# muelea/tuch

Measured on AMD Instinct MI355X. Metric: SMPLify-DC fit iters/sec at batch 64, higher is better.
Workload: dtype f32; 1 GPU; configs[1] extended to the full stage-2 step: batch=64/GPU SMPL forward + contact_fitting_loss (L_P/L_C push/pull, winding inside test, segment filter, r2r) + backward + Adam, V=6890 F=13776, float32; bodies_per_gpu=64, global_batch=64, launch=hipGraph replay of the whole step

## Files before the change

### include/tuch_amd.h

```cpp
#ifndef TUCH_AMD_H
#define TUCH_AMD_H

#include <stddef.h>
#include <stdint.h>

#ifdef __cplusplus
extern "C" {
#endif

const char* tuch_last_error(void);
int tuch_abi_version(void);


int tuch_batch_pairwise_dist(const float* x, const float* y, int B, int Nx, int Ny, int squared,
                             float* P, void* stream);

int tuch_batch_pairwise_dist_bwd(const float* x, const float* y, const float* grad_P, int B, int Nx, int Ny,
                                 int squared, float* grad_x, float* grad_y, void* stream);

int tuch_solid_angles_bwd(const float* points, const float* triangles, const float* grad_out, const float* grad_w,
                          int B, int Q, int F, float* grad_points, float* grad_triangles, void* stream);

int tuch_solid_angles(const float* points, const float* triangles, int B, int Q, int F, float* out,
                      void* stream);
// ... 74 lines not shown
size_t tuch_smplify_stage2_fused_scratch_floats(int B);
int tuch_smplify_stage2_fused(const float* points, const int32_t* partner, const uint8_t* exterior,
                              const uint8_t* body_valid, int B, int N, int mode, float euclthres,
                              const float* small_terms, const float* r2r, const int32_t* ij, int P, float contact_scale,
                              float r2r_scale, float* share, int* ticket, float* terms, float* out, float* grad_points,
                              const tuch_contact_model* model, const void* pair_keys, void* grad_fixed_zeroed, void* stream);
int tuch_fixed_to_float(const void* fixed, size_t n, float* out, void* stream);
void tuch_set_deterministic(int on);
int tuch_get_deterministic(void);

int tuch_region_pair_keys(const tuch_contact_model* model, const float* verts, int B, const uint8_t* select,
                          int use_geomask, void* keys_zeroed, void* stream);
int tuch_smplify_stage2_finish(const float* points, const int32_t* partner, const uint8_t* exterior,
                               const uint8_t* body_valid, int B, int N, int mode, float euclthres,
                               const float* small_terms, const float* r2r, int P, float contact_scale, float r2r_scale,
                               float* share, int* ticket, float* terms, float* out, void* stream);
int tuch_smplify_stage2_bwd(const float* grad_out, const uint8_t* body_valid, const float* points, const int32_t* partner,
                            const uint8_t* exterior, int B, int N, int mode, float euclthres, float contact_scale,
                            const int32_t* ij, int P, float r2r_scale, const float* gj, const float* gc, const float* gp,
                            int NJ, float* grad_points, float* gj_out, float* gc_out, float* gp_out, void* stream);

typedef struct tuch_contact_model tuch_contact_model;

int tuch_contact_model_create(tuch_contact_model** out, int V, int F, const int32_t* faces ,
                              const uint8_t* geomask ,
                              int num_segments, const int32_t* seg_q_off, const int32_t* seg_q_vidx,
                              const int32_t* seg_f_off, const int32_t* seg_faces,
                              int num_caps, const int32_t* cap_off, const int32_t* cap_vidx,
                              int num_regions, const int32_t* region_off, const int32_t* region_vidx,
                              int num_pairs, const int32_t* pairs);
void tuch_contact_model_destroy(tuch_contact_model* model);
int tuch_contact_model_set_option(tuch_contact_model* model, const char* name, int value);
int tuch_contact_model_get_option(const tuch_contact_model* model, const char* name, int* value);
int tuch_contact_model_canary_hits(const tuch_contact_model* model, int* hits_host, int reset);
int tuch_contact_model_canary_selftest(const tuch_contact_model* model, void* workspace, size_t workspace_bytes, void* stream);
const uint64_t* tuch_contact_model_mask_bits(const tuch_contact_model* model);
const int32_t* tuch_contact_model_faces(const tuch_contact_model* model);
int32_t* tuch_contact_model_tickets(const tuch_contact_model* model);
const uint64_t* tuch_contact_model_tree_mask_bits(const tuch_contact_model* model);
int tuch_contact_model_info(const tuch_contact_model* model, int* V, int* F, int* num_segments,
                            int* seg_q_total, int* num_pairs);
int tuch_contact_model_strips(const tuch_contact_model* model, int* stream_len, int* num_strips,
                              int32_t* vidx_host, float* sign_host);

int tuch_winding_tree_work(const tuch_contact_model* model, const float* verts, int B, void* workspace,
                           size_t workspace_bytes, unsigned long long* out_host, void* stream);

int tuch_ray_work(const tuch_contact_model* model, const float* verts, int B, void* workspace,
                  size_t workspace_bytes, unsigned long long* out_host, void* stream);
int tuch_contact_model_tree_order(const tuch_contact_model* model, int32_t* qperm_host, int32_t* face_leaf_host);

size_t tuch_v2v_model_workspace_bytes(const tuch_contact_model* model, int B);
size_t tuch_v2v_hint_bytes(const tuch_contact_model* model, int B);
int tuch_v2v_min_model(const tuch_contact_model* model, const float* verts, int B, float* min_d2,
                       int32_t* argmin, void* hint_inout, void* workspace, size_t workspace_bytes, void* stream);
int tuch_v2v_min_model_shared(const tuch_contact_model* model, const float* verts, int B, float* min_d2,
                              int32_t* argmin, void* hint_inout, void* workspace, size_t workspace_bytes, int leave_room,
                              void* stream);
int tuch_v2v_min_model_shared_zero(const tuch_contact_model* model, const float* verts, int B, float* min_d2, int32_t* argmin,
                                   void* hint_inout, void* workspace, size_t workspace_bytes, int leave_room, void* zero,
                                   size_t zero_bytes, void* stream);

int tuch_v2v_min_model_can_cap(const tuch_contact_model* model);
int tuch_v2v_min_model_capped(const tuch_contact_model* model, const float* verts, int B, float* min_d2, int32_t* argmin,
                              void* hint_inout, void* workspace, size_t workspace_bytes, int leave_room, void* zero,
                              size_t zero_bytes, const uint8_t* prev_exterior, float cap, void* stream);
int tuch_v2v_min_model_fix(const tuch_contact_model* model, int B, const uint8_t* exterior, uint8_t* prev_exterior, float cap,
                           float* min_d2, int32_t* argmin, void* hint_inout, void* workspace, size_t workspace_bytes,
                           void* stream);

typedef struct tuch_cluster_tree tuch_cluster_tree;
int tuch_cluster_tree_build(int V, int F, const int32_t* faces, int leaf_faces, tuch_cluster_tree** out);
void tuch_cluster_tree_free(tuch_cluster_tree* tree);
int tuch_cluster_tree_info(const tuch_cluster_tree* tree, int* num_nodes, int* exact_len, int* stream_len,
                           int* num_qblocks, int* num_frontiers, int* frontier_total);
int tuch_cluster_tree_export(const tuch_cluster_tree* tree, int32_t* nodes, int32_t* vidx, float* sign,
                             int32_t* qperm, int32_t* frontier_off, int32_t* frontier_nodes,
                             int32_t* launch_order, int32_t* rows, int32_t* face_leaf);

size_t tuch_exterior_workspace_bytes(const tuch_contact_model* model, int B);
int tuch_exterior_flags(const tuch_contact_model* model, const float* verts, int B, int apply_segments,
                        float thresh, float* w, uint8_t* exterior, float* seg_w, uint8_t* seg_exterior,
                        void* workspace, size_t workspace_bytes, void* stream);

size_t tuch_winding_points_workspace_bytes(const tuch_contact_model* model, int B, int Q);
int tuch_winding_points(const tuch_contact_model* model, const float* verts, const float* points,
                        const int32_t* counts, int B, int Q, float thresh, float* w, uint8_t* exterior,
                        void* workspace, size_t workspace_bytes, void* stream);

int tuch_region_pair_min(const tuch_contact_model* model, const float* verts, int B, const uint8_t* select,
                         int use_geomask, float* out_min, int32_t* out_ij, void* stream);
int tuch_region_pair_min_bwd(const tuch_contact_model* model, const float* verts, int B, const int32_t* ij,
                             const float* grad_out, float* grad_verts, void* stream);

int tuch_self_contact(const float* verts , const uint64_t* geomask_bits, int B, int V, float euclthres,
                      const int32_t* vreg_off , const int32_t* vreg , int R,
                      uint8_t* in_contact , int32_t* partner , float* min_d2 ,
                      float* sig_d2 , float* cnc_d2 , void* stream);

typedef struct tuch_smpl_model tuch_smpl_model;

int tuch_smpl_model_create(tuch_smpl_model** out, int V, const float* v_template, const float* shapedirs,
                           const float* posedirs, const float* J_regressor, const float* lbs_weights,
                           const int32_t* parents, const int32_t* extra_vertex_ids,
                           const float* J_regressor_extra, const int32_t* joint_map);
void tuch_smpl_model_destroy(tuch_smpl_model* model);
int tuch_smpl_model_info(const tuch_smpl_model* model, int* V);

size_t tuch_smpl_forward_workspace_bytes(const tuch_smpl_model* model, int B);
int tuch_smpl_forward(const tuch_smpl_model* model, const float* betas, const float* pose, int pose2rot, int B,
                      float* verts, float* joints, void* workspace, size_t workspace_bytes, void* stream);
int tuch_smpl_forward_split(const tuch_smpl_model* model, const float* betas, const float* global_orient,
                            int global_orient_stride, const float* body_pose, int body_pose_stride, int pose2rot, int B,
                            float* verts, float* joints, void* workspace, size_t workspace_bytes, void* stream);
size_t tuch_smpl_backward_workspace_bytes(const tuch_smpl_model* model, int B);
int tuch_smpl_backward(const tuch_smpl_model* model, const float* pose, int pose2rot, int B,
                       const void* fwd_workspace, const float* g_verts, const float* g_joints, float* g_betas,
                       float* g_pose, void* workspace, size_t workspace_bytes, void* stream);
int tuch_smpl_backward_split(const tuch_smpl_model* model, const float* global_orient, int global_orient_stride,
                             const float* body_pose, int body_pose_stride, int pose2rot, int B,
                             const void* fwd_workspace, const float* g_verts, const float* g_joints, float* g_betas,
                             float* g_global_orient, int g_global_orient_stride, float* g_body_pose,
                             int g_body_pose_stride, void* workspace, size_t workspace_bytes, void* stream);
int tuch_smpl_backward_split_add(const tuch_smpl_model* model, const float* global_orient, int global_orient_stride,
                                 const float* body_pose, int body_pose_stride, int pose2rot, int B,
                                 const void* fwd_workspace, const float* g_verts, const float* g_joints, float* g_betas,
                                 float* g_global_orient, int g_global_orient_stride, float* g_body_pose,
                                 int g_body_pose_stride, const float* g_body_pose_add, int g_body_pose_add_stride,
                                 void* workspace, size_t workspace_bytes, void* stream, const void* g_verts_fixed);
int tuch_smpl_backward_split_adam(const tuch_smpl_model* model, const float* global_orient, int global_orient_stride,
                                  const float* body_pose, int body_pose_stride, int B, const void* fwd_workspace,
                                  const float* g_verts, const float* g_joints, float* g_betas, float* g_global_orient,
                                  int g_global_orient_stride, float* g_body_pose, int g_body_pose_stride,
                                  const float* g_body_pose_add, int g_body_pose_add_stride,
                                  float* param_global_orient, int param_global_orient_stride, float* param_body_pose,
                                  int param_body_pose_stride, float* exp_avg_global_orient, float* exp_avg_sq_global_orient,
                                  float* exp_avg_body_pose, float* exp_avg_sq_body_pose, float* step, int* ticket,
                                  float lr, float beta1, float beta2, float eps,
                                  void* workspace, size_t workspace_bytes, void* stream, const void* g_verts_fixed);

int tuch_estimate_translation(const float* joints3d, const float* keypoints2d, const uint8_t* has_anno, int B, int J,
                              float focal_length, float img_size, float* trans, void* stream);
int tuch_rotmat_to_angle_axis(const float* rotmat, int N, int row_stride, float* angle_axis, void* stream);

int tuch_procrustes(const void* S1, const void* S2, int B, int N, int D, int coords_first, int is_double, void* S1_hat,
                    void* err, void* stream);
int tuch_pose_metrics(const float* pred_vertices, const float* gt_vertices, const float* gt_joints,
                      const float* J_regressor, const int32_t* joint_map, int B, int V, int R, int J, int pelvis_index,
                      float* mpjpe, float* pa_mpjpe, float* v2v, float* joints, void* stream);

typedef struct tuch_hd_model tuch_hd_model;
int tuch_hd_model_create(tuch_hd_model** out, const tuch_contact_model* contact_model, int N, const int32_t* hd_idx,
                         const float* hd_w, const int32_t* hd_face);
int tuch_hd_model_create_k(tuch_hd_model** out, const tuch_contact_model* contact_model, int N, int K,
                           const int32_t* hd_idx, const float* hd_w, const int32_t* hd_face);
void tuch_hd_model_destroy(tuch_hd_model* model);
int tuch_hd_model_info(const tuch_hd_model* model, int* N, int32_t* order_host);
size_t tuch_hd_contact_saved_bytes(const tuch_hd_model* model, int B);
size_t tuch_hd_contact_workspace_bytes(const tuch_hd_model* model, int B);
int tuch_hd_contact_fwd(const tuch_hd_model* model, const float* verts, const uint8_t* exterior, const float* min_d2,
                        const int32_t* partner, const uint8_t* valid, int B, float euclthres, float thresh, float* terms,
                        void* saved, size_t saved_bytes, void* workspace, size_t workspace_bytes, void* stream);
int tuch_hd_contact_bwd(const tuch_hd_model* model, const void* saved, const float* grad_terms, int B,
                        float* grad_verts, void* workspace, size_t workspace_bytes, void* stream);
int tuch_hd_contact_selection(const tuch_hd_model* model, const void* saved, int B, int32_t* counts_host,
                              int32_t* selected_host);
// ... 12 lines not shown
```

### tuch_amd/_C.py

```python
from __future__ import annotations

import ctypes
import os
from ctypes import POINTER, c_char_p, c_float, c_int, c_size_t, c_void_p

import torch

_HERE = os.path.dirname(os.path.abspath(__file__))
LIB_PATH = os.environ.get('TUCH_AMD_LIB') or os.path.join(_HERE, 'libtuch_amd.so')
_lib = None

_SIGNATURES = {
    'tuch_last_error': (c_char_p, []),
    'tuch_abi_version': (c_int, []),
    'tuch_batch_pairwise_dist': (c_int, [c_void_p, c_void_p, c_int, c_int, c_int, c_int, c_void_p, c_void_p]),
    'tuch_batch_pairwise_dist_bwd': (c_int, [c_void_p, c_void_p, c_void_p, c_int, c_int, c_int, c_int, c_void_p, c_void_p,
                                             c_void_p]),
    'tuch_solid_angles_bwd': (c_int, [c_void_p, c_void_p, c_void_p, c_void_p, c_int, c_int, c_int, c_void_p, c_void_p, c_void_p]),
    'tuch_solid_angles': (c_int, [c_void_p, c_void_p, c_int, c_int, c_int, c_void_p, c_void_p]),
    'tuch_gather_triangles': (c_int, [c_void_p, c_void_p, c_int, c_int, c_int, c_void_p, c_void_p]),
    'tuch_winding_workspace_bytes': (c_size_t, [c_int, c_int, c_int]),
    'tuch_winding_numbers': (c_int, [c_void_p, c_void_p, c_int, c_int, c_int, c_void_p, c_void_p, c_float,
                                     c_void_p, c_size_t, c_void_p]),
    'tuch_geomask_words': (c_int, [c_int]),
# ... 1 lines not shown
    'tuch_pack_geomask': (c_int, [c_void_p, c_int, c_void_p, c_void_p]),
    'tuch_v2v_workspace_bytes': (c_size_t, [c_int, c_int]),
    'tuch_v2v_min_masked': (c_int, [c_void_p, c_void_p, c_int, c_int, c_void_p, c_void_p, c_void_p, c_size_t,
                                    c_void_p]),
    'tuch_v2v_min_indexed_workspace_bytes': (c_size_t, [c_int, c_int]),
    'tuch_v2v_min_indexed': (c_int, [c_void_p, c_void_p, c_void_p, c_void_p, c_int, c_int, c_int, c_void_p, c_void_p,
                                     c_void_p, c_size_t, c_void_p]),
    'tuch_v2v_min_indexed_mfma_workspace_bytes': (c_size_t, [c_int, c_int]),
    'tuch_v2v_min_indexed_mfma': (c_int, [c_void_p, c_void_p, c_void_p, c_void_p, c_int, c_int, c_int, c_void_p, c_void_p,
                                          c_void_p, c_size_t, c_void_p]),
    'tuch_contact_terms_fwd': (c_int, [c_void_p, c_void_p, c_void_p, c_void_p, c_int, c_int, c_int, c_float,
                                       c_void_p, c_void_p]),
    'tuch_contact_terms_bwd': (c_int, [c_void_p, c_void_p, c_void_p, c_void_p, c_int, c_int, c_int, c_float,
                                       c_void_p, c_void_p]),
    'tuch_valid_mean_fwd': (c_int, [c_void_p, c_void_p, c_int, c_int, c_void_p, c_void_p]),
    'tuch_valid_mean_bwd': (c_int, [c_void_p, c_void_p, c_void_p, c_int, c_int, c_void_p, c_void_p]),
    'tuch_smpl_backward_split_adam': (c_int, [c_void_p, c_void_p, c_int, c_void_p, c_int, c_int, c_void_p, c_void_p, c_void_p,
                                              c_void_p, c_void_p, c_int, c_void_p, c_int, c_void_p, c_int,
                                              c_void_p, c_int, c_void_p, c_int, c_void_p, c_void_p, c_void_p, c_void_p, c_void_p,
                                              c_void_p, c_float, c_float, c_float, c_float, c_void_p, c_size_t, c_void_p, c_void_p]),
    'tuch_contact_terms_bwd_fixed': (c_int, [c_void_p, c_void_p, c_void_p, c_void_p, c_int, c_int, c_int, c_float,
                                             c_void_p, c_void_p, c_void_p]),
    'tuch_smplify_small_terms': (c_int, [c_void_p] * 9 + [c_int, c_int, c_int, c_float, c_float, c_float] + [c_void_p] * 5),
    'tuch_smplify_stage1_terms': (c_int, [c_void_p] * 7 + [c_int, c_int, c_int, c_float, c_float, c_float, c_float] + [c_void_p] * 7),
    'tuch_adam_step': (c_int, [c_int, c_void_p, c_void_p, c_void_p, c_void_p, c_void_p, c_void_p, c_void_p, c_float, c_float,
                                c_void_p]),
    'tuch_smplify_objective': (c_int, [c_void_p, c_void_p, c_void_p, c_int, c_int, c_float, c_float, c_void_p, c_void_p]),
    'tuch_smplify_objective_bwd': (c_int, [c_void_p, c_int, c_int, c_float, c_float, c_void_p, c_void_p, c_void_p,
                                           c_void_p]),
    'tuch_smplify_tail_bwd': (c_int, [c_void_p] * 5 + [c_int, c_int, c_int, c_float, c_float] + [c_void_p] * 6),
    'tuch_contact_model_create': (c_int, [POINTER(c_void_p), c_int, c_int, c_void_p, c_void_p,
                                          c_int, c_void_p, c_void_p, c_void_p, c_void_p,
                                          c_int, c_void_p, c_void_p,
                                          c_int, c_void_p, c_void_p, c_int, c_void_p]),
    'tuch_contact_model_destroy': (None, [c_void_p]),
    'tuch_contact_model_set_option': (c_int, [c_void_p, c_char_p, c_int]),
    'tuch_contact_model_get_option': (c_int, [c_void_p, c_char_p, POINTER(c_int)]),
    'tuch_contact_model_canary_hits': (c_int, [c_void_p, POINTER(c_int), c_int]),
    'tuch_contact_model_canary_selftest': (c_int, [c_void_p, c_void_p, c_size_t, c_void_p]),
    'tuch_contact_model_mask_bits': (c_void_p, [c_void_p]),
    'tuch_contact_model_faces': (c_void_p, [c_void_p]),
    'tuch_contact_model_tickets': (c_void_p, [c_void_p]),
    'tuch_contact_model_tree_mask_bits': (c_void_p, [c_void_p]),
    'tuch_contact_model_info': (c_int, [c_void_p, POINTER(c_int), POINTER(c_int), POINTER(c_int),
                                        POINTER(c_int), POINTER(c_int)]),
    'tuch_contact_model_strips': (c_int, [c_void_p, POINTER(c_int), POINTER(c_int), c_void_p, c_void_p]),
    'tuch_cluster_tree_build': (c_int, [c_int, c_int, c_void_p, c_int, POINTER(c_void_p)]),
    'tuch_cluster_tree_free': (None, [c_void_p]),
    'tuch_cluster_tree_info': (c_int, [c_void_p] + [POINTER(c_int)] * 6),
    'tuch_cluster_tree_export': (c_int, [c_void_p] * 10),
    'tuch_hd_points_fwd': (c_int, [c_void_p] * 5 + [c_int, c_int, c_void_p, c_void_p]),
    'tuch_hd_points_bwd': (c_int, [c_void_p] * 5 + [c_int, c_int, c_void_p, c_void_p]),
    'tuch_estimate_translation': (c_int, [c_void_p, c_void_p, c_void_p, c_int, c_int, c_float, c_float, c_void_p, c_void_p]),
    'tuch_rotmat_to_angle_axis': (c_int, [c_void_p, c_int, c_int, c_void_p, c_void_p]),
    'tuch_winding_tree_work': (c_int, [c_void_p, c_void_p, c_int, c_void_p, c_size_t, c_void_p, c_void_p]),
    'tuch_hd_model_create': (c_int, [POINTER(c_void_p), c_void_p, c_int, c_void_p, c_void_p, c_void_p]),
    'tuch_hd_model_create_k': (c_int, [POINTER(c_void_p), c_void_p, c_int, c_int, c_void_p, c_void_p, c_void_p]),
    'tuch_hd_model_destroy': (None, [c_void_p]),
    'tuch_hd_model_info': (c_int, [c_void_p, POINTER(c_int), c_void_p]),
    'tuch_hd_contact_saved_bytes': (c_size_t, [c_void_p, c_int]),
    'tuch_hd_contact_workspace_bytes': (c_size_t, [c_void_p, c_int]),
    'tuch_hd_contact_fwd': (c_int, [c_void_p] * 6 + [c_int, c_float, c_float, c_void_p, c_void_p, c_size_t, c_void_p, c_size_t,
                                    c_void_p]),
    'tuch_hd_contact_bwd': (c_int, [c_void_p, c_void_p, c_void_p, c_int, c_void_p, c_void_p, c_size_t, c_void_p]),
    'tuch_hd_contact_selection': (c_int, [c_void_p, c_void_p, c_int, c_void_p, c_void_p]),
    'tuch_hd_contact_details': (c_int, [c_void_p, c_void_p, c_int, c_void_p, c_void_p]),
    'tuch_ray_work': (c_int, [c_void_p, c_void_p, c_int, c_void_p, c_size_t, c_void_p, c_void_p]),
    'tuch_contact_model_tree_order': (c_int, [c_void_p, c_void_p, c_void_p]),
    'tuch_v2v_model_workspace_bytes': (c_size_t, [c_void_p, c_int]),
    'tuch_v2v_hint_bytes': (c_size_t, [c_void_p, c_int]),
    'tuch_v2v_min_model': (c_int, [c_void_p, c_void_p, c_int, c_void_p, c_void_p, c_void_p, c_void_p, c_size_t, c_void_p]),
    'tuch_v2v_min_model_shared': (c_int, [c_void_p, c_void_p, c_int, c_void_p, c_void_p, c_void_p, c_void_p, c_size_t, c_int,
                                          c_void_p]),
    'tuch_v2v_min_model_shared_zero': (c_int, [c_void_p, c_void_p, c_int, c_void_p, c_void_p, c_void_p, c_void_p, c_size_t, c_int,
                                               c_void_p, c_size_t, c_void_p]),
    'tuch_exterior_workspace_bytes': (c_size_t, [c_void_p, c_int]),
    'tuch_v2v_min_model_can_cap': (c_int, [c_void_p]),
    'tuch_v2v_min_model_capped': (c_int, [c_void_p, c_void_p, c_int, c_void_p, c_void_p, c_void_p, c_void_p, c_size_t, c_int,
                                          c_void_p, c_size_t, c_void_p, c_float, c_void_p]),
    'tuch_v2v_min_model_fix': (c_int, [c_void_p, c_int, c_void_p, c_void_p, c_float, c_void_p, c_void_p, c_void_p, c_void_p,
                                       c_size_t, c_void_p]),
    'tuch_exterior_flags': (c_int, [c_void_p, c_void_p, c_int, c_int, c_float, c_void_p, c_void_p, c_void_p,
                                    c_void_p, c_void_p, c_size_t, c_void_p]),
    'tuch_winding_points_workspace_bytes': (c_size_t, [c_void_p, c_int, c_int]),
    'tuch_winding_points': (c_int, [c_void_p, c_void_p, c_void_p, c_void_p, c_int, c_int, c_float, c_void_p, c_void_p,
                                    c_void_p, c_size_t, c_void_p]),
    'tuch_contact_terms_ragged_fwd': (c_int, [c_void_p, c_void_p, c_void_p, c_void_p, c_int, c_int, c_float, c_void_p,
                                              c_void_p]),
    'tuch_contact_terms_ragged_bwd': (c_int, [c_void_p, c_void_p, c_void_p, c_void_p, c_void_p, c_int, c_int, c_float,
                                              c_void_p, c_void_p]),
    'tuch_region_pair_min': (c_int, [c_void_p, c_void_p, c_int, c_void_p, c_int, c_void_p, c_void_p, c_void_p]),
    'tuch_smpl_model_create': (c_int, [POINTER(c_void_p), c_int] + [c_void_p] * 9),
    'tuch_smpl_model_destroy': (None, [c_void_p]),
    'tuch_smpl_model_info': (c_int, [c_void_p, POINTER(c_int)]),
    'tuch_smpl_forward_workspace_bytes': (c_size_t, [c_void_p, c_int]),
    'tuch_smpl_backward_workspace_bytes': (c_size_t, [c_void_p, c_int]),
    'tuch_smpl_forward': (c_int, [c_void_p, c_void_p, c_void_p, c_int, c_int, c_void_p, c_void_p, c_void_p,
                                  c_size_t, c_void_p]),
    'tuch_smpl_backward': (c_int, [c_void_p, c_void_p, c_int, c_int, c_void_p, c_void_p, c_void_p, c_void_p,
                                   c_void_p, c_void_p, c_size_t, c_void_p]),
    'tuch_smplify_stage2_fused_scratch_floats': (c_size_t, [c_int]),
    'tuch_smplify_stage2_fused': (c_int, [c_void_p, c_void_p, c_void_p, c_void_p, c_int, c_int, c_int, c_float, c_void_p, c_void_p,
                                           c_void_p, c_int, c_float, c_float, c_void_p, c_void_p, c_void_p, c_void_p, c_void_p,
                                           c_void_p, c_void_p, c_void_p, c_void_p]),
    'tuch_set_deterministic': (None, [c_int]),
    'tuch_get_deterministic': (c_int, []),
    'tuch_region_pair_keys': (c_int, [c_void_p, c_void_p, c_int, c_void_p, c_int, c_void_p, c_void_p]),
    'tuch_smplify_stage2_finish': (c_int, [c_void_p, c_void_p, c_void_p, c_void_p, c_int, c_int, c_int, c_float, c_void_p,
                                           c_void_p, c_int, c_float, c_float, c_void_p, c_void_p, c_void_p, c_void_p,
                                           c_void_p]),
    'tuch_smplify_stage2_bwd': (c_int, [c_void_p, c_void_p, c_void_p, c_void_p, c_void_p, c_int, c_int, c_int, c_float,
                                        c_float, c_void_p, c_int, c_float, c_void_p, c_void_p, c_void_p, c_int, c_void_p,
                                        c_void_p, c_void_p, c_void_p, c_void_p]),
    'tuch_smpl_forward_split': (c_int, [c_void_p, c_void_p, c_void_p, c_int, c_void_p, c_int, c_int, c_int, c_void_p,
                                        c_void_p, c_void_p, c_size_t, c_void_p]),
    'tuch_smpl_backward_split': (c_int, [c_void_p, c_void_p, c_int, c_void_p, c_int, c_int, c_int, c_void_p, c_void_p,
                                         c_void_p, c_void_p, c_void_p, c_int, c_void_p, c_int, c_void_p, c_size_t,
                                         c_void_p]),
    'tuch_smpl_backward_split_add': (c_int, [c_void_p, c_void_p, c_int, c_void_p, c_int, c_int, c_int, c_void_p, c_void_p,
                                             c_void_p, c_void_p, c_void_p, c_int, c_void_p, c_int, c_void_p, c_int, c_void_p,
                                             c_size_t, c_void_p, c_void_p]),
    'tuch_fixed_to_float': (c_int, [c_void_p, c_size_t, c_void_p, c_void_p]),
    'tuch_region_pair_min_bwd': (c_int, [c_void_p, c_void_p, c_int, c_void_p, c_void_p, c_void_p, c_void_p]),
    'tuch_self_contact': (c_int, [c_void_p, c_void_p, c_int, c_int, c_float, c_void_p, c_void_p, c_int] + [c_void_p] * 6),
    'tuch_procrustes': (c_int, [c_void_p, c_void_p, c_int, c_int, c_int, c_int, c_int, c_void_p, c_void_p, c_void_p]),
    'tuch_pose_metrics': (c_int, [c_void_p] * 5 + [c_int] * 5 + [c_void_p] * 5),
}


def exported_symbols():
    return sorted(_SIGNATURES)


def lib() -> ctypes.CDLL:
    global _lib
    if _lib is None:
        if not os.path.exists(LIB_PATH):
            raise RuntimeError(
                'libtuch_amd.so is not built (%s). Run `python -m tuch_amd._build` (needs hipcc); '
                'there is no CPU fallback.' % LIB_PATH)
        L = ctypes.CDLL(LIB_PATH)
        for name, (res, args) in _SIGNATURES.items():
            fn = getattr(L, name)
            fn.restype = res
            fn.argtypes = args
        _lib = L
    return _lib


class TuchError(RuntimeError):
    pass


def check(rc: int) -> None:
    if rc != 0:
        raise TuchError('libtuch_amd error %d: %s' % (rc, lib().tuch_last_error().decode()))


def ptr(t) -> c_void_p:
    if t is None:
        return c_void_p(0)
    if not t.is_cuda:
        raise TuchError('tuch_amd kernels need tensors on a HIP device, got %s' % t.device)
    if not t.is_contiguous():
        raise TuchError('tuch_amd kernels need contiguous tensors')
    return c_void_p(t.data_ptr())
# ... 19 lines not shown
```

### tuch_amd/csrc/model.h

```cpp
#pragma once
#include "common.h"
#include <vector>

struct tuch_cluster_tree {
    int V = 0, F = 0, num_nodes = 0, exact_len = 0, stream_len = 0, num_qblocks = 0, num_heights = 0;
    std::vector<int32_t> nodes;
    std::vector<int32_t> vidx;
    std::vector<float> sign;
    std::vector<int32_t> qperm;
    std::vector<int32_t> height_off, height_nodes;
    std::vector<int32_t> frontier_off, frontier_nodes;
    std::vector<int32_t> launch_order;
    std::vector<int32_t> ancestors;
    std::vector<int32_t> rows;
    std::vector<int32_t> face_leaf;
};

bool tuch_cluster_tree_build_impl(int V, int F, const int32_t* faces, int leaf_faces, tuch_cluster_tree& t);
void tuch_build_strips(const int32_t* faces, int F, std::vector<int32_t>& vidx, std::vector<float>& sign,
                       int* num_strips);

struct tuch_contact_model;

struct tuch_options {
    int winding_ray = 1;
    int winding_tree = 1;
    int winding_strips = 1;
    int tree_waves = 32768;
    int ray_pair_cap = 16;
    int ray_waves = 32768;
    int ray_fans = 0;
    int ray_cross = 0;
    int ray_cross_split = 0;
    int v2v_tree = 1;
    int v2v_waves = 0;
    int v2v_cap = 0;
    int v2v_flat = 2;
    int v2v_pairs = 24;
    int v2v_lds = -1;
    int seg_splits = 16;
    int seg_assist = 1;
    int seg_fused = 1;
    int canary = 0;
    int hd_search = 1;
    int hd_search_waves = 4;
    int hd_overlap = 1;
};
void tuch_options_from_env(tuch_options* o);

bool tuch_ray_available(const tuch_contact_model* m);
struct RayEntry { int32_t leaf, node; uint32_t mask_lo, mask_hi; };
struct RayTile { int32_t ex_off, ex_len, first, n; };
struct RayBody { int32_t tiles, overflow; };
struct TreeNode;
void tuch_ray_layout_touch(const tuch_contact_model* m, int B, int Q);
size_t tuch_ray_workspace_bytes(const tuch_contact_model* m, int B, int Q);
int tuch_ray_exterior_verts(const tuch_contact_model* m, const float* verts, int B, float thresh, uint8_t* exterior,
                            float* w, void* workspace, hipStream_t s, unsigned long long* stats_host,
                            uint8_t* exterior_copy = nullptr);
const int32_t* tuch_ray_segment_counts(const tuch_contact_model* m, int B, const void* workspace);
void tuch_ray_segment_prepare(const tuch_contact_model* m, const float* verts, const float* caps, int assisted, int B,
                              float* seg_entries, hipStream_t s);
bool tuch_ray_segment_fused_available(const tuch_contact_model* m);
int tuch_ray_segment_flags_one(const tuch_contact_model* m, const float* verts, const uint8_t* body_flags,
                               const int32_t* leaf_counts, int B, float thresh, uint8_t* exterior, hipStream_t s);
int tuch_ray_segment_flags(const tuch_contact_model* m, const float* verts, const float* caps, const int32_t* seg_count,
                           const int32_t* seg_list, const int32_t* leaf_counts, int B, int nsplit, float thresh, float* seg_tris,
                           int32_t* seg_partial, float* seg_w, uint8_t* seg_ext, uint8_t* exterior, hipStream_t s);
int tuch_ray_exterior_points(const tuch_contact_model* m, const float* verts, const float* points, const int32_t* counts,
                             int B, int Q, float thresh, uint8_t* exterior, float* w, void* workspace, hipStream_t s);

int tuch_v2v_min_indexed_seeded(const float* points, const int32_t* vertex_ids, const int32_t* offsets,
                                const int32_t* counts, const float* seed_best, const int32_t* seed_arg,
                                const int32_t* all_masked_arg, const uint64_t* geomask_bits, int B, int V,
                                int max_points_per_body, float* min_d2, int32_t* argmin, void* workspace, hipStream_t s);
extern "C" size_t tuch_v2v_min_indexed_workspace_bytes(int B, int max_points_per_body);
size_t tuch_hd_search_workspace_bytes(int B, int max_points_per_body);
int tuch_hd_search(const float* points, const int32_t* vertex_ids, const int32_t* offsets, const int32_t* counts,
                   const int32_t* all_masked_arg, const uint64_t* geomask_bits, int B, int V, int max_points_per_body,
                   float* min_d2, int32_t* argmin, void* workspace, hipStream_t s, int waves);
extern "C" size_t tuch_winding_points_workspace_bytes(const tuch_contact_model* m, int B, int Q);
extern "C" int tuch_winding_points(const tuch_contact_model* m, const float* verts, const float* points,
                                   const int32_t* counts, int B, int Q, float thresh, float* w,
                                   uint8_t* exterior, void* workspace, size_t workspace_bytes, void* stream);

struct tuch_contact_model {
    int device;
    tuch_options opt;
    int V, F;
    int32_t* faces;
    int32_t* tickets;
    int32_t* canary_hits;
    uint64_t* mask_bits;
    int strip_len, num_strips;
    int32_t* strip_vidx;
    float* strip_sign;
    int tree_nodes, tree_stream_len, tree_exact_len, tree_qblocks, tree_heights, tree_leaves;
    int32_t* tree_node;
    int32_t* tree_vidx;
    float* tree_sign;
    int32_t* tree_sign_word;
    int32_t* tree_qperm;
    int32_t* tree_height_off;
    int32_t* tree_height_nodes;
    int32_t* tree_frontier_nodes;
    int32_t* tree_launch_order;
    int32_t* tree_ancestors;
    int32_t* tree_rows;
    int32_t* tree_v2v_info;
    uint64_t* tree_mask_bits;
    uint64_t* tree_masked;
    int32_t* tree_sub_leaf;
    uint64_t* tree_masked_leaf;
    int32_t* tree_leaf_group;
    uint64_t* tree_mask_bits_g;
    int tree_groups;
    int tree_leaf_rows_max;
    int mask_symmetric;
    int tree_num_frontiers;
    int tree_leaf_runs_tile;
    int* tree_frontier_off_host;
    int* tree_sub_leaf_host;
    int32_t* tree_face_leaf_host;
    int32_t* tree_qperm_host;
    int32_t* ring_off;
    int32_t* ring_vidx;
    int ring_max;
    int num_segments, num_caps, seg_q_total, seg_f_total;
    int32_t* seg_q_off;
    int32_t* seg_q_vidx;
    int32_t* seg_f_off;
    int32_t* seg_faces;
    int32_t* cap_off;
    int32_t* cap_vidx;
    int32_t* seg_link_off;
    int32_t* seg_link;
    int32_t* seg_ray_off;
    int32_t* seg_ray_ent;
    int seg_ray_total;
    int32_t* seg_elem_mask;
    int32_t* seg_vmask;
    int32_t* seg_vpos;
// ... 19 lines not shown
```

### tuch_amd/csrc/model.hip

```cpp
#include "model.h"
#include <stdio.h>
#include <stdlib.h>
#include <string.h>
#include <algorithm>
#include <vector>
#include <unordered_map>

extern "C" int tuch_geomask_words(int V);

namespace {

template <typename T>
int upload(T** dst, const T* src, size_t count)
{
    return tuch_table_upload((void**)dst, src, count * sizeof(T));
}

int* host_copy(const int32_t* src, size_t n)
{
    int* p = (int*)malloc(sizeof(int) * (n ? n : 1));
    if (n) memcpy(p, src, sizeof(int) * n);
    return p;
}

// ... 345 lines not shown
                        m->seg_cap_total = coff.back();
                        elem_mask_host = emask;
                        rc = upload(&m->seg_elem_mask, emask.data(), emask.size());
                        if (rc == TUCH_OK) rc = upload(&m->seg_vmask, vmask.data(), vmask.size());
                        if (rc == TUCH_OK) rc = upload(&m->seg_vpos, vpos.data(), vpos.size());
                        if (rc == TUCH_OK) rc = upload(&m->seg_cap_off, coff.data(), coff.size());
                        if (rc == TUCH_OK) rc = upload(&m->seg_cap_ent, cent.data(), cent.size());
                        std::vector<int32_t> crange(1, 0);
                        bool consecutive = true;
                        for (int sg = 0; sg < num_segments && consecutive; ++sg) {
                            int lo = num_caps, hi = -1;
                            auto see = [&](int id) { if (id >= V) { lo = std::min(lo, id - V); hi = std::max(hi, id - V); } };
                            for (int e = coff[sg]; e < coff[sg + 1]; ++e)
                                for (int k = 0; k < 3; ++k) see(cent[3 * (size_t)e + k]);
                            for (int q = seg_q_off[sg]; q < seg_q_off[sg + 1]; ++q)
                                for (int e = loff[q]; e < loff[q + 1]; ++e) { see(links[2 * (size_t)e]); see(links[2 * (size_t)e + 1]); }
                            if (hi < 0) { crange.push_back(crange.back()); continue; }
                            consecutive = lo == crange.back() && hi - lo + 1 <= 8;
                            crange.push_back(hi + 1);
                        }
                        if (rc == TUCH_OK && consecutive) rc = upload(&m->seg_cap_range, crange.data(), crange.size());
                    }
                }
            }
        }
    }
    if (rc == TUCH_OK && num_regions > 0) {
        m->num_regions = num_regions;
        m->num_pairs = num_pairs;
        m->region_off_host = host_copy(region_off, num_regions + 1);
        for (int r = 0; r < num_regions; ++r) {
            const int n = region_off[r + 1] - region_off[r];
            if (n > m->region_max) m->region_max = n;
        }
        rc = upload(&m->region_off, region_off, (size_t)num_regions + 1);
        if (rc == TUCH_OK) rc = upload(&m->region_vidx, region_vidx, (size_t)region_off[num_regions]);
        if (rc == TUCH_OK && num_pairs > 0) rc = upload(&m->pairs, pairs, (size_t)num_pairs * 2);
        if (rc == TUCH_OK && num_pairs > 0 && geomask) {
            std::vector<int64_t> off(num_pairs + 1, 0);
            for (int p = 0; p < num_pairs; ++p) {
                const int n1 = region_off[pairs[2 * p] + 1] - region_off[pairs[2 * p]];
                const int n2 = region_off[pairs[2 * p + 1] + 1] - region_off[pairs[2 * p + 1]];
                off[p + 1] = off[p] + (int64_t)n1 * ((n2 + 31) / 32);
            }
            std::vector<uint32_t> words((size_t)off[num_pairs], 0u);
            for (int p = 0; p < num_pairs; ++p) {
                const int32_t* r1 = region_vidx + region_off[pairs[2 * p]];
                const int32_t* r2 = region_vidx + region_off[pairs[2 * p + 1]];
                const int n1 = region_off[pairs[2 * p] + 1] - region_off[pairs[2 * p]];
                const int n2 = region_off[pairs[2 * p + 1] + 1] - region_off[pairs[2 * p + 1]];
                const int wpr = (n2 + 31) / 32;
                for (int a = 0; a < n1; ++a)
                    for (int k = 0; k < n2; ++k)
                        if (geomask[(size_t)r1[a] * V + r2[k]])
                            words[(size_t)off[p] + (size_t)a * wpr + (k >> 5)] |= 1u << (k & 31);
            }
            rc = upload(&m->pair_mask, words.data(), words.size());
            if (rc == TUCH_OK) rc = upload(&m->pair_mask_off, off.data(), off.size());
        }
    }
    if (rc == TUCH_OK && !tree_sign_host.empty()) {
        std::vector<int32_t> word(tree_sign_host.size(), 0);
        for (size_t p = 0; p < word.size(); ++p) {
            const int32_t sg = tree_sign_host[p] > 0.0f ? 1 : tree_sign_host[p] < 0.0f ? -1 : 0;
            const int32_t em = p < elem_mask_host.size() ? elem_mask_host[p] : 0;
            word[p] = (int32_t)(((uint32_t)em << 24) | ((uint32_t)sg & 0xffffffu));
        }
        rc = upload(&m->tree_sign_word, word.data(), word.size());
    }
    if (rc != TUCH_OK) {
        tuch_contact_model_destroy(m);
        *out = nullptr;
        return rc;
    }
    *out = m;
    return TUCH_OK;
}

namespace {
struct OptionName { const char* name; int tuch_options::*field; };
const OptionName kOptions[] = {
    {"winding_ray", &tuch_options::winding_ray}, {"winding_tree", &tuch_options::winding_tree},
    {"winding_strips", &tuch_options::winding_strips}, {"tree_waves", &tuch_options::tree_waves},
    {"ray_pair_cap", &tuch_options::ray_pair_cap}, {"ray_waves", &tuch_options::ray_waves}, {"ray_fans", &tuch_options::ray_fans}, {"ray_cross", &tuch_options::ray_cross}, {"v2v_cap", &tuch_options::v2v_cap}, {"ray_cross_split", &tuch_options::ray_cross_split},
    {"v2v_tree", &tuch_options::v2v_tree}, {"v2v_flat", &tuch_options::v2v_flat}, {"v2v_pairs", &tuch_options::v2v_pairs}, {"v2v_waves", &tuch_options::v2v_waves}, {"v2v_lds", &tuch_options::v2v_lds},
    {"seg_splits", &tuch_options::seg_splits}, {"seg_assist", &tuch_options::seg_assist}, {"seg_fused", &tuch_options::seg_fused},
    {"canary", &tuch_options::canary}, {"hd_search", &tuch_options::hd_search}, {"hd_search_waves", &tuch_options::hd_search_waves}, {"hd_overlap", &tuch_options::hd_overlap},
};
}

void tuch_options_from_env(tuch_options* o)
{
    for (const OptionName& k : kOptions) {
        char env[64] = "TUCH_";
        size_t n = strlen(env);
        for (const char* c = k.name; *c && n + 1 < sizeof(env); ++c) env[n++] = (char)toupper((unsigned char)*c);
        env[n] = 0;
        const char* e = getenv(env);
        if (e && *e) o->*(k.field) = atoi(e);
    }
}

extern "C" int tuch_contact_model_set_option(tuch_contact_model* m, const char* name, int value)
{
    TUCH_REQUIRE(m && name, "tuch_contact_model_set_option: null argument");
    for (const OptionName& k : kOptions)
        if (!strcmp(k.name, name)) {
            TUCH_REQUIRE(strcmp(name, "seg_assist") != 0, "tuch_contact_model_set_option: seg_assist is fixed when the model "
                         "is created (TUCH_SEG_ASSIST)");
            m->opt.*(k.field) = value;
            return TUCH_OK;
        }
    tuch_set_error("tuch_contact_model_set_option: unknown option '%s'", name);
    return TUCH_ERR_ARG;
}

extern "C" int tuch_contact_model_canary_hits(const tuch_contact_model* m, int* hits_host, int reset)
{
    TUCH_REQUIRE(m && hits_host, "tuch_contact_model_canary_hits: null argument");
    if (hipDeviceSynchronize() != hipSuccess ||
        hipMemcpy(hits_host, m->canary_hits, sizeof(int32_t), hipMemcpyDeviceToHost) != hipSuccess ||
        (reset && hipMemset(m->canary_hits, 0, sizeof(int32_t)) != hipSuccess)) {
        tuch_set_error("tuch_contact_model_canary_hits: %s", hipGetErrorString(hipGetLastError()));
        return TUCH_ERR_HIP;
    }
    return TUCH_OK;
}

extern "C" int tuch_contact_model_get_option(const tuch_contact_model* m, const char* name, int* value)
{
    TUCH_REQUIRE(m && name && value, "tuch_contact_model_get_option: null argument");
    if (!strcmp(name, "seg_fused_active")) {
        *value = tuch_ray_segment_fused_available(m) ? 1 : 0;
        return TUCH_OK;
    }
    for (const OptionName& k : kOptions)
        if (!strcmp(k.name, name)) {
            *value = m->opt.*(k.field);
            return TUCH_OK;
        }
    tuch_set_error("tuch_contact_model_get_option: unknown option '%s'", name);
    return TUCH_ERR_ARG;
}

extern "C" const uint64_t* tuch_contact_model_mask_bits(const tuch_contact_model* m)
{
    return m ? m->mask_bits : nullptr;
}

extern "C" const uint64_t* tuch_contact_model_tree_mask_bits(const tuch_contact_model* m)
{
    return m ? m->tree_mask_bits : nullptr;
}

extern "C" int32_t* tuch_contact_model_tickets(const tuch_contact_model* m)
{
    return m ? m->tickets : nullptr;
}

extern "C" const int32_t* tuch_contact_model_faces(const tuch_contact_model* m)
{
    return m ? m->faces : nullptr;
}

extern "C" int tuch_contact_model_tree_order(const tuch_contact_model* m, int32_t* qperm_host, int32_t* face_leaf_host)
{
    TUCH_REQUIRE(m, "tuch_contact_model_tree_order: null model");
// ... 32 lines not shown
```

### tuch_amd/csrc/ray_winding.hip

```cpp
#include "common.h"
#include "model.h"
#include "workspace.h"
#include "tree_device.h"
#include <stdlib.h>

#pragma clang fp contract(off)

namespace {

constexpr float kPi = 3.14159265358979323846f;
constexpr int kBlock = 256;
constexpr int kRayQueries = 64;
constexpr float kShearX = 0.3217f, kShearY = 0.4331f;
constexpr float kFanX = 0.8191f, kFanY = 0.3467f, kFanZ = 0.4571f;
constexpr int kSlabs = 9;
constexpr int kSlabStride = 10;
constexpr int kNearSlabs = 13;

struct RayElem { float x, y, z, sign; };

__device__ __forceinline__ float shear_x(float x, float z) { return __builtin_fmaf(-kShearX, z, x); }
__device__ __forceinline__ float shear_y(float y, float z) { return __builtin_fmaf(-kShearY, z, y); }

__global__ __launch_bounds__(kBlock) void ray_stream_kernel(
// ... 4 lines not shown
    const int p = blockIdx.x * kBlock + threadIdx.x;
    for (size_t g = ((size_t)b * gridDim.x + blockIdx.x) * kBlock + threadIdx.x; g < zeroed_n;
         g += (size_t)gridDim.x * gridDim.y * kBlock)
        zeroed[g] = make_uint4(0u, 0u, 0u, 0u);
    if (p >= Lpad) return;
    RayElem e = {0.f, 0.f, 0.f, 0.f};
    if (p < L) {
        const float* c = verts + ((size_t)b * V + vidx[p]) * 3;
        e.x = shear_x(c[0], c[2]); e.y = shear_y(c[1], c[2]); e.z = c[2]; e.sign = sign[p];
    }
    out[(size_t)b * Lpad + p] = e;
}

__device__ __forceinline__ void slab_project(float x, float y, float z, float (&p)[kSlabs])
{
    p[0] = x; p[1] = y; p[2] = z;
    p[3] = x + y; p[4] = x - y; p[5] = x + z; p[6] = x - z; p[7] = y + z; p[8] = y - z;
}

template <int kCtrl>
__device__ __forceinline__ float dpp_move(float x)
{
    return __int_as_float(__builtin_amdgcn_update_dpp(0, __float_as_int(x), kCtrl, 0xF, 0xF, true));
}
__device__ __forceinline__ float row_min(float v)
{
    v = fminf(v, dpp_move<0xB1>(v));
    v = fminf(v, dpp_move<0x4E>(v));
    v = fminf(v, dpp_move<0x141>(v));
    v = fminf(v, dpp_move<0x140>(v));
    return v;
}

__device__ __forceinline__ uint32_t half_below(float x)
{
    const _Float16 h = (_Float16)x;
    uint32_t u = __builtin_bit_cast(uint16_t, h);
    if ((float)h > x) u = (u & 0x8000u) ? u + 1 : (u == 0 ? 0x8001u : u - 1);
    return u;
}
__device__ __forceinline__ uint32_t half_above(float x)
{
    const _Float16 h = (_Float16)x;
    uint32_t u = __builtin_bit_cast(uint16_t, h);
    if ((float)h < x) u = (u & 0x8000u) ? (u == 0x8000u ? 0x0001u : u - 1) : u + 1;
    return u;
}
__device__ __host__ __forceinline__ size_t near_records_at(int B, int L) { return (size_t)B * kNearSlabs * L; }
__device__ __host__ __forceinline__ size_t near_centres_at(int B, int L) { return near_records_at(B, L) + (size_t)B * L * 8; }

struct QRec { float x, y, z; int32_t tag; };
constexpr int kNoSlot = 0xffffff;
struct RayPre { int blocks, qblocks; QRec* qrec; float4* ranges; const int32_t* vmask; };

__device__ __forceinline__ void ray_block_prepass(const float* __restrict__ vb, int first_vertex,
                                                  const int32_t* __restrict__ qperm, const int32_t* __restrict__ vmask,
                                                  int Q, int qb, int lane, QRec* __restrict__ qrec, float4* __restrict__ ranges)
{
    const int slot = qb * kRayQueries + lane;
    const float* q3 = vb + 3 * (size_t)qperm[slot];
    const float* c0 = vb + 3 * (size_t)first_vertex;
    const float qz = q3[2], qx = shear_x(q3[0], qz), qy = shear_y(q3[1], qz);
    const float cz = c0[2], cx = shear_x(c0[0], cz), cy = shear_y(c0[1], cz);
    QRec r;
    r.x = qx; r.y = qy; r.z = qz;
    r.tag = slot < Q ? (slot | (vmask ? vmask[slot] << 24 : 0)) : kNoSlot;
    qrec[slot] = r;
    const float rx = qx - cx, ry = qy - cy, rz = qz - cz;
    const float r4 = rx + ry, r5 = rx - ry, r6 = rx + rz, r7 = rx - rz, r8 = ry + rz, r9 = ry - rz;
    const float bx0 = wave_min_uniform(rx), bx1 = wave_max_uniform(rx), by0 = wave_min_uniform(ry), by1 = wave_max_uniform(ry);
    const float b40 = wave_min_uniform(r4), b41 = wave_max_uniform(r4), b50 = wave_min_uniform(r5), b51 = wave_max_uniform(r5);
    const float bz0 = wave_min_uniform(rz), b60 = wave_min_uniform(r6), b71 = wave_max_uniform(r7);
    const float b80 = wave_min_uniform(r8), b91 = wave_max_uniform(r9);
    if (lane == 0) {
        ranges[0] = make_float4(bx0, bx1, by0, by1);
        ranges[1] = make_float4(b40, b41, b50, b51);
        ranges[2] = make_float4(bz0, b60, b71, b80);
        ranges[3] = make_float4(b91, 0.f, 0.f, 0.f);
    }
}

__device__ __forceinline__ float fan_terms(const float* __restrict__ vb, int v, bool real, int& n,
                                           const int32_t* __restrict__ ring_off, const int32_t* __restrict__ ring_vidx);
template <bool kPose>
__global__ __launch_bounds__(kBoundsBlock) void ray_leaf_bounds_kernel(
    const RayElem* __restrict__ stream, int T, const TreeNode* __restrict__ nodes, int N,
    const int32_t* __restrict__ height_off, const int32_t* __restrict__ height_nodes, float* __restrict__ bounds,
    const float* __restrict__ verts, const int32_t* __restrict__ vidx, const float* __restrict__ sign, int V, int Lexact,
    RayElem* __restrict__ stream_out, uint4* __restrict__ zeroed, size_t zeroed_n,
    int leaf_blocks = 0, const int32_t* __restrict__ qperm = nullptr, const int32_t* __restrict__ ring_off = nullptr,
    const int32_t* __restrict__ ring_vidx = nullptr, float2* __restrict__ fans = nullptr, int fan_stride = 0,
    RayPre pre = RayPre{0, 0, nullptr, nullptr, nullptr})
{
    if (kPose && pre.blocks > 0 && (int)blockIdx.x >= (int)gridDim.x - pre.blocks) {
        for (size_t g = ((size_t)blockIdx.y * gridDim.x + blockIdx.x) * kBoundsBlock + threadIdx.x; g < zeroed_n;
             g += (size_t)gridDim.x * gridDim.y * kBoundsBlock)
            zeroed[g] = make_uint4(0u, 0u, 0u, 0u);
        const int qb = ((int)blockIdx.x - ((int)gridDim.x - pre.blocks)) * (kBoundsBlock / 64) + (int)(threadIdx.x >> 6);
        if (qb < pre.qblocks)
            ray_block_prepass(verts + (size_t)blockIdx.y * V * 3, vidx[0], qperm, pre.vmask, V, qb, threadIdx.x & 63,
                              pre.qrec + (size_t)blockIdx.y * pre.qblocks * kRayQueries,
                              pre.ranges + ((size_t)blockIdx.y * pre.qblocks + qb) * 4);
        return;
    }
    if (kPose && leaf_blocks > 0 && (int)blockIdx.x >= leaf_blocks) {
        for (size_t g = ((size_t)blockIdx.y * gridDim.x + blockIdx.x) * kBoundsBlock + threadIdx.x; g < zeroed_n;
             g += (size_t)gridDim.x * gridDim.y * kBoundsBlock)
            zeroed[g] = make_uint4(0u, 0u, 0u, 0u);
        const int i = ((int)blockIdx.x - leaf_blocks) * kBoundsBlock + (int)threadIdx.x;
        const bool real = i < V;
        const int v = qperm[real ? i : V - 1];
        int cr = 0;
        const float half = fan_terms(verts + (size_t)blockIdx.y * V * 3, v, real, cr, ring_off, ring_vidx);
        if (i < fan_stride) fans[(size_t)blockIdx.y * fan_stride + i] = make_float2(__int_as_float(cr), half);
        return;
    }
    const int b = blockIdx.y;
    const RayElem* st = stream + (size_t)b * T;
    const int group = threadIdx.x >> 4, sub = threadIdx.x & 15;
    const int i = height_off[0] + blockIdx.x * (kBoundsBlock / 16) + group;
    const bool real = i < height_off[1];
    const int node = height_nodes[real ? i : height_off[0]];
    const int off = nodes[node].ex_off, len = real ? nodes[node].ex_len : 0;
    if (kPose) {
        for (size_t g = ((size_t)b * gridDim.x + blockIdx.x) * kBoundsBlock + threadIdx.x; g < zeroed_n;
             g += (size_t)gridDim.x * gridDim.y * kBoundsBlock)
            zeroed[g] = make_uint4(0u, 0u, 0u, 0u);
        if (blockIdx.x == 0)
            for (int p = Lexact + (int)threadIdx.x; p < T; p += kBoundsBlock) stream_out[(size_t)b * T + p] = RayElem{0.f, 0.f, 0.f, 0.f};
    }
    float lo[kSlabs], nhi[kSlabs];
#pragma unroll
    for (int k = 0; k < kSlabs; ++k) { lo[k] = 3.0e38f; nhi[k] = 3.0e38f; }
    for (int p = sub; p < len; p += 16) {
        RayElem e;
        if (kPose) {
            const float* c = verts + ((size_t)b * V + vidx[off + p]) * 3;
            e.x = shear_x(c[0], c[2]); e.y = shear_y(c[1], c[2]); e.z = c[2]; e.sign = sign[off + p];
            stream_out[(size_t)b * T + off + p] = e;
        } else {
            e = st[off + p];
        }
        float pr[kSlabs];
        slab_project(e.x, e.y, e.z, pr);
#pragma unroll
        for (int k = 0; k < kSlabs; ++k) { lo[k] = fminf(lo[k], pr[k]); nhi[k] = fminf(nhi[k], -pr[k]); }
    }
#pragma unroll
    for (int k = 0; k < kSlabs; ++k) { lo[k] = row_min(lo[k]); nhi[k] = row_min(nhi[k]); }
    if (real && sub == 0) {
        const int L = height_off[1] - height_off[0], leaf = i - height_off[0];
        float lo_p[kSlabs], hi_p[kSlabs];
#pragma unroll
        for (int k = 0; k < kSlabs; ++k) {
            const float hi = -nhi[k];
            const float pad = 4e-7f * fmaxf(fabsf(lo[k]), fabsf(hi)) + 1e-9f;
            lo_p[k] = lo[k] - pad;
            hi_p[k] = hi + pad;
        }
        float c[3];
        if (kPose) {
            const float* c0 = verts + ((size_t)b * V + vidx[0]) * 3;
            c[0] = shear_x(c0[0], c0[2]); c[1] = shear_y(c0[1], c0[2]); c[2] = c0[2];
        } else {
            const RayElem e0 = st[0];
            c[0] = e0.x; c[1] = e0.y; c[2] = e0.z;
        }
        float pc[kSlabs];
        slab_project(c[0], c[1], c[2], pc);
        uint32_t lo_h[kSlabs], hi_h[kSlabs];
#pragma unroll
        for (int k = 0; k < kSlabs; ++k) {
            const float pad = 4e-6f * (fabsf(lo_p[k]) + fabsf(hi_p[k]) + fabsf(pc[k])) + 1e-7f;
            lo_h[k] = half_below(lo_p[k] - pc[k] - pad);
            hi_h[k] = half_above(hi_p[k] - pc[k] + pad);
        }
        uint4* r = reinterpret_cast<uint4*>(bounds + near_records_at(gridDim.y, L)) + ((size_t)b * L + leaf) * 2;
        r[0] = make_uint4(lo_h[0] | lo_h[1] << 16, lo_h[3] | lo_h[4] << 16, lo_h[6] | lo_h[8] << 16, hi_h[0] | hi_h[1] << 16);
        r[1] = make_uint4(hi_h[2] | hi_h[3] << 16, hi_h[4] | hi_h[5] << 16, hi_h[7] | (uint32_t)leaf << 16, (uint32_t)node);
        if (leaf == 0) *reinterpret_cast<float4*>(bounds + near_centres_at(gridDim.y, L) + (size_t)b * 4) = make_float4(c[0], c[1], c[2], 0.f);
    }
// ... 73 lines not shown
    s[A].z = el.z - qz;
    e[Bq] = edge_fn(s[Cq], s[A]);
    e[Cq] = edge_fn(s[A], s[Bq]);
    const int word = __float_as_int(el.sign);
    if ((word & 0xffffff) != 0) {
        const float numz = __builtin_fmaf(e[A], s[A].z, __builtin_fmaf(e[Cq], s[Cq].z, e[Bq] * s[Bq].z));
        const float mn = __builtin_fminf(__builtin_fminf(e[0], e[1]), e[2]);
        const float mx = __builtin_fmaxf(__builtin_fmaxf(e[0], e[1]), e[2]);
        int c = (int)(__builtin_fminf(mn, numz) > 0.0f) - (int)(__builtin_fmaxf(mx, numz) < 0.0f);
        const bool edge_zero = mn * mx == 0.0f;
        if (__builtin_amdgcn_ballot_w64(edge_zero)) {
            const bool tie = edge_zero & (numz != 0.0f);
            if (__builtin_amdgcn_ballot_w64(tie)) {
                if (tie) c = crossing_with_ties<kSkipIncident>(p3(s[Bq]), p3(s[Cq]), p3(s[A]), e[Bq], e[Cq], e[A]);
            }
        }
        asm("v_mad_i32_i24 %0, %1, %2, %0" : "+v"(count) : "v"(c), "s"(word));
        if (kSeg && ((uint32_t)word >> 24) != 0) {
            const uint32_t t = ((uint32_t)word >> 24) & (uint32_t)qmask;
            if (__builtin_amdgcn_ballot_w64((t != 0) & (c != 0))) {
                uint32_t cs;
                asm("v_mul_i32_i24 %0, %1, %2" : "=v"(cs) : "v"(c), "s"(word));
                pa += cs * (((t & 15u) * 0x00204081u) & 0x01010101u);
                pb += cs * ((((t >> 4) & 15u) * 0x00204081u) & 0x01010101u);
            }
        }
    }
}

template <bool kSkipIncident, bool kSeg>
__device__ __forceinline__ void ray_run(const RayElem* __restrict__ st, int off, int len,
                                        S3 (&s)[3], float (&e)[3], v2f qxy, float qz, int& count,
                                        int qmask, uint32_t& pa, uint32_t& pb)
{
    const RayElem* p = st + off;
    RayElem n0 = p[0], n1 = p[1], n2 = p[2];
    for (int left = len; left > 0; left -= 3, p += 3) {
        asm("" : "+s"(left));
        const RayElem e0 = n0, e1 = n1, e2 = n2;
        n0 = p[3]; n1 = p[4]; n2 = p[5];
        ray_step<0, kSkipIncident, kSeg>(e0, s, e, qxy, qz, count, qmask, pa, pb);
        ray_step<1, kSkipIncident, kSeg>(e1, s, e, qxy, qz, count, qmask, pa, pb);
        ray_step<2, kSkipIncident, kSeg>(e2, s, e, qxy, qz, count, qmask, pa, pb);
    }
}

constexpr int kFallbackChunks = 8;

__device__ __forceinline__ float wave_min(float v) { return wave_min_uniform(v); }
__device__ __forceinline__ float wave_max(float v) { return wave_max_uniform(v); }


__device__ __forceinline__ float lo_minus(uint32_t s, float q)
{
    float d;
    asm("v_fma_mix_f32 %0, %1, 1.0, -%2 op_sel_hi:[1,0,0]" : "=v"(d) : "v"(s), "v"(q));
    return d;
}
__device__ __forceinline__ float hi_minus(uint32_t s, float q)
{
    float d;
    asm("v_fma_mix_f32 %0, %1, 1.0, -%2 op_sel:[1,0,0] op_sel_hi:[1,0,0]" : "=v"(d) : "v"(s), "v"(q));
    return d;
}
__device__ __forceinline__ float minus_lo(float q, uint32_t s)
{
    float d;
    asm("v_fma_mix_f32 %0, -%1, 1.0, %2 op_sel_hi:[1,0,0]" : "=v"(d) : "v"(s), "v"(q));
    return d;
}
__device__ __forceinline__ float minus_hi(float q, uint32_t s)
{
    float d;
    asm("v_fma_mix_f32 %0, -%1, 1.0, %2 op_sel:[1,0,0] op_sel_hi:[1,0,0]" : "=v"(d) : "v"(s), "v"(q));
    return d;
}
__device__ __forceinline__ float max3(float a, float b, float c)
{
    float d;
    asm("v_max3_f32 %0, %1, %2, %3" : "=v"(d) : "v"(a), "v"(b), "v"(c));
    return d;
}

template <bool kVerts, int kWaves>
__global__ __launch_bounds__(64 * kWaves) void ray_near_kernel(
    const float* __restrict__ pts, const TreeNode* __restrict__ nodes, const float* __restrict__ bounds, int N,
    int num_leaves, const int32_t* __restrict__ qperm,
    const int32_t* __restrict__ counts, int Q, int qblocks, RayEntry* __restrict__ lists, int32_t* __restrict__ list_len,
    int32_t* __restrict__ leaf_cnt,
    unsigned long long* __restrict__ stats,
    const int32_t* __restrict__ ring_off = nullptr, const int32_t* __restrict__ ring_vidx = nullptr,
    float2* __restrict__ fans = nullptr)
{
    if (kVerts && (int)blockIdx.x >= qblocks) {
        const int i = ((int)blockIdx.x - qblocks) * (64 * kWaves) + (int)threadIdx.x;
        const bool real = i < Q;
        const int v = qperm[real ? i : Q - 1];
        int cr = 0;
        const float half = fan_terms(pts + (size_t)blockIdx.y * Q * 3, v, real, cr, ring_off, ring_vidx);
        if (i < qblocks * kRayQueries) fans[(size_t)blockIdx.y * qblocks * kRayQueries + i] = make_float2(__int_as_float(cr), half);
        return;
    }
    __builtin_amdgcn_s_setprio(3);
    const int qb = blockIdx.x, b = blockIdx.y, lane = threadIdx.x & 63;
    const int wave = kWaves > 1 ? __builtin_amdgcn_readfirstlane(threadIdx.x >> 6) : 0;
    __shared__ uint4 queue[64 * kWaves][2];
    __shared__ float range[16];
    __shared__ int queued[2], slots;
    int i0;
    bool real;
    if (kVerts) {
        i0 = qperm[qb * kRayQueries + lane];
        real = qb * kRayQueries + lane < Q;
    } else {
        const int n = counts ? counts[b] : Q;
        if (qb * kRayQueries >= n) {
            if (threadIdx.x == 0) list_len[(size_t)b * qblocks + qb] = 0;
            return;
        }
        i0 = min(qb * kRayQueries + lane, n - 1);
        real = qb * kRayQueries + lane < n;
    }
    if (threadIdx.x == 0) { queued[0] = 0; queued[1] = 0; slots = 0; }
    const float4 ctr = *reinterpret_cast<const float4*>(bounds + near_centres_at(gridDim.y, num_leaves) + (size_t)b * 4);
    const uint4* recs = reinterpret_cast<const uint4*>(bounds + near_records_at(gridDim.y, num_leaves)) + (size_t)b * num_leaves * 2;
    struct Chunk { uint4 r0, r1; };
    auto load_chunk = [&](int base) {
        Chunk c;
        const int lc = min(base + lane, num_leaves - 1);
        c.r0 = recs[lc * 2];
        c.r1 = recs[lc * 2 + 1];
        return c;
    };
    Chunk nxt = load_chunk(wave * 64);
    const float* q3 = pts + ((size_t)b * Q + i0) * 3;
    const float qz = q3[2];
    const float qx = shear_x(q3[0], qz), qy = shear_y(q3[1], qz);
    const float rx = qx - ctr.x, ry = qy - ctr.y, rz = qz - ctr.z;
    const float r4 = rx + ry, r5 = rx - ry, r6 = rx + rz, r7 = rx - rz, r8 = ry + rz, r9 = ry - rz;
    float bx0, bx1, by0, by1, b40, b41, b50, b51, bz0, b60, b71, b80, b91;
    if (kWaves == 4) {
        if (wave == 0) {
            const float a = wave_min(rx), c = wave_max(rx), d = wave_min(ry), e = wave_max(ry);
            if (lane == 0) { range[0] = a; range[1] = c; range[2] = d; range[3] = e; }
        } else if (wave == 1) {
            const float a = wave_min(r4), c = wave_max(r4), d = wave_min(r5), e = wave_max(r5);
            if (lane == 0) { range[4] = a; range[5] = c; range[6] = d; range[7] = e; }
        } else if (wave == 2) {
            const float a = wave_min(rz), c = wave_min(r6), d = wave_max(r7);
            if (lane == 0) { range[8] = a; range[9] = c; range[10] = d; }
        } else {
            const float a = wave_min(r8), c = wave_max(r9);
            if (lane == 0) { range[11] = a; range[12] = c; }
        }
        __syncthreads();
        bx0 = range[0]; bx1 = range[1]; by0 = range[2]; by1 = range[3]; b40 = range[4]; b41 = range[5]; b50 = range[6];
        b51 = range[7]; bz0 = range[8]; b60 = range[9]; b71 = range[10]; b80 = range[11]; b91 = range[12];
    } else {
        bx0 = wave_min(rx); bx1 = wave_max(rx); by0 = wave_min(ry); by1 = wave_max(ry);
        b40 = wave_min(r4); b41 = wave_max(r4); b50 = wave_min(r5); b51 = wave_max(r5);
        bz0 = wave_min(rz); b60 = wave_min(r6); b71 = wave_max(r7); b80 = wave_min(r8); b91 = wave_max(r9);
    }
    RayEntry* list = lists + ((size_t)b * qblocks + qb) * num_leaves;
    unsigned long long useful = 0, listed = 0;
    auto outside13 = [&](const uint4& s0, const uint4& s1, float x1, float x0, float y1, float y0, float p1, float p0,
                         float m1, float m0, float z0, float xz0, float xz1, float yz0, float yz1) {
        float out = max3(lo_minus(s0.x, x1), minus_lo(x0, s0.w), hi_minus(s0.x, y1));
        out = max3(out, minus_hi(y0, s0.w), lo_minus(s0.y, p1));
        out = max3(out, minus_hi(p0, s1.x), hi_minus(s0.y, m1));
        out = max3(out, minus_lo(m0, s1.y), minus_lo(z0, s1.x));
        out = max3(out, minus_hi(xz0, s1.y), lo_minus(s0.z, xz1));
        return max3(out, minus_lo(yz0, s1.z), hi_minus(s0.z, yz1));
    };
    auto outside = [&](const uint4& s0, const uint4& s1) {
        return outside13(s0, s1, rx, rx, ry, ry, r4, r4, r5, r5, rz, r6, r7, r8, r9);
    };
    int nslots = 0;
    auto emit = [&](const uint4& s1, unsigned long long hit) {
        if (!hit) return;
        const int leaf = (int)(s1.z >> 16), nd = (int)s1.w;
        if (kWaves == 1) ++nslots;
        if (lane == 0) {
            const int slot = kWaves == 1 ? nslots - 1 : atomicAdd(&slots, 1);
            list[slot] = RayEntry{leaf, nd, (uint32_t)hit, (uint32_t)(hit >> 32)};
            atomicAdd(&leaf_cnt[(size_t)b * num_leaves + leaf], __builtin_popcountll(hit));
        }
        if (stats) {
            const int len = nodes[nd].ex_len;
            useful += (unsigned long long)__builtin_popcountll(hit) * len;
            listed += 64ull * len;
        }
    };
    auto sync = [&] { if (kWaves > 1) __syncthreads(); else __builtin_amdgcn_wave_barrier(); };
    for (int round = 0; round * 64 * kWaves < num_leaves; ++round) {
        const int base = (round * kWaves + wave) * 64;
        const Chunk c = nxt;
        if (base + 64 * kWaves < num_leaves) nxt = load_chunk(base + 64 * kWaves);
        const bool pass = (base + lane < num_leaves) &
                          !(outside13(c.r0, c.r1, bx1, bx0, by1, by0, b41, b40, b51, b50, bz0, b60, b71, b80, b91) > 0.0f);
        const unsigned long long mask = __builtin_amdgcn_ballot_w64(pass);
        if (mask) {
            int at = 0;
            if (kWaves > 1) {
                if (lane == 0) at = atomicAdd(&queued[round & 1], __builtin_popcountll(mask));
                at = __builtin_amdgcn_readfirstlane(at);
            }
            at += __builtin_amdgcn_mbcnt_hi((uint32_t)(mask >> 32), __builtin_amdgcn_mbcnt_lo((uint32_t)mask, 0));
            if (pass) { queue[at][0] = c.r0; queue[at][1] = c.r1; }
        }
        sync();
        const int n = kWaves > 1 ? queued[round & 1] : __builtin_popcountll(mask);
        if (kWaves > 1 && threadIdx.x == 0) queued[(round + 1) & 1] = 0;
        if (kWaves == 1) {
            for (int i = 0; i < n; i += 4) {
                const int k1 = min(i + 1, n - 1), k2 = min(i + 2, n - 1), k3 = min(i + 3, n - 1);
                const uint4 a0 = queue[i][0], a1 = queue[i][1], c0 = queue[k1][0], c1 = queue[k1][1];
                const uint4 d0 = queue[k2][0], d1 = queue[k2][1], f0 = queue[k3][0], f1 = queue[k3][1];
                const float out_a = outside(a0, a1), out_c = outside(c0, c1), out_d = outside(d0, d1), out_f = outside(f0, f1);
                const unsigned long long hit_a = __builtin_amdgcn_ballot_w64(real && !(out_a > 0.0f));
                const unsigned long long hit_c = __builtin_amdgcn_ballot_w64(real && !(out_c > 0.0f) && i + 1 < n);
                const unsigned long long hit_d = __builtin_amdgcn_ballot_w64(real && !(out_d > 0.0f) && i + 2 < n);
                const unsigned long long hit_f = __builtin_amdgcn_ballot_w64(real && !(out_f > 0.0f) && i + 3 < n);
                emit(a1, hit_a);
                emit(c1, hit_c);
                emit(d1, hit_d);
                emit(f1, hit_f);
            }
        } else
        for (int i = wave * 2; i < n; i += kWaves * 2) {
            const int k = i + 1 < n ? i + 1 : i;
            const uint4 a0 = queue[i][0], a1 = queue[i][1], c0 = queue[k][0], c1 = queue[k][1];
            const float out_a = outside(a0, a1), out_c = outside(c0, c1);
            const unsigned long long hit_a = __builtin_amdgcn_ballot_w64(real && !(out_a > 0.0f));
            const unsigned long long hit_c = __builtin_amdgcn_ballot_w64(real && !(out_c > 0.0f) && k != i);
            emit(a1, hit_a);
            emit(c1, hit_c);
        }
        sync();
    }
    if (stats && lane == 0) { atomicAdd(stats + 1, useful); atomicAdd(stats + 2, listed); }
    if (threadIdx.x == 0) list_len[(size_t)b * qblocks + qb] = kWaves == 1 ? nslots : slots;
}

constexpr int kTilesBlock = 256;
__global__ __launch_bounds__(kTilesBlock) void ray_tiles_kernel(
    const int32_t* __restrict__ leaf_cnt, const TreeNode* __restrict__ nodes, const int32_t* __restrict__ leaf_nodes,
    int num_leaves, int cap, int max_tiles, int fallback_tiles, int32_t* __restrict__ leaf_off,
    RayTile* __restrict__ tiles, RayBody* __restrict__ body)
{
    const int b = blockIdx.x, t = threadIdx.x;
    const int per = (num_leaves + kTilesBlock - 1) / kTilesBlock;
    const int l0 = min(t * per, num_leaves), l1 = min(l0 + per, num_leaves);
    const int32_t* cnt = leaf_cnt + (size_t)b * num_leaves;
    int pairs = 0, ntile = 0;
    for (int l = l0; l < l1; ++l) { pairs += cnt[l]; ntile += (cnt[l] + 63) >> 6; }
    __shared__ int sp[kTilesBlock], st[kTilesBlock];
    sp[t] = pairs;
    st[t] = ntile;
    __syncthreads();
    for (int d = 1; d < kTilesBlock; d <<= 1) {
        const int ap = t >= d ? sp[t - d] : 0, at = t >= d ? st[t - d] : 0;
        __syncthreads();
        sp[t] += ap;
        st[t] += at;
        __syncthreads();
    }
    const int total_pairs = sp[kTilesBlock - 1], total_tiles = st[kTilesBlock - 1];
    const bool overflow = total_pairs > cap || total_tiles > max_tiles;
    if (t == 0) body[b] = RayBody{overflow ? fallback_tiles : total_tiles, overflow ? 1 : 0};
    if (overflow) return;
    int off = sp[t] - pairs, tile = st[t] - ntile;
    RayTile* out = tiles + (size_t)b * max_tiles;
    for (int l = l0; l < l1; ++l) {
        leaf_off[(size_t)b * num_leaves + l] = off;
        const TreeNode nd = nodes[leaf_nodes[l]];
        for (int k = 0; k < cnt[l]; k += 64) out[tile++] = RayTile{nd.ex_off, nd.ex_len, off + k, min(64, cnt[l] - k)};
        off += cnt[l];
    }
}

__global__ __launch_bounds__(64) void ray_fill_kernel(
    const RayEntry* __restrict__ lists, const int32_t* __restrict__ list_len, const RayBody* __restrict__ body,
    const int32_t* __restrict__ leaf_off, int num_leaves, int qblocks, int cap, int32_t* __restrict__ leaf_fill,
    int32_t* __restrict__ pairs)
{
    const int qb = blockIdx.x, b = blockIdx.y, lane = threadIdx.x;
    if (body[b].overflow) return;
    const int cnt = list_len[(size_t)b * qblocks + qb];
    const RayEntry* list = lists + ((size_t)b * qblocks + qb) * num_leaves;
    int32_t* out = pairs + (size_t)b * cap;
    for (int base = 0; base < cnt; base += 64) {
        const int j = base + lane;
        RayEntry e = RayEntry{0, 0, 0u, 0u};
        int dst = 0;
        if (j < cnt) {
            e = list[j];
            const int n = __builtin_popcount(e.mask_lo) + __builtin_popcount(e.mask_hi);
            dst = leaf_off[(size_t)b * num_leaves + e.leaf] + atomicAdd(&leaf_fill[(size_t)b * num_leaves + e.leaf], n);
        }
        const int m = min(64, cnt - base);
        for (int k = 0; k < m; ++k) {
            const uint32_t lo = __builtin_amdgcn_readlane(e.mask_lo, k), hi = __builtin_amdgcn_readlane(e.mask_hi, k);
            const int d = __builtin_amdgcn_readlane(dst, k);
            const unsigned long long mask = ((unsigned long long)hi << 32) | lo;
            if ((mask >> lane) & 1ull)
                out[d + __builtin_popcountll(mask & ((1ull << lane) - 1ull))] = qb * kRayQueries + lane;
        }
    }
}

constexpr int kTilesFillBlock = 64, kFillSplit = 64, kFillMaxBlocks = 2048;
__device__ __forceinline__ int wave_inclusive_scan(int v, int lane)
{
#pragma unroll
    for (int d = 1; d < 64; d <<= 1) {
        const int up = __shfl_up(v, d, 64);
        if (lane >= d) v += up;
    }
    return v;
}
__global__ __launch_bounds__(kTilesFillBlock) void ray_tiles_fill_kernel(
    const int32_t* __restrict__ leaf_cnt, const TreeNode* __restrict__ nodes, const int32_t* __restrict__ leaf_nodes,
    int num_leaves, int cap, int max_tiles, int fallback_tiles, RayTile* __restrict__ tiles, RayBody* __restrict__ body,
    const RayEntry* __restrict__ lists, const int32_t* __restrict__ list_len, int qblocks, int32_t* __restrict__ leaf_fill,
    int32_t* __restrict__ pairs, int list_stride)
{
    __builtin_amdgcn_s_setprio(3);
    extern __shared__ int32_t dyn[];
    int32_t* off_s = dyn;
    int32_t* tile_s = dyn + num_leaves;
    int32_t* blk = dyn + 2 * num_leaves;
    const int b = blockIdx.x, lane = threadIdx.x;
    const int per = (num_leaves + 63) / 64;
    const int l0 = min(lane * per, num_leaves), l1 = min(l0 + per, num_leaves);
    const int perq = (qblocks + 63) / 64;
    const int q0 = min(lane * perq, qblocks), q1 = min(q0 + perq, qblocks);
    const int32_t* cnt = leaf_cnt + (size_t)b * num_leaves;
    const int32_t* len = list_len + (size_t)b * qblocks;
    int npairs = 0, ntile = 0, nent = 0;
    for (int l = l0; l < l1; ++l) { const int c = cnt[l]; npairs += c; ntile += (c + 63) >> 6; }
    for (int q = q0; q < q1; ++q) nent += len[q];
    const int sp = wave_inclusive_scan(npairs, lane), st = wave_inclusive_scan(ntile, lane), sq = wave_inclusive_scan(nent, lane);
    const int total_pairs = __builtin_amdgcn_readlane(sp, 63), total_tiles = __builtin_amdgcn_readlane(st, 63);
    const int total = __builtin_amdgcn_readlane(sq, 63);
    const bool overflow = total_pairs > cap || total_tiles > max_tiles;
    if (lane == 0 && blockIdx.y == 0) body[b] = RayBody{overflow ? fallback_tiles : total_tiles, overflow ? 1 : 0};
    if (overflow) return;
    {
        int off = sp - npairs, tile = st - ntile;
        for (int l = l0; l < l1; ++l) {
            const int c = cnt[l];
            off_s[l] = off;
            tile_s[l] = tile;
            off += c;
            tile += (c + 63) >> 6;
        }
        int ent = sq - nent;
        for (int q = q0; q < q1; ++q) { blk[q] = ent; ent += len[q]; }
        if (lane == 0) blk[qblocks] = total;
    }
    __syncthreads();
    for (int l = (int)blockIdx.y + (int)gridDim.y * lane; l < num_leaves; l += (int)gridDim.y * 64) {
        const TreeNode nd = nodes[leaf_nodes[l]];
        const int ex_off = nd.ex_off, ex_len = nd.ex_len;
        const int c = cnt[l], off = off_s[l];
        RayTile* out = tiles + (size_t)b * max_tiles + tile_s[l];
        for (int k = 0; k < c; k += 64) *out++ = RayTile{ex_off, ex_len, off + k, min(64, c - k)};
    }
    int32_t* fill = leaf_fill + (size_t)b * num_leaves;
    int32_t* out = pairs + (size_t)b * cap;
    for (int base = (int)blockIdx.y * 64; base < total; base += (int)gridDim.y * 64) {
        const int g = base + lane;
        RayEntry e = RayEntry{0, 0, 0u, 0u};
        int dst = 0, qb = 0;
        if (g < total) {
            int lo = 0, hi = qblocks;
            while (hi - lo > 1) {
                const int mid = (lo + hi) >> 1;
                if (blk[mid] <= g) lo = mid; else hi = mid;
            }
            qb = lo;
            e = lists[((size_t)b * qblocks + qb) * list_stride + (g - blk[qb])];
            dst = off_s[e.leaf] + atomicAdd(&fill[e.leaf], __builtin_popcount(e.mask_lo) + __builtin_popcount(e.mask_hi));
        }
        const int m = min(64, total - base);
        for (int k = 0; k < m; ++k) {
            const uint32_t lo = __builtin_amdgcn_readlane(e.mask_lo, k), hi = __builtin_amdgcn_readlane(e.mask_hi, k);
            const int d = __builtin_amdgcn_readlane(dst, k), q = __builtin_amdgcn_readlane(qb, k);
            const unsigned long long mask = ((unsigned long long)hi << 32) | lo;
            if ((mask >> lane) & 1ull)
                out[d + __builtin_popcountll(mask & ((1ull << lane) - 1ull))] = q * kRayQueries + lane;
        }
    }
}

template <bool kVerts, bool kCount, bool kSeg>
__global__ __launch_bounds__(64) void ray_leaf_kernel(
    const float* __restrict__ pts, const RayElem* __restrict__ stream, const RayTile* __restrict__ tiles,
    const RayBody* __restrict__ body, const int32_t* __restrict__ pairs, const RayEntry* __restrict__ lists,
    const int32_t* __restrict__ list_len, const TreeNode* __restrict__ nodes, int num_leaves,
    const int32_t* __restrict__ qperm, const int32_t* __restrict__ counts, int Q, int T, int qblocks, int num_bodies,
    int cap, int max_tiles, int32_t* __restrict__ count, unsigned long long* __restrict__ stats,
    const int32_t* __restrict__ vmask, int32_t* __restrict__ seg_count)
{
    const int lane = threadIdx.x;
    struct Work { int b, off, len, slot, qmask; bool active; float qx, qy, qz; };
    int b_cur = blockIdx.x, base = 0, g = blockIdx.y;
    auto fetch = [&]() {
        Work w;
        w.b = -1; w.off = w.len = w.slot = 0; w.qmask = 0; w.active = false; w.qx = w.qy = w.qz = 0.0f;
        while (b_cur < num_bodies) {
            const int b = b_cur;
            const int nt = __builtin_amdgcn_readfirstlane(body[b].tiles);
            if (g >= base + nt) { base += nt; b_cur += gridDim.x; continue; }
            const int t = g - base;
            g += gridDim.y;
            const float* pb = pts + (size_t)b * Q * 3;
            w.b = b;
            int i0;
            if (!__builtin_amdgcn_readfirstlane(body[b].overflow)) {
                const RayTile tile = tiles[(size_t)b * max_tiles + t];
                const int n = __builtin_amdgcn_readfirstlane(tile.n), first = __builtin_amdgcn_readfirstlane(tile.first);
                w.active = lane < n;
                w.slot = pairs[(size_t)b * cap + first + (w.active ? lane : 0)];
                i0 = kVerts ? qperm[w.slot] : w.slot;
                w.off = __builtin_amdgcn_readfirstlane(tile.ex_off);
                w.len = __builtin_amdgcn_readfirstlane(tile.ex_len);
            } else {
                const int nq = kVerts ? Q : (counts ? counts[b] : Q);
                w.slot = (t / kFallbackChunks) * kRayQueries + lane;
                w.active = w.slot < nq;
                i0 = kVerts ? qperm[w.slot] : min(w.slot, nq - 1);
                w.off = t;
                w.len = -1;
            }
            w.qz = pb[3 * i0 + 2];
            w.qx = shear_x(pb[3 * i0], w.qz);
            w.qy = shear_y(pb[3 * i0 + 1], w.qz);
            if (kSeg) w.qmask = vmask[w.slot];
            break;
        }
        return w;
    };
    int walked = 0;
    Work next = fetch();
    while (next.b >= 0) {
        const Work w = next;
        next = fetch();
        S3 s[3];
        float e[3];
#pragma unroll
        for (int k = 0; k < 3; ++k) { s[k].xy = (v2f){0.0f, 0.0f}; s[k].z = 0.0f; e[k] = 0.0f; }
        const v2f qxy = {w.qx, w.qy};
        int crossings = 0;
        uint32_t pa = kSegBias, pb = kSegBias;
        const RayElem* st = stream + (size_t)w.b * T;
        if (w.len >= 0) {
            ray_run<kVerts, kSeg>(st, w.off, w.len, s, e, qxy, w.qz, crossings, w.qmask, pa, pb);
            if (kCount) walked += w.len;
        } else {
            const int qb = w.off / kFallbackChunks, c = w.off % kFallbackChunks;
            const int cnt = __builtin_amdgcn_readfirstlane(list_len[(size_t)w.b * qblocks + qb]);
            const RayEntry* list = lists + ((size_t)w.b * qblocks + qb) * num_leaves;
            for (int j = c; j < cnt; j += kFallbackChunks) {
                const TreeNode nd = nodes[__builtin_amdgcn_readfirstlane(list[j].node)];
                ray_run<kVerts, kSeg>(st, nd.ex_off, nd.ex_len, s, e, qxy, w.qz, crossings, w.qmask, pa, pb);
                if (kCount) walked += nd.ex_len;
            }
        }
        if (w.active && crossings != 0) atomicAdd(&count[((size_t)w.b * qblocks) * kRayQueries + w.slot], crossings);
        if (kSeg && w.active && (pa != kSegBias || pb != kSegBias)) {
            int32_t* sc = seg_count + 2 * (((size_t)w.b * qblocks) * kRayQueries + w.slot);
            if (pa != kSegBias) atomicAdd(sc, (int32_t)(pa - kSegBias));
            if (pb != kSegBias) atomicAdd(sc + 1, (int32_t)(pb - kSegBias));
        }
    }
    if (kCount && lane == 0) atomicAdd(stats, (unsigned long long)walked);
}

constexpr int kCrossRing = 256, kCrossTrip = 3;
template <bool kSeg>
__global__ __launch_bounds__(64) void ray_cross_kernel(
    const RayElem* __restrict__ stream, const TreeNode* __restrict__ nodes, const float* __restrict__ bounds, int num_leaves,
    int nsplit,
    const QRec* __restrict__ qrec, const float4* __restrict__ ranges, int T, int qblocks, int num_bodies,
    int32_t* __restrict__ count, int32_t* __restrict__ seg_count)
{
    __shared__ QRec ring[kCrossRing];
    const int lane = threadIdx.x;
    const int unit = blockIdx.y / nsplit, z = blockIdx.y % nsplit;
    const int b = blockIdx.x + gridDim.x * (unit / num_leaves);
    if (b >= num_bodies) return;
    const int leaf = unit % num_leaves;
    const uint4* recs = reinterpret_cast<const uint4*>(bounds + near_records_at(num_bodies, num_leaves)) + ((size_t)b * num_leaves + leaf) * 2;
    const uint4 s0 = recs[0], s1 = recs[1];
    const float4 ctr = *reinterpret_cast<const float4*>(bounds + near_centres_at(num_bodies, num_leaves) + (size_t)b * 4);
    const TreeNode nd = nodes[(int)s1.w];
    const int ex_off = __builtin_amdgcn_readfirstlane(nd.ex_off), ex_len = __builtin_amdgcn_readfirstlane(nd.ex_len);
    const RayElem* st = stream + (size_t)b * T;
    const QRec* qb_base = qrec + (size_t)b * qblocks * kRayQueries;
    const float4* rg = ranges + (size_t)b * qblocks * 4;
    const int mine = qblocks > z ? (qblocks - z + nsplit - 1) / nsplit : 0;
    auto outside13 = [&](float x1, float x0, float y1, float y0, float p1, float p0, float m1, float m0, float z0, float xz0,
                         float xz1, float yz0, float yz1) {
        float out = max3(lo_minus(s0.x, x1), minus_lo(x0, s0.w), hi_minus(s0.x, y1));
        out = max3(out, minus_hi(y0, s0.w), lo_minus(s0.y, p1));
        out = max3(out, minus_hi(p0, s1.x), hi_minus(s0.y, m1));
        out = max3(out, minus_lo(m0, s1.y), minus_lo(z0, s1.x));
        out = max3(out, minus_hi(xz0, s1.y), lo_minus(s0.z, xz1));
        return max3(out, minus_lo(yz0, s1.z), hi_minus(s0.z, yz1));
    };
// ... 432 lines not shown
    bool active = q < Qs_total;
    const int s = active ? seg_of_q[q] : 0;
    const int k = q - seg_q_off[s];
    active = active && k < count[b * S + s];
    int n = 0;
    float half_sum = 0.0f;
    int qq = 0, v = 0;
    if (active) {
        for (int sp = 0; sp < ns; ++sp) {
            n += partial[((size_t)b * nsplit + sp) * Qs_total + q];
            half_sum += partial_half[((size_t)b * nsplit + sp) * Qs_total + q];
        }
        qq = seg_q_off[s] + list[(size_t)b * Qs_total + q];
        v = seg_q_vidx[qq];
        if (leaf_counts) n += seg_leaf_count(leaf_counts + 2 * ((size_t)b * slots + vpos[v]), s);
    }
    const float* vb = verts + (size_t)b * V * 3;
    const float* cb = caps + (size_t)b * K * 3;
    const float vx = vb[3 * v], vy = vb[3 * v + 1], vz = vb[3 * v + 2];
    const float qx = shear_x(vx, vz), qy = shear_y(vy, vz);
    const P3 u_dir = {kFanX, kFanY, kFanZ};
    const P3 us = {shear_x(kFanX, kFanZ), shear_y(kFanY, kFanZ), kFanZ};
    auto cone = [&](const float* p0, const float* p1, float ax, float ay, float az, float sx, float sy, float& h, int& c) {
        const P3 pb = {p0[0] - ax, p0[1] - ay, p0[2] - az}, pc = {p1[0] - ax, p1[1] - ay, p1[2] - az};
        const P3 sb = {shear_x(p0[0], p0[2]) - sx, shear_y(p0[1], p0[2]) - sy, p0[2] - az};
        const P3 sc = {shear_x(p1[0], p1[2]) - sx, shear_y(p1[1], p1[2]) - sy, p1[2] - az};
        int c1;
        float h1;
        cone_term(us, sb, sc, u_dir, pb, pc, c1, h1);
        h += h1;
        c += c1;
    };
    const int e0 = active ? link_off[qq] : 0, e1 = active ? link_off[qq + 1] : 0;
    constexpr int kLongLinks = 16;
    if (e1 - e0 <= kLongLinks) {
        for (int e = e0; e < e1; e += 2) {
            int id[4];
            float pp[4][3];
#pragma unroll
            for (int u = 0; u < 4; ++u) id[u] = link[2 * min(e + (u >> 1), e1 - 1) + (u & 1)];
#pragma unroll
            for (int u = 0; u < 4; ++u) {
                const float* p = id[u] < V ? vb + 3 * (size_t)id[u] : cb + 3 * (size_t)(id[u] - V);
                pp[u][0] = p[0]; pp[u][1] = p[1]; pp[u][2] = p[2];
            }
#pragma unroll
            for (int h = 0; h < 2; ++h)
                if (e + h < e1) cone(pp[2 * h], pp[2 * h + 1], vx, vy, vz, qx, qy, half_sum, n);
        }
    }
    unsigned long long todo = __builtin_amdgcn_ballot_w64(e1 - e0 > kLongLinks);
    const int lane = threadIdx.x & 63;
    while (todo) {
        const int src = __builtin_ctzll(todo);
        todo &= todo - 1;
        const int le0 = __builtin_amdgcn_readlane(e0, src), le1 = __builtin_amdgcn_readlane(e1, src);
        const float lvx = __shfl(vx, src), lvy = __shfl(vy, src), lvz = __shfl(vz, src);
        const float lqx = __shfl(qx, src), lqy = __shfl(qy, src);
        float h = 0.0f;
        int cr = 0;
        for (int e = le0 + lane; e < le1; e += 64) {
            const int i0 = link[2 * e], i1 = link[2 * e + 1];
            const float* p0 = i0 < V ? vb + 3 * (size_t)i0 : cb + 3 * (size_t)(i0 - V);
            const float* p1 = i1 < V ? vb + 3 * (size_t)i1 : cb + 3 * (size_t)(i1 - V);
            const float a0[3] = {p0[0], p0[1], p0[2]}, a1[3] = {p1[0], p1[1], p1[2]};
            cone(a0, a1, lvx, lvy, lvz, lqx, lqy, h, cr);
        }
#pragma unroll
        for (int m = 32; m >= 1; m >>= 1) { h += __shfl_xor(h, m); cr += __shfl_xor(cr, m); }
        if (lane == src) { half_sum += h; n += cr; }
    }
    if (!active) return;
    const float w = (float)n - half_sum * (0.5f / kPi);
    const size_t o = (size_t)b * Qs_total + qq;
    if (seg_w) seg_w[o] = w;
    if (seg_ext) seg_ext[o] = w <= thresh;
    if (exterior && !(w <= thresh)) exterior[(size_t)b * V + v] = 1;
}

inline size_t align256(size_t x) { return (x + 255) & ~(size_t)255; }

struct RayLayout {
    size_t stream, bounds, lists, list_len, zeroed, zeroed_bytes, leaf_cnt, leaf_fill, count, leaf_off, tiles, body, pairs,
        stats, fans, qrec, ranges, total;
    int T, qblocks, cap, max_tiles, workers, columns;
    size_t seg_count;
};

constexpr int kSegFusedMaxQ = 4096;
constexpr int kSegFusedMaxCaps = 8;

template <int kWaves>
__device__ __forceinline__ void seg_fused_caps(const float* __restrict__ vb, const int32_t* __restrict__ cap_off,
                                               const int32_t* __restrict__ cap_vidx, int c_lo, int c_hi, float* s_caps)
{
    const int lane = threadIdx.x & 63, wave = threadIdx.x >> 6;
    for (int c = c_lo + wave; c < c_hi; c += kWaves) {
        float sx = 0.f, sy = 0.f, sz = 0.f;
        const int beg = cap_off[c], end = cap_off[c + 1];
        for (int k = beg + lane; k < end; k += 64) {
            const float* p = vb + 3 * cap_vidx[k];
            sx += p[0]; sy += p[1]; sz += p[2];
        }
#pragma unroll
        for (int o = 32; o > 0; o >>= 1) { sx += __shfl_down(sx, o, 64); sy += __shfl_down(sy, o, 64); sz += __shfl_down(sz, o, 64); }
        if (lane == 0) {
            const float inv = 1.0f / (float)(end - beg);
            s_caps[3 * (c - c_lo)] = sx * inv; s_caps[3 * (c - c_lo) + 1] = sy * inv; s_caps[3 * (c - c_lo) + 2] = sz * inv;
        }
    }
}

constexpr int kSegOneBlock = 512, kSegOneWaves = kSegOneBlock / 64, kSegOneChunk = 256, kSegOneZ = 8;
constexpr int kSegOneOwn = kSegFusedMaxQ / kSegOneZ;
#ifdef TUCH_SEG_CLOCKS
__device__ unsigned long long g_seg_clocks[8192][8];
#define SEG_CLOCK(i) do { if (threadIdx.x == 0) { const int blk = (blockIdx.z * gridDim.y + blockIdx.y) * gridDim.x + blockIdx.x; if (blk < 8192) g_seg_clocks[blk][i] = __builtin_amdgcn_s_memrealtime(); } } while (0)
extern "C" int tuch_debug_seg_clocks(unsigned long long* out)
{
    return hipMemcpyFromSymbol(out, HIP_SYMBOL(g_seg_clocks), sizeof(unsigned long long) * 8192 * 8) == hipSuccess ? TUCH_OK : TUCH_ERR_HIP;
}
#else
#define SEG_CLOCK(i) do { } while (0)
#endif

__global__ __launch_bounds__(kSegOneBlock) void segment_one_kernel(
    const float* __restrict__ verts, const uint8_t* __restrict__ body_flags, uint8_t* __restrict__ exterior,
    const int32_t* __restrict__ seg_q_off, const int32_t* __restrict__ seg_q_vidx,
    const int32_t* __restrict__ cap_range, const int32_t* __restrict__ cap_off, const int32_t* __restrict__ cap_vidx,
    const int32_t* __restrict__ ent_off, const int32_t* __restrict__ ent,
    const int32_t* __restrict__ link_off, const int32_t* __restrict__ link, const int32_t* __restrict__ leaf_counts,
    const int32_t* __restrict__ vpos, int slots, int V, float thresh)
{
    __shared__ int32_t s_list[kSegFusedMaxQ];
    __shared__ int32_t s_cnt[kSegOneOwn];
    __shared__ float s_half[kSegOneOwn];
    __shared__ float sT[kSegOneChunk * 9];
    __shared__ float s_caps[kSegFusedMaxCaps * 3];
    __shared__ int32_t s_wave[kSegOneWaves];
    __shared__ int32_t s_n;
    const int sg = blockIdx.x, b = blockIdx.y, z = blockIdx.z, t = threadIdx.x, lane = t & 63, wave = t >> 6;
    const float* vb = verts + (size_t)b * V * 3;
    uint8_t* eb = exterior + (size_t)b * V;
    const int q_beg = seg_q_off[sg], nq = seg_q_off[sg + 1] - q_beg;
    SEG_CLOCK(0);
    {
        const uint8_t* fb = body_flags + (size_t)b * V;
        constexpr int kRounds = kSegFusedMaxQ / kSegOneBlock;
        uint32_t interior = 0;
#pragma unroll
        for (int r = 0; r < kRounds; ++r) {
            const int q = r * kSegOneBlock + t;
            if (q < nq && fb[seg_q_vidx[q_beg + q]] == 0) interior |= 1u << r;
        }
        if (t == 0) s_n = 0;
        __syncthreads();
        for (int r = 0; r * kSegOneBlock < nq; ++r) {
            const bool in = (interior >> r) & 1u;
            const unsigned long long bal = __builtin_amdgcn_ballot_w64(in);
            if (lane == 0) s_wave[wave] = __builtin_popcountll(bal);
            __syncthreads();
            int base = s_n;
            for (int w2 = 0; w2 < wave; ++w2) base += s_wave[w2];
            if (in) s_list[base + __builtin_popcountll(bal & ((1ull << lane) - 1ull))] = r * kSegOneBlock + t;
            __syncthreads();
            if (t == 0) { int add = 0; for (int w2 = 0; w2 < kSegOneWaves; ++w2) add += s_wave[w2]; s_n += add; }
            __syncthreads();
// ... 132 lines not shown
            const float lvx = __shfl(vx, src), lvy = __shfl(vy, src), lvz = __shfl(vz, src);
            const float lqx = __shfl(qx, src), lqy = __shfl(qy, src);
            float h = 0.0f;
            int cr = 0;
            for (int e = le0 + lane; e < le1; e += 64) {
                float a0[3], a1[3];
                pos(link[2 * e], a0);
                pos(link[2 * e + 1], a1);
                cone(a0, a1, lvx, lvy, lvz, lqx, lqy, h, cr);
            }
#pragma unroll
            for (int m2 = 32; m2 >= 1; m2 >>= 1) { h += __shfl_xor(h, m2); cr += __shfl_xor(cr, m2); }
            if (lane == src) { half_sum += h; cnt += cr; }
        }
        if (active) {
            const float w = (float)cnt - half_sum * (0.5f / kPi);
            if (!(w <= thresh)) eb[v] = 1;
        }
    }
    SEG_CLOCK(4);
}

}

bool tuch_ray_segment_fused_available(const tuch_contact_model* m)
{
    return m && m->seg_cap_off && m->seg_cap_range && m->seg_elem_mask && m->seg_q_max <= kSegFusedMaxQ && m->opt.seg_fused != 0;
}

int tuch_ray_segment_flags_one(const tuch_contact_model* m, const float* verts, const uint8_t* body_flags,
                               const int32_t* leaf_counts, int B, float thresh, uint8_t* exterior, hipStream_t s)
{
    hipLaunchKernelGGL(segment_one_kernel, dim3(m->num_segments, B, kSegOneZ), dim3(kSegOneBlock), 0, s, verts, body_flags, exterior,
                       (const int32_t*)m->seg_q_off, (const int32_t*)m->seg_q_vidx, (const int32_t*)m->seg_cap_range,
                       (const int32_t*)m->cap_off, (const int32_t*)m->cap_vidx, (const int32_t*)m->seg_cap_off,
                       (const int32_t*)m->seg_cap_ent, (const int32_t*)m->seg_link_off, (const int32_t*)m->seg_link, leaf_counts,
                       (const int32_t*)m->seg_vpos, 2 * m->tree_qblocks * kRayQueries, m->V, thresh);
    return tuch_check_launch("tuch_ray_segment_flags_one");
}

bool tuch_ray_available(const tuch_contact_model* m)
{
    if (!m || m->tree_nodes <= 0 || !m->ring_off || m->tree_exact_len <= 0) return false;
    if (m->tree_leaves > 65535) return false;
    return m->opt.winding_ray != 0;
}

static int ray_pair_cap(const tuch_contact_model* m) { return m->opt.ray_pair_cap < 1 ? 1 : m->opt.ray_pair_cap; }

static RayLayout full_layout(const tuch_contact_model* m, int B, int Q, bool verts)
{
    RayLayout l;
    l.qblocks = verts ? 2 * m->tree_qblocks : ceil_div(Q, kRayQueries);
    l.T = ceil_div(m->tree_exact_len, 3) * 3 + 6;
    const int L = m->tree_leaves;
    const long cap = (long)ray_pair_cap(m) * Q;
    l.cap = (int)(cap < 0x3fffffffL ? cap : 0x3fffffffL);
    l.max_tiles = l.cap / 64 + L;
    if (l.max_tiles < l.qblocks * kFallbackChunks) l.max_tiles = l.qblocks * kFallbackChunks;
    l.columns = B < 8 ? B : 8;
    const int waves = m->opt.ray_waves > 0 ? m->opt.ray_waves : 32768;
    l.workers = waves / l.columns > 0 ? waves / l.columns : 1;
    size_t o = 0;
    l.stream = tuch_ws_take(o, (size_t)B * l.T * sizeof(RayElem));
    l.bounds = tuch_ws_take(o, (size_t)B * m->tree_nodes * 2 * kSlabStride * sizeof(float));
    l.lists = tuch_ws_take(o, (size_t)B * l.qblocks * L * sizeof(RayEntry));
    l.list_len = tuch_ws_take(o, (size_t)B * l.qblocks * sizeof(int32_t));
    l.zeroed = o;
    l.leaf_cnt = tuch_ws_take(o, (size_t)B * L * sizeof(int32_t), false);
    l.leaf_fill = tuch_ws_take(o, (size_t)B * L * sizeof(int32_t), false);
    l.count = tuch_ws_take(o, (size_t)B * l.qblocks * kRayQueries * sizeof(int32_t), false);
    l.seg_count = o;
    if (verts && m->seg_elem_mask) o += align256(2 * (size_t)B * l.qblocks * kRayQueries * sizeof(int32_t));
    l.zeroed_bytes = o - l.zeroed;
    (void)tuch_ws_take(o, 0);
    l.leaf_off = tuch_ws_take(o, (size_t)B * L * sizeof(int32_t));
    l.tiles = tuch_ws_take(o, (size_t)B * l.max_tiles * sizeof(RayTile));
    l.body = tuch_ws_take(o, (size_t)B * sizeof(RayBody));
    l.pairs = tuch_ws_take(o, (size_t)B * l.cap * sizeof(int32_t));
    l.stats = tuch_ws_take(o, 256);
    l.fans = verts ? tuch_ws_take(o, (size_t)B * l.qblocks * kRayQueries * sizeof(float2)) : 0;
    l.qrec = verts ? tuch_ws_take(o, (size_t)B * l.qblocks * kRayQueries * sizeof(QRec)) : 0;
    l.ranges = verts ? tuch_ws_take(o, (size_t)B * l.qblocks * 4 * sizeof(float4)) : 0;
    l.total = o;
    return l;
}

void tuch_ray_layout_touch(const tuch_contact_model* m, int B, int Q)
{
    (void)full_layout(m, B, Q > 0 ? Q : m->V, Q <= 0);
}

size_t tuch_ray_workspace_bytes(const tuch_contact_model* m, int B, int Q)
{
    if (!m || m->tree_nodes <= 0 || B <= 0) return 0;
    const size_t a = full_layout(m, B, m->V, true).total;
    const size_t b = Q > 0 ? full_layout(m, B, Q, false).total : 0;
    return a > b ? a : b;
}

static bool fans_in_bounds_launch(const tuch_contact_model* m) { return m->ring_off && m->opt.ray_fans == 1 && m->tree_leaf_runs_tile; }
static bool cross_in_one_launch(const tuch_contact_model* m);
static bool fans_in_near_launch(const tuch_contact_model* m) { return m->ring_off && m->opt.ray_fans == 2 && !cross_in_one_launch(m); }

static bool cross_in_one_launch(const tuch_contact_model* m)
{
    return m->opt.ray_cross != 0 && 2L * m->tree_qblocks * kRayQueries < kNoSlot;
}

static void launch_ray_boxes(const tuch_contact_model* m, const RayLayout& l, const float* verts, int B, char* ws, hipStream_t s,
                             bool one_launch, bool query_side = false)
{
    RayElem* st = (RayElem*)(ws + l.stream);
    float* bounds = (float*)(ws + l.bounds);
    const RayPre pre{query_side ? ceil_div(l.qblocks, kBoundsBlock / 64) : 0, l.qblocks, (QRec*)(ws + l.qrec), (float4*)(ws + l.ranges),
                     (const int32_t*)m->seg_vmask};
    if (one_launch && m->tree_leaf_runs_tile) {
        const int leaf_blocks = ceil_div(m->tree_leaves, kBoundsBlock / 16);
        const bool fans = fans_in_bounds_launch(m);
        hipLaunchKernelGGL(ray_leaf_bounds_kernel<true>, dim3(leaf_blocks + (fans ? ceil_div(m->V, kBoundsBlock) : 0) + pre.blocks, B),
                           dim3(kBoundsBlock), 0,
                           s, (const RayElem*)st, l.T, (const TreeNode*)m->tree_node, m->tree_nodes,
                           (const int32_t*)m->tree_height_off, (const int32_t*)m->tree_height_nodes, bounds, verts,
                           (const int32_t*)m->tree_vidx, (const float*)m->tree_sign_word, m->V, m->tree_exact_len, st,
                           (uint4*)(ws + l.zeroed), l.zeroed_bytes / sizeof(uint4), fans ? leaf_blocks : 0,
                           (const int32_t*)m->tree_qperm, (const int32_t*)m->ring_off, (const int32_t*)m->ring_vidx,
                           (float2*)(ws + l.fans), l.qblocks * kRayQueries, pre);
        return;
    }
    if (query_side)
        hipLaunchKernelGGL(ray_prepass_kernel, dim3(pre.blocks, B), dim3(kBoundsBlock), 0, s, verts, (const int32_t*)m->tree_vidx,
                           (const int32_t*)m->tree_qperm, m->V, pre);
    hipLaunchKernelGGL(ray_stream_kernel, dim3(ceil_div(l.T, kBlock), B), dim3(kBlock), 0, s, verts,
                       (const int32_t*)m->tree_vidx, (const float*)m->tree_sign_word, m->V, m->tree_exact_len, l.T, st,
                       (uint4*)(ws + l.zeroed), l.zeroed_bytes / sizeof(uint4));
    hipLaunchKernelGGL(ray_leaf_bounds_kernel<false>, dim3(ceil_div(m->tree_leaves, kBoundsBlock / 16), B), dim3(kBoundsBlock), 0, s,
                       (const RayElem*)st, l.T, (const TreeNode*)m->tree_node, m->tree_nodes,
                       (const int32_t*)m->tree_height_off, (const int32_t*)m->tree_height_nodes, bounds,
                       (const float*)nullptr, (const int32_t*)nullptr, (const float*)nullptr, 0, 0, (RayElem*)nullptr,
                       (uint4*)nullptr, (size_t)0);
}

template <bool kVerts>
static int launch_ray_counts(const tuch_contact_model* m, const RayLayout& l, const float* verts, const float* queries,
                             const int32_t* counts, int B, int Q, char* ws, hipStream_t s, unsigned long long* stats)
{
    const bool one = kVerts && !stats && cross_in_one_launch(m);
    launch_ray_boxes(m, l, verts, B, ws, s, kVerts, one);
    const int L = m->tree_leaves;
    const TreeNode* nodes = (const TreeNode*)m->tree_node;
    if (one) {
        const int columns = B < 8 ? B : 8;
        int nsplit = m->opt.ray_cross_split > 0 ? m->opt.ray_cross_split : (B <= 8 ? 4 : B <= 32 ? 2 : 1);
        if (nsplit > l.qblocks) nsplit = l.qblocks;
        const dim3 grid(columns, ceil_div(B, columns) * L * nsplit);
        int32_t* seg_cnt = (int32_t*)(ws + l.seg_count);
        if (m->seg_elem_mask)
            hipLaunchKernelGGL(ray_cross_kernel<true>, grid, dim3(64), 0, s, (const RayElem*)(ws + l.stream), nodes, (const float*)(ws + l.bounds), L,
                               nsplit, (const QRec*)(ws + l.qrec), (const float4*)(ws + l.ranges), l.T, l.qblocks, B,
                               (int32_t*)(ws + l.count), seg_cnt);
        else
            hipLaunchKernelGGL(ray_cross_kernel<false>, grid, dim3(64), 0, s, (const RayElem*)(ws + l.stream), nodes, (const float*)(ws + l.bounds), L,
                               nsplit, (const QRec*)(ws + l.qrec), (const float4*)(ws + l.ranges), l.T, l.qblocks, B,
                               (int32_t*)(ws + l.count), seg_cnt);
        return TUCH_OK;
    }
    const int32_t* leaf_nodes = (const int32_t*)m->tree_height_nodes;
    const int32_t* qperm = kVerts ? (const int32_t*)m->tree_qperm : nullptr;
    RayEntry* lists = (RayEntry*)(ws + l.lists);
    int32_t* list_len = (int32_t*)(ws + l.list_len);
    int32_t* leaf_cnt = (int32_t*)(ws + l.leaf_cnt);
    int32_t* leaf_off = (int32_t*)(ws + l.leaf_off);
    RayTile* tiles = (RayTile*)(ws + l.tiles);
    RayBody* body = (RayBody*)(ws + l.body);
    int32_t* pairs = (int32_t*)(ws + l.pairs);
    const bool fans = kVerts && fans_in_near_launch(m);
    float2* fan_out = fans ? (float2*)(ws + l.fans) : nullptr;
    if ((long)l.qblocks * B <= 2048)
        hipLaunchKernelGGL((ray_near_kernel<kVerts, 4>), dim3(l.qblocks + (fans ? ceil_div(Q, 256) : 0), B), dim3(256), 0, s, queries, nodes,
                           (const float*)(ws + l.bounds), m->tree_nodes, L, qperm, counts, Q, l.qblocks, lists, list_len,
                           leaf_cnt, stats, (const int32_t*)m->ring_off, (const int32_t*)m->ring_vidx, fan_out);
    else
        hipLaunchKernelGGL((ray_near_kernel<kVerts, 1>), dim3(l.qblocks + (fans ? ceil_div(Q, 64) : 0), B), dim3(64), 0, s, queries, nodes,
                           (const float*)(ws + l.bounds), m->tree_nodes, L, qperm, counts, Q, l.qblocks, lists, list_len,
                           leaf_cnt, stats, (const int32_t*)m->ring_off, (const int32_t*)m->ring_vidx, fan_out);
    const size_t tf_lds = (2 * (size_t)L + l.qblocks + 1) * sizeof(int32_t);
    if (l.qblocks <= kFillMaxBlocks && tf_lds <= 48u * 1024)
        hipLaunchKernelGGL(ray_tiles_fill_kernel, dim3(B, std::min(256, std::max(kFillSplit, 2048 / B))), dim3(kTilesFillBlock), tf_lds, s, (const int32_t*)leaf_cnt,
                           nodes, leaf_nodes, L, l.cap, l.max_tiles, l.qblocks * kFallbackChunks, tiles, body,
                           (const RayEntry*)lists, (const int32_t*)list_len, l.qblocks, (int32_t*)(ws + l.leaf_fill), pairs, L);
    else {
    hipLaunchKernelGGL(ray_tiles_kernel, dim3(B), dim3(kTilesBlock), 0, s, (const int32_t*)leaf_cnt, nodes, leaf_nodes, L, l.cap,
                       l.max_tiles, l.qblocks * kFallbackChunks, leaf_off, tiles, body);
    hipLaunchKernelGGL(ray_fill_kernel, dim3(l.qblocks, B), dim3(64), 0, s, (const RayEntry*)lists, (const int32_t*)list_len,
                       (const RayBody*)body, (const int32_t*)leaf_off, L, l.qblocks, l.cap, (int32_t*)(ws + l.leaf_fill), pairs);
    }
    const dim3 grid(l.columns, l.workers);
    const bool seg = kVerts && m->seg_elem_mask;
    const int32_t* vmask = (const int32_t*)m->seg_vmask;
    int32_t* seg_count = (int32_t*)(ws + l.seg_count);
#define TUCH_LAUNCH_RAY_LEAF(COUNT, SEG)                                                                                      \
    hipLaunchKernelGGL((ray_leaf_kernel<kVerts, COUNT, SEG>), grid, dim3(64), 0, s, queries, (const RayElem*)(ws + l.stream),  \
                       (const RayTile*)tiles, (const RayBody*)body, (const int32_t*)pairs, (const RayEntry*)lists,            \
                       (const int32_t*)list_len, nodes, L, qperm, counts, Q, l.T, l.qblocks, B, l.cap, l.max_tiles,           \
                       (int32_t*)(ws + l.count), stats, vmask, seg_count)
    if (stats) {
        if (seg) TUCH_LAUNCH_RAY_LEAF(true, kVerts); else TUCH_LAUNCH_RAY_LEAF(true, false);
    } else {
        if (seg) TUCH_LAUNCH_RAY_LEAF(false, kVerts); else TUCH_LAUNCH_RAY_LEAF(false, false);
    }
#undef TUCH_LAUNCH_RAY_LEAF
    return TUCH_OK;
}

int tuch_ray_exterior_verts(const tuch_contact_model* m, const float* verts, int B, float thresh, uint8_t* exterior,
                            float* w, void* workspace, hipStream_t s, unsigned long long* stats_host, uint8_t* exterior_copy)
{
    const RayLayout l = full_layout(m, B, m->V, true);
    char* ws = (char*)workspace;
    unsigned long long* stats = stats_host ? (unsigned long long*)(ws + l.stats) : nullptr;
    if (stats && hipMemsetAsync(stats, 0, 4 * sizeof(unsigned long long), s) != hipSuccess) return TUCH_ERR_HIP;
    const int rc = launch_ray_counts<true>(m, l, verts, verts, nullptr, B, m->V, ws, s, stats);
    if (rc != TUCH_OK) return rc;
    if (w || exterior)
        hipLaunchKernelGGL(ray_finalize_verts_kernel, dim3(ceil_div(m->V, kBlock), B), dim3(kBlock), 0, s, verts,
                           (const int32_t*)(ws + l.count), (const int32_t*)m->tree_qperm, (const int32_t*)m->ring_off,
                           (const int32_t*)m->ring_vidx, m->V, l.qblocks * kRayQueries, thresh, w, exterior, exterior_copy,
                           (const float2*)(fans_in_bounds_launch(m) || fans_in_near_launch(m) ? ws + l.fans : nullptr));
    if (stats_host) {
        RayBody bodies[8];
        const int nb = B < 8 ? B : 8;
        if (hipMemcpyAsync(stats_host, stats, 3 * sizeof(unsigned long long), hipMemcpyDeviceToHost, s) != hipSuccess ||
            hipMemcpyAsync(bodies, ws + l.body, nb * sizeof(RayBody), hipMemcpyDeviceToHost, s) != hipSuccess ||
            hipStreamSynchronize(s) != hipSuccess)
            return TUCH_ERR_HIP;
        unsigned long long tiles = 0;
        for (int b = 0; b < nb; ++b) tiles += bodies[b].tiles;
        stats_host[3] = tiles * B / nb;
    }
    return tuch_check_launch("tuch_ray_exterior_verts");
}

const int32_t* tuch_ray_segment_counts(const tuch_contact_model* m, int B, const void* workspace)
{
    if (!m->seg_elem_mask) return nullptr;
    return (const int32_t*)((const char*)workspace + full_layout(m, B, m->V, true).seg_count);
}

int tuch_ray_exterior_points(const tuch_contact_model* m, const float* verts, const float* points, const int32_t* counts,
                             int B, int Q, float thresh, uint8_t* exterior, float* w, void* workspace, hipStream_t s)
{
    const RayLayout l = full_layout(m, B, Q, false);
    char* ws = (char*)workspace;
    const int rc = launch_ray_counts<false>(m, l, verts, points, counts, B, Q, ws, s, nullptr);
    if (rc != TUCH_OK) return rc;
    hipLaunchKernelGGL(ray_finalize_points_kernel, dim3(ceil_div(Q, kBlock), B), dim3(kBlock), 0, s,
                       (const int32_t*)(ws + l.count), counts, Q, l.qblocks * kRayQueries, thresh, w, exterior);
    return tuch_check_launch("tuch_ray_exterior_points");
}

void tuch_ray_segment_prepare(const tuch_contact_model* m, const float* verts, const float* caps, int assisted, int B,
                              float* seg_entries, hipStream_t s)
{
    const bool as = assisted && m->seg_cap_off;
    const int E = as ? m->seg_cap_total : m->seg_ray_total;
    hipLaunchKernelGGL(segment_shear_entries_kernel, dim3(ceil_div(E > 0 ? E : 1, kBlock), B), dim3(kBlock), 0, s,
                       verts, caps, (const int32_t*)(as ? m->seg_cap_ent : m->seg_ray_ent), m->V, m->num_caps, E, seg_entries);
}

int tuch_ray_segment_flags(const tuch_contact_model* m, const float* verts, const float* caps, const int32_t* seg_count,
                           const int32_t* seg_list, const int32_t* leaf_counts, int B, int nsplit, float thresh,
                           float* seg_entries, int32_t* seg_partial, float* seg_w, uint8_t* seg_ext, uint8_t* exterior,
                           hipStream_t s)
{
    const bool assisted = leaf_counts && m->seg_cap_off;
    const int E = assisted ? m->seg_cap_total : m->seg_ray_total;
    const int32_t* ent_off = (const int32_t*)(assisted ? m->seg_cap_off : m->seg_ray_off);
    float* partial_half = (float*)(seg_partial + (size_t)B * nsplit * m->seg_q_total);
    int2* items = (int2*)(partial_half + (size_t)B * nsplit * m->seg_q_total);
    int32_t* items_total = (int32_t*)(items + (size_t)B * m->num_seg_blocks);
    const long worst = (long)B * m->num_seg_blocks * nsplit;
    const int grid = (int)(worst < 8192 ? worst : 8192);
    hipLaunchKernelGGL(segment_items_kernel, dim3(1), dim3(kItemsBlock), 0, s, seg_count, B * m->num_segments, items, items_total,
                       nsplit, grid);
    hipLaunchKernelGGL(segment_ray_kernel, dim3((unsigned)grid), dim3(64), 0, s, verts,
                       (const float*)seg_entries, (const int2*)items, (const int32_t*)items_total, (const int32_t*)m->seg_q_off,
                       (const int32_t*)m->seg_q_vidx, ent_off, seg_count, seg_list, m->V, E,
                       m->seg_q_total, m->num_segments, nsplit, seg_partial, partial_half);
    hipLaunchKernelGGL(segment_ray_finalize_kernel, dim3(ceil_div(m->seg_q_total, kBlock), B), dim3(kBlock), 0, s, verts, caps,
                       (const int32_t*)seg_partial, (const float*)partial_half, (const int32_t*)m->seg_of_q,
                       (const int32_t*)m->seg_q_off, (const int32_t*)m->seg_q_vidx, (const int32_t*)m->seg_link_off,
                       (const int32_t*)m->seg_link, seg_count, seg_list, assisted ? leaf_counts : nullptr,
                       (const int32_t*)m->seg_vpos, 2 * m->tree_qblocks * kRayQueries, m->V,
                       m->num_caps, m->seg_q_total, m->num_segments, nsplit, (const int32_t*)items_total, thresh, seg_w, seg_ext,
                       exterior);
    return tuch_check_launch("tuch_ray_segment_flags");
}
```

### tuch_amd/csrc/winding.hip

```cpp
#include "common.h"
#include "model.h"
#include "workspace.h"
#include "tree_device.h"
#include <stdlib.h>

namespace {

constexpr float kPi = 3.14159265358979323846f;
constexpr float kHalfPi = 1.57079632679489661923f;
constexpr int kBlock = 256;
constexpr int kQueriesPerLane = 2;
constexpr int kQueriesPerBlock = kBlock * kQueriesPerLane;
constexpr int kStripBlock = 128;
constexpr int kStripQueries = kStripBlock * kQueriesPerLane;

__device__ __forceinline__ v2f atan_poly(v2f t)
{
    const v2f s = t * t;
    v2f p = splat2(0.0024567253421992064f);
    p = fma2(p, s, splat2(-0.014401361346244812f));
    p = fma2(p, s, splat2(0.03978123143315315f));
    p = fma2(p, s, splat2(-0.07234857976436615f));
    p = fma2(p, s, splat2(0.10498946160078049f));
    p = fma2(p, s, splat2(-0.14161229133605957f));
// ... 745 lines not shown
                       (const int32_t*)m->tree_height_off, (const int32_t*)m->tree_height_nodes, m->tree_heights,
                       bounds);
}

void launch_tree_walk(const tuch_contact_model* m, const ExteriorLayout& l, const float* verts, int B, char* ws,
                      unsigned long long* stats, hipStream_t s)
{
    StreamElem* st = (StreamElem*)(ws + l.tris);
    const int T = m->tree_stream_len + 3;
    float* bounds = (float*)(ws + l.bounds);
    launch_tree_boxes(m, verts, B, st, bounds, s);
    const int f0 = m->tree_frontier_off_host[l.tree_frontier];
    const dim3 grid(B < 8 ? B : 8, 2 * l.tree_subs * m->tree_qblocks, ceil_div(B, 8));
    const int32_t* frontier = (const int32_t*)m->tree_frontier_nodes + f0;
    const int32_t* ancestors = (const int32_t*)m->tree_ancestors + (size_t)f0 * kMaxAncestors;
    const int32_t* order = (const int32_t*)m->tree_launch_order + (size_t)f0 * m->tree_qblocks;
    if (stats)
        hipLaunchKernelGGL(winding_tree_kernel<true>, grid, dim3(64), 0, s, verts, (const StreamElem*)st,
                           (const TreeNode*)m->tree_node, (const float*)bounds, m->tree_nodes, frontier, ancestors, order,
                           (const int32_t*)m->tree_qperm, (const int32_t*)nullptr, m->V, T, l.tree_subs, B, (float*)(ws + l.partial), stats);
    else
        hipLaunchKernelGGL(winding_tree_kernel<false>, grid, dim3(64), 0, s, verts, (const StreamElem*)st,
                           (const TreeNode*)m->tree_node, (const float*)bounds, m->tree_nodes, frontier, ancestors, order,
                           (const int32_t*)m->tree_qperm, (const int32_t*)nullptr, m->V, T, l.tree_subs, B, (float*)(ws + l.partial), stats);
}

}

extern "C" size_t tuch_winding_workspace_bytes(int B, int Q, int F)
{
    if (B <= 0 || Q <= 0 || F <= 0) return 0;
    return (size_t)B * choose_splits(B, Q, F) * Q * sizeof(float);
}

extern "C" int tuch_winding_numbers(const float* points, const float* triangles, int B, int Q, int F,
                                    float* w, uint8_t* exterior, float exterior_thresh,
                                    void* workspace, size_t workspace_bytes, void* stream)
{
    TUCH_REQUIRE(points && triangles && (w || exterior), "tuch_winding_numbers: null pointer");
    TUCH_REQUIRE(B > 0 && B <= 65535 && Q > 0 && F > 0, "tuch_winding_numbers: bad sizes B=%d Q=%d F=%d", B, Q, F);
    const int nsplit = choose_splits(B, Q, F);
    const size_t need = (size_t)B * nsplit * Q * sizeof(float);
    if (!workspace || workspace_bytes < need) {
        tuch_set_error("tuch_winding_numbers: workspace %zu < %zu bytes", workspace_bytes, need);
        return TUCH_ERR_WORKSPACE;
    }
    hipStream_t s = (hipStream_t)stream;
    const int per_split = ceil_div(F, nsplit);
    dim3 grid(ceil_div(Q, kQueriesPerBlock), nsplit, B);
    hipLaunchKernelGGL(winding_partial_kernel, grid, dim3(kBlock), 0, s, points, triangles, Q, F,
                       per_split, (float*)workspace);
    hipLaunchKernelGGL(winding_finalize_kernel, dim3(ceil_div(Q, kBlock), B), dim3(kBlock), 0, s,
                       (const float*)workspace, Q, Q, nsplit, exterior_thresh, w, exterior);
    return tuch_check_launch("tuch_winding_numbers");
}

extern "C" int tuch_solid_angles(const float* points, const float* triangles, int B, int Q, int F,
                                 float* out, void* stream)
{
    TUCH_REQUIRE(points && triangles && out, "tuch_solid_angles: null pointer");
    TUCH_REQUIRE(B > 0 && Q > 0 && F > 0 && F <= 65535 && B <= 65535, "tuch_solid_angles: bad sizes");
    hipLaunchKernelGGL(solid_angles_kernel, dim3(ceil_div(Q, kBlock), F, B), dim3(kBlock), 0,
                       (hipStream_t)stream, points, triangles, Q, F, out);
    return tuch_check_launch("tuch_solid_angles");
}

extern "C" int tuch_gather_triangles(const float* verts, const int32_t* faces, int B, int V, int F,
                                     float* triangles, void* stream)
{
    TUCH_REQUIRE(verts && faces && triangles, "tuch_gather_triangles: null pointer");
    TUCH_REQUIRE(B > 0 && V > 0 && F > 0, "tuch_gather_triangles: bad sizes");
    hipLaunchKernelGGL(gather_triangles_kernel, dim3(ceil_div(F * 3, kBlock), B), dim3(kBlock), 0,
                       (hipStream_t)stream, verts, faces, V, F, triangles);
    return tuch_check_launch("tuch_gather_triangles");
}

extern "C" size_t tuch_exterior_workspace_bytes(const tuch_contact_model* m, int B)
{
    if (!m || B <= 0) return 0;
    tuch_ws_scope scope(m->opt.canary != 0);
    return exterior_layout(m, B).total;
}

extern "C" int tuch_exterior_flags(const tuch_contact_model* m, const float* verts, int B,
                                   int apply_segments, float thresh, float* w, uint8_t* exterior,
                                   float* seg_w, uint8_t* seg_exterior,
                                   void* workspace, size_t workspace_bytes, void* stream)
{
    TUCH_REQUIRE(m && verts && exterior, "tuch_exterior_flags: null pointer");
    TUCH_REQUIRE(B > 0 && B <= 65535, "tuch_exterior_flags: bad batch %d", B);
    tuch_ws_scope scope(m->opt.canary != 0);
    const ExteriorLayout l = scope.record(0, [&] { return exterior_layout(m, B); });
    if (!workspace || workspace_bytes < l.total) {
        tuch_set_error("tuch_exterior_flags: workspace %zu < %zu bytes", workspace_bytes, l.total);
        return TUCH_ERR_WORKSPACE;
    }
    if (tuch_ray_available(m)) scope.record(l.ray, [&] { tuch_ray_layout_touch(m, B, 0); return 0; });
    scope.arm(workspace, m->canary_hits, (hipStream_t)stream);
    char* ws = (char*)workspace;
    float* tris = (float*)(ws + l.tris);
    hipStream_t s = (hipStream_t)stream;
    int rc = TUCH_OK;
    const int ray = ray_mode(m);
    const bool segments = apply_segments && m->num_segments > 0;
    const bool body_by_rays = ray == 2 || (ray == 1 && !w);
    const bool segments_by_rays = segments && m->seg_link_off && (ray == 2 || (ray == 1 && !seg_w));
    const bool segments_fused = segments && segments_by_rays && body_by_rays && !seg_w && !seg_exterior &&
                                tuch_ray_segment_fused_available(m);
    if (segments && !segments_fused) {
        if (m->num_caps > 0) {
            hipLaunchKernelGGL(cap_centroid_kernel, dim3(m->num_caps, B), dim3(64), 0, s,
                               verts, (const int32_t*)m->cap_off, (const int32_t*)m->cap_vidx, m->V,
                               m->num_caps, (float*)(ws + l.caps), (int32_t*)(ws + l.seg_count), m->num_segments);
        } else if (hipMemsetAsync(ws + l.seg_count, 0, (size_t)B * m->num_segments * sizeof(int32_t), s) != hipSuccess) {
            tuch_set_error("tuch_exterior_flags: hipMemsetAsync failed");
            return TUCH_ERR_HIP;
        }
        if (segments_by_rays)
            tuch_ray_segment_prepare(m, verts, (const float*)(ws + l.caps), body_by_rays && m->seg_elem_mask, B,
                                     (float*)(ws + l.seg_tris), s);
    }
    if (body_by_rays) {
        rc = tuch_ray_exterior_verts(m, verts, B, thresh, exterior, w, ws + l.ray, s, nullptr,
                                     segments_fused ? (uint8_t*)(ws + l.body_flags) : (uint8_t*)nullptr);
        if (rc != TUCH_OK) return rc;
    } else if (use_strips(m) && use_tree(m)) {
        launch_tree_walk(m, l, verts, B, ws, nullptr, s);
        hipLaunchKernelGGL(winding_finalize_tree_kernel, dim3(ceil_div(m->V, kBlock), B), dim3(kBlock), 0, s,
                           (const float*)(ws + l.partial), (const int32_t*)m->tree_qperm, m->V,
                           2 * m->tree_qblocks * kTreeQueries, l.tree_subs, thresh, w, exterior);
    } else if (use_strips(m) && m->strip_len > 0) {
        StreamElem* st = (StreamElem*)tris;
        hipLaunchKernelGGL(gather_stream_kernel, dim3(ceil_div(l.lpad, kBlock), B), dim3(kBlock), 0, s, verts,
                           (const int32_t*)m->strip_vidx, (const float*)m->strip_sign, m->V, m->strip_len,
                           l.lpad, st);
        const int nsplit = choose_strip_splits(B, m->V, l.lpad);
        const int per_split = ceil_div(ceil_div(l.lpad - 6, nsplit), 3) * 3;
        hipLaunchKernelGGL(winding_strip_kernel, dim3(B, nsplit, ceil_div(m->V, kStripQueries)), dim3(kStripBlock),
                           0, s, verts, (const StreamElem*)st, m->V, l.lpad, per_split, (const int32_t*)nullptr,
                           (float*)(ws + l.partial));
        hipLaunchKernelGGL(winding_finalize_kernel, dim3(ceil_div(m->V, kBlock), B), dim3(kBlock), 0, s,
                           (const float*)(ws + l.partial), m->V, m->V, nsplit, thresh, w, exterior);
    } else {
        hipLaunchKernelGGL(gather_triangles_kernel, dim3(ceil_div(m->F * 3, kBlock), B), dim3(kBlock), 0, s,
                           verts, (const int32_t*)m->faces, m->V, m->F, tris);
        rc = tuch_winding_numbers(verts, tris, B, m->V, m->F, w, exterior, thresh, ws + l.partial,
                                  l.bounds - l.partial, stream);
        if (rc != TUCH_OK) return rc;
    }
    if (segments_fused) {
        rc = tuch_ray_segment_flags_one(m, verts, (const uint8_t*)(ws + l.body_flags), tuch_ray_segment_counts(m, B, ws + l.ray), B, thresh,
                                        exterior, s);
        if (rc != TUCH_OK) return rc;
    } else if (segments) {
        float* caps = (float*)(ws + l.caps);
        float* seg_tris = (float*)(ws + l.seg_tris);
        float* seg_partial = (float*)(ws + l.seg_partial);
        int32_t* seg_count = (int32_t*)(ws + l.seg_count);
        int32_t* seg_list = (int32_t*)(ws + l.seg_list);
        const bool all = seg_w || seg_exterior;
        hipLaunchKernelGGL(segment_compact_kernel, dim3(ceil_div(m->seg_q_total, kBlock), B), dim3(kBlock), 0, s,
                           all ? (const uint8_t*)nullptr : (const uint8_t*)exterior, (const int32_t*)m->seg_of_q,
                           (const int32_t*)m->seg_q_off, (const int32_t*)m->seg_q_vidx, m->V, m->seg_q_total,
                           m->num_segments, seg_count, seg_list);
        if (segments_by_rays) {
            rc = tuch_ray_segment_flags(m, verts, caps, seg_count, seg_list,
                                        body_by_rays ? tuch_ray_segment_counts(m, B, ws + l.ray) : nullptr, B, seg_splits(m),
                                        thresh, seg_tris, (int32_t*)seg_partial, seg_w, seg_exterior, exterior, s);
            if (rc != TUCH_OK) return rc;
            return tuch_check_launch("tuch_exterior_flags");
        }
        hipLaunchKernelGGL(gather_segment_triangles_kernel, dim3(ceil_div(m->seg_f_total * 3, kBlock), B),
                           dim3(kBlock), 0, s, verts, (const float*)caps, (const int32_t*)m->seg_faces,
                           m->V, m->num_caps, m->seg_f_total, seg_tris);
        hipLaunchKernelGGL(segment_winding_kernel, dim3(B, seg_splits(m), m->num_seg_blocks), dim3(kSegBlock),
                           0, s, verts, (const float*)seg_tris, (const int32_t*)m->seg_blocks,
                           (const int32_t*)m->seg_q_off, (const int32_t*)m->seg_q_vidx,
                           (const int32_t*)m->seg_f_off, (const int32_t*)seg_count, (const int32_t*)seg_list,
                           m->V, m->seg_f_total, m->seg_q_total, m->num_segments, seg_partial);
        hipLaunchKernelGGL(segment_finalize_kernel, dim3(ceil_div(m->seg_q_total, kBlock), B), dim3(kBlock), 0, s,
                           (const float*)seg_partial, (const int32_t*)m->seg_of_q, (const int32_t*)m->seg_q_off,
                           (const int32_t*)m->seg_q_vidx, (const int32_t*)seg_count, (const int32_t*)seg_list,
                           m->V, m->seg_q_total, m->num_segments, seg_splits(m), thresh, seg_w, seg_exterior, exterior);
    }
    return tuch_check_launch("tuch_exterior_flags");
}

extern "C" int tuch_winding_tree_work(const tuch_contact_model* m, const float* verts, int B,
                                      void* workspace, size_t workspace_bytes, unsigned long long* out_host, void* stream)
{
    TUCH_REQUIRE(m && verts && out_host, "tuch_winding_tree_work: null pointer");
    TUCH_REQUIRE(m->tree_nodes > 0, "tuch_winding_tree_work: the model has no cluster tree");
    TUCH_REQUIRE(B > 0 && B <= 65535, "tuch_winding_tree_work: bad batch %d", B);
    const ExteriorLayout l = exterior_layout(m, B);
    if (!workspace || workspace_bytes < l.total) {
        tuch_set_error("tuch_winding_tree_work: workspace %zu < %zu bytes", workspace_bytes, l.total);
        return TUCH_ERR_WORKSPACE;
    }
    char* ws = (char*)workspace;
    hipStream_t s = (hipStream_t)stream;
    unsigned long long* stats = (unsigned long long*)(ws + l.stats);
    if (hipMemsetAsync(stats, 0, 2 * sizeof(unsigned long long), s) != hipSuccess) return TUCH_ERR_HIP;
    launch_tree_walk(m, l, verts, B, ws, stats, s);
    if (hipMemcpyAsync(out_host, stats, 2 * sizeof(unsigned long long), hipMemcpyDeviceToHost, s) != hipSuccess ||
        hipStreamSynchronize(s) != hipSuccess) {
        tuch_set_error("tuch_winding_tree_work: copy back failed");
        return TUCH_ERR_HIP;
    }
    out_host[2] = (unsigned long long)B * l.tree_subs * m->tree_qblocks * 2;
    out_host[3] = (unsigned long long)m->strip_len;
    return tuch_check_launch("tuch_winding_tree_work");
}

extern "C" int tuch_ray_work(const tuch_contact_model* m, const float* verts, int B, void* workspace,
                             size_t workspace_bytes, unsigned long long* out_host, void* stream)
{
    TUCH_REQUIRE(m && verts && out_host, "tuch_ray_work: null pointer");
    TUCH_REQUIRE(tuch_ray_available(m), "tuch_ray_work: the model has no cluster tree / vertex rings");
    TUCH_REQUIRE(B > 0 && B <= 65535, "tuch_ray_work: bad batch %d", B);
    const ExteriorLayout l = exterior_layout(m, B);
    if (!workspace || workspace_bytes < l.total) {
        tuch_set_error("tuch_ray_work: workspace %zu < %zu bytes", workspace_bytes, l.total);
        return TUCH_ERR_WORKSPACE;
    }
    return tuch_ray_exterior_verts(m, verts, B, 0.99f, nullptr, nullptr, (char*)workspace + l.ray, (hipStream_t)stream, out_host);
}

struct PointsLayout { size_t stream, bounds, partial, total; int frontier, nsub, qblocks; };

static PointsLayout points_layout(const tuch_contact_model* m, int B, int Q)
{
    PointsLayout l;
    l.qblocks = ceil_div(Q, kTreeQueries);
    int f = 0;
    while (f + 1 < m->tree_num_frontiers &&
           (long)B * l.qblocks * (m->tree_frontier_off_host[f + 1] - m->tree_frontier_off_host[f]) < 65536L) ++f;
    l.frontier = f;
    l.nsub = m->tree_frontier_off_host[f + 1] - m->tree_frontier_off_host[f];
    size_t o = 0;
    l.stream = tuch_ws_take(o, (size_t)B * (m->tree_stream_len + 3) * sizeof(StreamElem));
    l.bounds = tuch_ws_take(o, (size_t)B * m->tree_nodes * 2 * kSlabStride * sizeof(float));
    l.partial = tuch_ws_take(o, (size_t)B * l.nsub * l.qblocks * kTreeQueries * sizeof(float));
    l.total = o;
    return l;
}

extern "C" size_t tuch_winding_points_workspace_bytes(const tuch_contact_model* m, int B, int Q)
{
    if (!m || B <= 0 || Q <= 0) return 0;
    tuch_ws_scope scope(m->opt.canary != 0);
    const int lpad = strip_lpad(m->strip_len);
    const size_t flat = align256((size_t)B * lpad * sizeof(StreamElem)) +
                        align256((size_t)B * choose_strip_splits(B, Q, lpad) * Q * sizeof(float));
    if (m->tree_nodes <= 0) return flat;
    size_t tree = points_layout(m, B, Q).total;
    const size_t ray = tuch_ray_workspace_bytes(m, B, Q);
    if (ray > tree) tree = ray;
    return tree > flat ? tree : flat;
}

extern "C" int tuch_winding_points(const tuch_contact_model* m, const float* verts, const float* points,
                                   const int32_t* counts, int B, int Q, float thresh, float* w,
                                   uint8_t* exterior, void* workspace, size_t workspace_bytes, void* stream)
{
    TUCH_REQUIRE(m && verts && points && (w || exterior), "tuch_winding_points: null pointer");
    TUCH_REQUIRE(B > 0 && B <= 65535 && Q > 0, "tuch_winding_points: bad sizes B=%d Q=%d", B, Q);
    const size_t need = tuch_winding_points_workspace_bytes(m, B, Q);
    if (!workspace || workspace_bytes < need) {
        tuch_set_error("tuch_winding_points: workspace %zu < %zu bytes", workspace_bytes, need);
        return TUCH_ERR_WORKSPACE;
// ... 50 lines not shown
```

### tuch_amd/ops.py

```python
from __future__ import annotations

import contextlib
import ctypes
import os
import weakref
from typing import Dict, List, Optional, Sequence, Tuple

import numpy as np
import torch
from torch.autograd.function import once_differentiable

from . import _C, backward_pass
from .backward_pass import backward_scalar

MODE_SMPLIFY = 0
MODE_TRAIN = 1


def _f32(t: torch.Tensor) -> torch.Tensor:
    if t.dtype is torch.float32 and t.is_contiguous():
        return t.detach()
    return t.detach().to(torch.float32).contiguous()


# ... 599 lines not shown


_DERIVED = {}


def cached_derived(key_tensors, build):
    key = tuple((t.data_ptr(), t._version, tuple(t.shape)) if t is not None else None for t in key_tensors)
    hit = _DERIVED.get(key)
    if hit is None:
        while len(_DERIVED) >= 256:
            _DERIVED.pop(next(iter(_DERIVED)))
        hit = (build(), key_tensors)
        _DERIVED[key] = hit
    return hit[0]


def region_tables(cdict):
    csig = cdict['csig']
    names = list(csig.keys())
    index = {n: i for i, n in enumerate(names)}

    def find(key):
        for k in (key, str(key)):
            try:
                if k in index:
                    return index[k]
            except TypeError:
                pass
        if hasattr(key, 'item'):
            return find(key.item())
        raise KeyError('region %r of cdict[\'classes\'] is not a key of cdict[\'csig\']' % (key,))
    regions = [np.asarray(csig[n], dtype=np.int64) for n in names]
    pairs = np.asarray([[find(p[0]), find(p[1])] for p in cdict['classes']], np.int64).reshape(-1, 2)
    return regions, pairs


def _i32(a) -> np.ndarray:
    return np.ascontiguousarray(np.asarray(a), dtype=np.int32)


def segment_faces(body_faces: np.ndarray, vidx: np.ndarray, bands: Sequence[np.ndarray], first_cap: int,
                  num_verts: Optional[int] = None) -> np.ndarray:
    body_faces = np.asarray(body_faces, np.int64)
    inside = np.isin(body_faces, np.asarray(vidx)).sum(1) == 3
    fans = []
    for k, band in enumerate(bands):
        band = np.asarray(band, np.int64)
        fans.append(np.stack([band[1:], band[:-1], np.full(len(band) - 1, first_cap + k, np.int64)], 1))
    return np.concatenate([body_faces[inside]] + fans, 0) if fans else body_faces[inside]


def cluster_tree(faces, num_verts: int, leaf_faces: int = 64) -> dict:
    L = _C.lib()
    f = np.ascontiguousarray(np.asarray(faces).reshape(-1, 3), dtype=np.int32)
    h = ctypes.c_void_p()
    _C.check(L.tuch_cluster_tree_build(int(num_verts), f.shape[0], f.ctypes.data_as(ctypes.c_void_p), int(leaf_faces),
                                       ctypes.byref(h)))
    try:
        vals = [ctypes.c_int(0) for _ in range(6)]
        _C.check(L.tuch_cluster_tree_info(h, *[ctypes.byref(v) for v in vals]))
        n, exact_len, stream_len, qblocks, nfr, frtot = [v.value for v in vals]
        out = dict(nodes=np.zeros((n, 8), np.int32), vidx=np.zeros(stream_len, np.int32),
                   sign=np.zeros(stream_len, np.float32), qperm=np.zeros(qblocks * 128, np.int32),
                   frontier_off=np.zeros(nfr + 1, np.int32), frontier_nodes=np.zeros(frtot, np.int32),
                   launch_order=np.zeros(frtot * qblocks, np.int32), rows=np.zeros((n, 2), np.int32),
                   face_leaf=np.zeros(f.shape[0], np.int32))
        _C.check(L.tuch_cluster_tree_export(h, *[out[k].ctypes.data_as(ctypes.c_void_p) for k in
                                                 ('nodes', 'vidx', 'sign', 'qperm', 'frontier_off', 'frontier_nodes',
                                                  'launch_order', 'rows', 'face_leaf')]))
        out['exact_len'] = exact_len
        return out
    finally:
        L.tuch_cluster_tree_free(h)


class ContactModel:

    def __init__(self, faces, geomask=None, segments=None, regions=None, pairs=None,
                 device: Optional[torch.device] = None):
        self.device = torch.device(device if device is not None else 'cuda')
        faces = np.asarray(faces.detach().cpu() if isinstance(faces, torch.Tensor) else faces)
        self.faces_np = faces.astype(np.int64)
        self._hints = {}
        self._prev_flags = {}
        self.num_verts = int(faces.max()) + 1
        self.num_faces = int(faces.shape[0])
        gm = None
        if geomask is not None:
            gm = geomask.detach().cpu().numpy() if isinstance(geomask, torch.Tensor) else np.asarray(geomask)
            self.num_verts = max(self.num_verts, gm.shape[0])
            gm = np.ascontiguousarray(gm.astype(np.uint8))
            assert gm.shape == (self.num_verts, self.num_verts)
        self.has_mask = gm is not None
        v = self.num_verts
        segments = list(segments or [])
        seg_q_off, seg_q, seg_f_off, seg_f, cap_off, cap_v = [0], [], [0], [], [0], []
        for vidx, bands in segments:
            first_cap = v + len(cap_off) - 1
            seg_f.append(segment_faces(self.faces_np, vidx, bands, first_cap))
            seg_f_off.append(seg_f_off[-1] + len(seg_f[-1]))
            seg_q.append(np.asarray(vidx, np.int64))
            seg_q_off.append(seg_q_off[-1] + len(vidx))
            for band in bands:
                cap_v.append(np.asarray(band, np.int64))
                cap_off.append(cap_off[-1] + len(band))
        self.num_segments = len(segments)
        self.seg_q_total = seg_q_off[-1]
        self.seg_q_off = seg_q_off
        self.seg_vidx = [np.asarray(s[0], np.int64) for s in segments]
        regions = list(regions or [])
        reg_off = np.cumsum([0] + [len(r) for r in regions])
        self.num_pairs = 0 if pairs is None else len(pairs)
        cat = lambda lst, width=None: (np.concatenate(lst) if lst else np.zeros(0, np.int64))
        keep = dict(
            faces=_i32(faces), seg_q_off=_i32(seg_q_off), seg_q=_i32(cat(seg_q)), seg_f_off=_i32(seg_f_off),
            seg_f=_i32(cat(seg_f).reshape(-1, 3)), cap_off=_i32(cap_off), cap_v=_i32(cat(cap_v)),
            reg_off=_i32(reg_off), reg_v=_i32(cat([np.asarray(r) for r in regions])),
            pairs=_i32(pairs if pairs is not None else np.zeros((0, 2))))
        self._host = (keep, gm, len(cap_off) - 1, len(regions))
        self._h = None
        self._faces_i32 = None
        self._py_options = {'overlap': int(os.environ.get('TUCH_OVERLAP', '1') != '0'),
                            'v2v_hint': int(os.environ.get('TUCH_V2V_HINT', '1') != '0'),
                            'inside_first': int(os.environ.get('TUCH_INSIDE_FIRST', '1') != '0')}
        self._pending_options = {}

    @property
    def _handle(self):
        if self._h is None:
            keep, gm, num_caps, num_regions = self._host
            host_tables = os.environ.get('TUCH_HOST_TABLES', '0') not in ('', '0')
            if self.device.type != 'cuda' and not host_tables:
                raise _C.TuchError('tuch_amd kernels need a HIP device, the model was created for %s' % self.device)
            p = lambda a: a.ctypes.data_as(ctypes.c_void_p) if a.size else ctypes.c_void_p(0)
            handle = ctypes.c_void_p(0)
            with (contextlib.nullcontext() if host_tables else torch.cuda.device(self.device)):
                _C.check(_C.lib().tuch_contact_model_create(
                    ctypes.byref(handle), self.num_verts, self.num_faces, p(keep['faces']),
                    gm.ctypes.data_as(ctypes.c_void_p) if gm is not None else ctypes.c_void_p(0),
                    self.num_segments, p(keep['seg_q_off']), p(keep['seg_q']), p(keep['seg_f_off']), p(keep['seg_f']),
                    num_caps, p(keep['cap_off']), p(keep['cap_v']),
                    num_regions, p(keep['reg_off']), p(keep['reg_v']), self.num_pairs, p(keep['pairs'])))
            self._h = handle
            self._host = None
            for name, value in self._pending_options.items():
                _C.check(_C.lib().tuch_contact_model_set_option(handle, name.encode(), int(value)))
            self._pending_options = {}
        return self._h

    def set_option(self, name: str, value: int) -> None:
        if name in self._py_options:
            self._py_options[name] = int(value)
        elif self._h is None:
            self._pending_options[name] = int(value)
        else:
            _C.check(_C.lib().tuch_contact_model_set_option(self._h, name.encode(), int(value)))

    def get_option(self, name: str) -> int:
        if name in self._py_options:
            return self._py_options[name]
        out = ctypes.c_int(0)
        _C.check(_C.lib().tuch_contact_model_get_option(self._handle, name.encode(), ctypes.byref(out)))
        return out.value

    def canary_hits(self, reset: bool = True) -> int:
        out = ctypes.c_int(0)
        _C.check(_C.lib().tuch_contact_model_canary_hits(self._handle, ctypes.byref(out), int(reset)))
        return out.value

    def canary_selftest(self) -> int:
        ws = _workspace(8192, self.device)
        rc = _C.lib().tuch_contact_model_canary_selftest(self._handle, _C.ptr(ws), ws.numel(), _C.stream())
        if rc < 0:
            _C.check(rc)
        return rc

    @property
    def faces_i32(self):
        if self._faces_i32 is None:
            self._faces_i32 = torch.as_tensor(_i32(self.faces_np), device=self.device)
        return self._faces_i32

    def __del__(self):
        h = getattr(self, '_h', None)
        if h:
            try:
                _C.lib().tuch_contact_model_destroy(h)
            except Exception:
                pass
            self._h = None

    def strips(self):
        n, k = ctypes.c_int(0), ctypes.c_int(0)
        L = _C.lib()
        _C.check(L.tuch_contact_model_strips(self._handle, ctypes.byref(n), ctypes.byref(k), None, None))
        vidx = np.zeros(n.value, np.int32)
        sign = np.zeros(n.value, np.float32)
        _C.check(L.tuch_contact_model_strips(self._handle, None, None, vidx.ctypes.data_as(ctypes.c_void_p),
                                             sign.ctypes.data_as(ctypes.c_void_p)))
        return vidx, sign, k.value

    def exterior_and_partner(self, verts: torch.Tensor, apply_segments: bool = True, also=None, zero_floats: int = 0,
                             iterative: bool = False, cap: Optional[float] = None):
        zero = torch.empty((int(zero_floats) + 3) // 4 * 4, dtype=torch.float32, device=verts.device) if zero_floats > 0 else None
        call_also = (lambda: None) if also is None else also if zero is None else (lambda: also(zero))
        capped = cap is not None and verts.is_cuda and self.v2v_can_cap(verts.shape[0])
        overlap = bool(verts.is_cuda and self._py_options['overlap'])
        if overlap:
            cur, side = _current_stream(verts.device), _side_stream(verts.device)
            side.wait_stream(cur)
        first = not overlap or capped or self._py_options.get('inside_first', 0)
        exterior = self.exterior_flags(verts, apply_segments=apply_segments) if first else None
        with (torch.cuda.stream(side) if overlap else contextlib.nullcontext()):
            if overlap and zero is not None:
                zero.record_stream(side)
            mn, partner, *state = self.v2v_min(verts, leave_room=overlap, zero=zero, iterative=iterative,
                                               cap=cap if capped else None)
            if capped and not overlap:
                self.v2v_fix(exterior, mn, partner, state[0])
            extra = call_also()
        if not first:
            exterior = self.exterior_flags(verts, apply_segments=apply_segments)
        if overlap:
            cur.wait_stream(side)
            for t in (mn, partner, *(st[0] for st in state), *(extra if isinstance(extra, (tuple, list)) else (extra,))):
                if torch.is_tensor(t):
                    t.record_stream(cur)
            if capped:
                self.v2v_fix(exterior, mn, partner, state[0])
        return exterior, mn, partner, extra

    def winding_tree_work(self, verts: torch.Tensor) -> dict:
        verts = _f32(verts)
        b = verts.shape[0]
        L = _C.lib()
        nbytes = L.tuch_exterior_workspace_bytes(self._handle, b)
        ws = _workspace(nbytes, verts.device)
        out = (ctypes.c_ulonglong * 4)()
        _C.check(L.tuch_winding_tree_work(self._handle, _C.ptr(verts), b, _C.ptr(ws), nbytes, out, _C.stream()))
        return dict(leaf_elements=int(out[0]), cap_elements=int(out[1]), wavefronts=int(out[2]),
                    flat_stream_elements=int(out[3]), queries_per_step=64,
                    query_blocks=-(-self.num_verts // 128) * 2 * b)

    def ray_work(self, verts: torch.Tensor) -> dict:
        verts = _f32(verts)
        b = verts.shape[0]
        L = _C.lib()
        nbytes = L.tuch_exterior_workspace_bytes(self._handle, b)
        ws = _workspace(nbytes, verts.device)
        out = (ctypes.c_ulonglong * 4)()
        _C.check(L.tuch_ray_work(self._handle, _C.ptr(verts), b, _C.ptr(ws), nbytes, out, _C.stream()))
        return dict(elements=int(out[0]), wavefronts=int(out[3]), queries_per_step=64,
                    lanes_inside_leaf_slabs=int(out[1]) / max(int(out[2]), 1))

    def exterior_flags(self, verts: torch.Tensor, apply_segments: bool = True, thresh: float = 0.99,
                       return_details: bool = False):
        verts = _f32(verts)
        b = verts.shape[0]
        assert verts.shape[1] == self.num_verts
        L = _C.lib()
        ext = torch.empty(b, self.num_verts, dtype=torch.uint8, device=verts.device)
        w = torch.empty(b, self.num_verts, dtype=torch.float32, device=verts.device) if return_details else None
        seg_w = seg_e = None
        if return_details and self.num_segments:
            seg_w = torch.empty(b, self.seg_q_total, dtype=torch.float32, device=verts.device)
            seg_e = torch.empty(b, self.seg_q_total, dtype=torch.uint8, device=verts.device)
        nbytes = L.tuch_exterior_workspace_bytes(self._handle, b)
        ws = _workspace(nbytes, verts.device)
        _C.check(L.tuch_exterior_flags(self._handle, _C.ptr(verts), b, int(apply_segments), float(thresh),
                                       _C.ptr(w), _C.ptr(ext), _C.ptr(seg_w), _C.ptr(seg_e), _C.ptr(ws), nbytes,
                                       _C.stream()))
        return (ext, w, seg_w, seg_e) if return_details else ext

    def v2v_min(self, verts: torch.Tensor, leave_room: bool = False, zero: Optional[torch.Tensor] = None, iterative: bool = False,
                cap: Optional[float] = None):
        if not self.has_mask:
            raise _C.TuchError('ContactModel was created without a geodesic mask')
        verts = _f32(verts)
        b = verts.shape[0]
        assert verts.shape[1] == self.num_verts
        L = _C.lib()
        mn = torch.empty(b, self.num_verts, dtype=torch.float32, device=verts.device)
        arg = torch.empty(b, self.num_verts, dtype=torch.int32, device=verts.device)
        nbytes = L.tuch_v2v_model_workspace_bytes(self._handle, b)
        ws = _workspace(nbytes, verts.device)
        flags = int(bool(leave_room)) | (2 if iterative else 0)
        zbytes = zero.numel() * zero.element_size() if zero is not None else 0
        if cap is not None:
            prev = self._v2v_prev(b)
            _C.check(L.tuch_v2v_min_model_capped(self._handle, _C.ptr(verts), b, _C.ptr(mn), _C.ptr(arg), _C.ptr(self._v2v_hint(b)),
                                                 _C.ptr(ws), nbytes, flags, _C.ptr(zero), zbytes, _C.ptr(prev), float(cap), _C.stream()))
            return mn, arg, (ws, nbytes, prev, float(cap))
        _C.check(L.tuch_v2v_min_model_shared_zero(self._handle, _C.ptr(verts), b, _C.ptr(mn), _C.ptr(arg),
                                                  _C.ptr(self._v2v_hint(b)), _C.ptr(ws), nbytes, flags, _C.ptr(zero), zbytes, _C.stream()))
        return mn, arg

    def v2v_can_cap(self, batch: int) -> bool:
        return bool(self.has_mask and _C.lib().tuch_v2v_min_model_can_cap(self._handle)) and self._v2v_hint(batch) is not None

    def v2v_fix(self, exterior: torch.Tensor, mn: torch.Tensor, arg: torch.Tensor, state) -> None:
        ws, nbytes, prev, cap = state
        b = exterior.shape[0]
        _C.check(_C.lib().tuch_v2v_min_model_fix(self._handle, b, _C.ptr(exterior), _C.ptr(prev), cap, _C.ptr(mn), _C.ptr(arg),
                                                 _C.ptr(self._v2v_hint(b)), _C.ptr(ws), nbytes, _C.stream()))

    def _v2v_prev(self, batch: int) -> torch.Tensor:
        buf = self._prev_flags.get(batch)
        if buf is None:
            buf = self._prev_flags[batch] = torch.zeros(batch, self.num_verts, dtype=torch.uint8, device=self.device)
        return buf

    def _v2v_hint(self, batch: int) -> Optional[torch.Tensor]:
        if not self._py_options['v2v_hint']:
            return None
        buf = self._hints.get(batch)
        if buf is None:
            n = _C.lib().tuch_v2v_hint_bytes(self._handle, batch)
            if n == 0:
                return None
            buf = torch.zeros(n, dtype=torch.uint8, device=self.device)
            self._hints[batch] = buf
        return buf

    def winding_points(self, verts: torch.Tensor, points: torch.Tensor, counts: Optional[torch.Tensor] = None,
                       thresh: float = 0.99, flags_only: bool = False):
        v, pts = _f32(verts), _f32(points)
        b, q, _ = pts.shape
        L = _C.lib()
        w = torch.empty(b, q, dtype=torch.float32, device=pts.device) if not flags_only else None
        ext = torch.empty(b, q, dtype=torch.uint8, device=pts.device)
        nbytes = L.tuch_winding_points_workspace_bytes(self._handle, b, q)
        ws = _workspace(nbytes, pts.device)
        _C.check(L.tuch_winding_points(self._handle, _C.ptr(v), _C.ptr(pts), _C.ptr(counts), b, q, float(thresh),
                                       _C.ptr(w), _C.ptr(ext), _C.ptr(ws), nbytes, _C.stream()))
        return w, ext

    def v2v_min_indexed(self, points: torch.Tensor, vertex_ids: torch.Tensor, offsets: torch.Tensor,
                        max_points: int, tree_order: bool = False, mfma: bool = False):
        if not self.has_mask:
            raise _C.TuchError('ContactModel was created without a geodesic mask')
        pts = _f32(points)
        n = pts.shape[0]
        mn = torch.empty(n, dtype=torch.float32, device=pts.device)
        arg = torch.empty(n, dtype=torch.int32, device=pts.device)
        L = _C.lib()
        bits = L.tuch_contact_model_tree_mask_bits(self._handle) if tree_order else \
            L.tuch_contact_model_mask_bits(self._handle)
        if not bits:
            raise _C.TuchError('ContactModel has no mask in tree order (no cluster tree)')
        size_fn, fn = (L.tuch_v2v_min_indexed_mfma_workspace_bytes, L.tuch_v2v_min_indexed_mfma) if mfma else \
            (L.tuch_v2v_min_indexed_workspace_bytes, L.tuch_v2v_min_indexed)
        nbytes = size_fn(offsets.shape[0] - 1, int(max_points))
        ws = _workspace(nbytes, pts.device)
        vertex_ids, offsets = vertex_ids.contiguous(), offsets.contiguous()
        _C.check(fn(_C.ptr(pts), _C.ptr(vertex_ids), _C.ptr(offsets),
# ... 132 lines not shown
```

Baseline: 151,500 body-fit iterations/s.

## Plan ray-winding leaf bins from previous iteration's per-leaf counts

Adds an iterative ray-winding path that keeps per-leaf pair counts from the previous fit step as a hint. It pre-allocates leaf bins and tiles with slack during the bounds kernel, so the near kernel can scatter pairs directly and the tile-fill pass is skipped when nothing overflows. If a bin overflows, it falls back to the old fill path. The new path is gated by a ray_plan option that defaults to 0, so it may not run unless enabled. It also adds state buffers, plus a report API for how often the plan is used or repaired.

```diff
diff --git a/include/tuch_amd.h b/include/tuch_amd.h
--- a/include/tuch_amd.h
+++ b/include/tuch_amd.h
@@ -180,6 +180,13 @@
 int tuch_exterior_flags(const tuch_contact_model* model, const float* verts, int B, int apply_segments,
                         float thresh, float* w, uint8_t* exterior, float* seg_w, uint8_t* seg_exterior,
                         void* workspace, size_t workspace_bytes, void* stream);
+size_t tuch_ray_hint_bytes(const tuch_contact_model* model, int B);
+int tuch_exterior_flags_iterative(const tuch_contact_model* model, const float* verts, int B, int apply_segments,
+                                  float thresh, float* w, uint8_t* exterior, float* seg_w, uint8_t* seg_exterior,
+                                  int32_t* ray_hint, size_t ray_hint_bytes, void* workspace, size_t workspace_bytes,
+                                  void* stream);
+int tuch_ray_plan_report(const tuch_contact_model* model, const int32_t* ray_hint, size_t ray_hint_bytes, int B,
+                         int32_t* out_host, void* stream);
 
 size_t tuch_winding_points_workspace_bytes(const tuch_contact_model* model, int B, int Q);
 int tuch_winding_points(const tuch_contact_model* model, const float* verts, const float* points,
diff --git a/tuch_amd/_C.py b/tuch_amd/_C.py
--- a/tuch_amd/_C.py
+++ b/tuch_amd/_C.py
@@ -107,6 +107,10 @@
                                        c_size_t, c_void_p]),
     'tuch_exterior_flags': (c_int, [c_void_p, c_void_p, c_int, c_int, c_float, c_void_p, c_void_p, c_void_p,
                                     c_void_p, c_void_p, c_size_t, c_void_p]),
+    'tuch_ray_hint_bytes': (c_size_t, [c_void_p, c_int]),
+    'tuch_exterior_flags_iterative': (c_int, [c_void_p, c_void_p, c_int, c_int, c_float, c_void_p, c_void_p, c_void_p,
+                                              c_void_p, c_void_p, c_size_t, c_void_p, c_size_t, c_void_p]),
+    'tuch_ray_plan_report': (c_int, [c_void_p, c_void_p, c_size_t, c_int, c_void_p, c_void_p]),
     'tuch_winding_points_workspace_bytes': (c_size_t, [c_void_p, c_int, c_int]),
     'tuch_winding_points': (c_int, [c_void_p, c_void_p, c_void_p, c_void_p, c_int, c_int, c_float, c_void_p, c_void_p,
                                     c_void_p, c_size_t, c_void_p]),
diff --git a/tuch_amd/csrc/model.h b/tuch_amd/csrc/model.h
--- a/tuch_amd/csrc/model.h
+++ b/tuch_amd/csrc/model.h
@@ -31,6 +31,8 @@
     int ray_waves = 32768;
     int ray_fans = 0;
     int ray_cross = 0;
+    int ray_plan = 0;
+    int ray_plan_slack = 2;
     int ray_cross_split = 0;
     int v2v_tree = 1;
     int v2v_waves = 0;
@@ -57,7 +59,8 @@
 size_t tuch_ray_workspace_bytes(const tuch_contact_model* m, int B, int Q);
 int tuch_ray_exterior_verts(const tuch_contact_model* m, const float* verts, int B, float thresh, uint8_t* exterior,
                             float* w, void* workspace, hipStream_t s, unsigned long long* stats_host,
-                            uint8_t* exterior_copy = nullptr);
+                            uint8_t* exterior_copy = nullptr, int32_t* ray_hint = nullptr);
+extern "C" size_t tuch_ray_hint_bytes(const tuch_contact_model* m, int B);
 const int32_t* tuch_ray_segment_counts(const tuch_contact_model* m, int B, const void* workspace);
 void tuch_ray_segment_prepare(const tuch_contact_model* m, const float* verts, const float* caps, int assisted, int B,
                               float* seg_entries, hipStream_t s);
diff --git a/tuch_amd/csrc/model.hip b/tuch_amd/csrc/model.hip
--- a/tuch_amd/csrc/model.hip
+++ b/tuch_amd/csrc/model.hip
@@ -451,7 +451,7 @@
 const OptionName kOptions[] = {
     {"winding_ray", &tuch_options::winding_ray}, {"winding_tree", &tuch_options::winding_tree},
     {"winding_strips", &tuch_options::winding_strips}, {"tree_waves", &tuch_options::tree_waves},
-    {"ray_pair_cap", &tuch_options::ray_pair_cap}, {"ray_waves", &tuch_options::ray_waves}, {"ray_fans", &tuch_options::ray_fans}, {"ray_cross", &tuch_options::ray_cross}, {"v2v_cap", &tuch_options::v2v_cap}, {"ray_cross_split", &tuch_options::ray_cross_split},
+    {"ray_pair_cap", &tuch_options::ray_pair_cap}, {"ray_waves", &tuch_options::ray_waves}, {"ray_fans", &tuch_options::ray_fans}, {"ray_cross", &tuch_options::ray_cross}, {"v2v_cap", &tuch_options::v2v_cap}, {"ray_cross_split", &tuch_options::ray_cross_split}, {"ray_plan", &tuch_options::ray_plan}, {"ray_plan_slack", &tuch_options::ray_plan_slack},
     {"v2v_tree", &tuch_options::v2v_tree}, {"v2v_flat", &tuch_options::v2v_flat}, {"v2v_pairs", &tuch_options::v2v_pairs}, {"v2v_waves", &tuch_options::v2v_waves}, {"v2v_lds", &tuch_options::v2v_lds},
     {"seg_splits", &tuch_options::seg_splits}, {"seg_assist", &tuch_options::seg_assist}, {"seg_fused", &tuch_options::seg_fused},
     {"canary", &tuch_options::canary}, {"hd_search", &tuch_options::hd_search}, {"hd_search_waves", &tuch_options::hd_search_waves}, {"hd_overlap", &tuch_options::hd_overlap},
diff --git a/tuch_amd/csrc/ray_winding.hip b/tuch_amd/csrc/ray_winding.hip
--- a/tuch_amd/csrc/ray_winding.hip
+++ b/tuch_amd/csrc/ray_winding.hip
@@ -110,6 +110,67 @@
 
 __device__ __forceinline__ float fan_terms(const float* __restrict__ vb, int v, bool real, int& n,
                                            const int32_t* __restrict__ ring_off, const int32_t* __restrict__ ring_vidx);
+
+struct RayPlanArgs {
+    const int32_t* hint;
+    int2* bins;
+    int32_t* state;
+    RayTile* tiles;
+    const int32_t* leaf_nodes;
+    int Q, cap, max_tiles, slack;
+};
+constexpr int kPlanMaxSlots = 32768;
+
+__device__ __forceinline__ int ray_plan_capacity(int h, int Q, int slack)
+{
+    if (h <= 0) return 0;
+    h = h > Q ? Q : h;
+    const int extra = max((int)(((long long)h * slack) >> 3), 16 * slack);
+    const long long c = ((long long)h + extra + 63) & ~63ll;
+    return (int)(c < 0x40000000ll ? c : 0x40000000ll);
+}
+
+__device__ __forceinline__ void ray_plan_body(const RayPlanArgs& p, const TreeNode* __restrict__ nodes, int L, int b)
+{
+    __shared__ long long sp[kBoundsBlock], st[kBoundsBlock];
+    const int t = threadIdx.x;
+    const int per = (L + kBoundsBlock - 1) / kBoundsBlock;
+    const int l0 = min(t * per, L), l1 = min(l0 + per, L);
+    const int32_t* hint = p.hint + (size_t)b * L;
+    long long npairs = 0, ntile = 0;
+    int big = 0;
+    for (int l = l0; l < l1; ++l) {
+        const int c = ray_plan_capacity(hint[l], p.Q, p.slack);
+        npairs += c;
+        ntile += c >> 6;
+        big |= (c >> 6) > kPlanMaxSlots;
+    }
+    sp[t] = npairs;
+    st[t] = ntile;
+    big = __syncthreads_or(big);
+    for (int d = 1; d < kBoundsBlock; d <<= 1) {
+        const long long ap = t >= d ? sp[t - d] : 0, at = t >= d ? st[t - d] : 0;
+        __syncthreads();
+        sp[t] += ap;
+        st[t] += at;
+        __syncthreads();
+    }
+    const long long total_pairs = sp[kBoundsBlock - 1], total_tiles = st[kBoundsBlock - 1];
+    const bool ok = !big && total_pairs <= p.cap && total_tiles <= p.max_tiles;
+    if (t == 0) *reinterpret_cast<int4*>(p.state + (size_t)b * 4) = make_int4(ok ? 1 : 0, ok ? (int)total_tiles : 0, 0, 0);
+    if (!ok) return;
+    int off = (int)(sp[t] - npairs), tile = (int)(st[t] - ntile);
+    RayTile* out = p.tiles + (size_t)b * p.max_tiles;
+    for (int l = l0; l < l1; ++l) {
+        const int c = ray_plan_capacity(hint[l], p.Q, p.slack);
+        p.bins[(size_t)b * L + l] = make_int2(off, c);
+        const TreeNode nd = nodes[p.leaf_nodes[l]];
+        for (int k = 0; k < (c >> 6); ++k)
+            out[tile++] = RayTile{nd.ex_off, nd.ex_len, off + 64 * k, (int32_t)(0x80000000u | (uint32_t)k << 16 | (uint32_t)l)};
+        off += c;
+    }
+}
+
 template <bool kPose>
 __global__ __launch_bounds__(kBoundsBlock) void ray_leaf_bounds_kernel(
     const RayElem* __restrict__ stream, int T, const TreeNode* __restrict__ nodes, int N,
@@ -118,13 +179,22 @@
     RayElem* __restrict__ stream_out, uint4* __restrict__ zeroed, size_t zeroed_n,
     int leaf_blocks = 0, const int32_t* __restrict__ qperm = nullptr, const int32_t* __restrict__ ring_off = nullptr,
     const int32_t* __restrict__ ring_vidx = nullptr, float2* __restrict__ fans = nullptr, int fan_stride = 0,
-    RayPre pre = RayPre{0, 0, nullptr, nullptr, nullptr})
-{
-    if (kPose && pre.blocks > 0 && (int)blockIdx.x >= (int)gridDim.x - pre.blocks) {
+    RayPre pre = RayPre{0, 0, nullptr, nullptr, nullptr},
+    RayPlanArgs plan = RayPlanArgs{nullptr, nullptr, nullptr, nullptr, nullptr, 0, 0, 0, 0})
+{
+    const int gx = (int)gridDim.x - (kPose && plan.hint ? 1 : 0);
+    if (kPose && plan.hint && (int)blockIdx.x == gx) {
         for (size_t g = ((size_t)blockIdx.y * gridDim.x + blockIdx.x) * kBoundsBlock + threadIdx.x; g < zeroed_n;
              g += (size_t)gridDim.x * gridDim.y * kBoundsBlock)
             zeroed[g] = make_uint4(0u, 0u, 0u, 0u);
-        const int qb = ((int)blockIdx.x - ((int)gridDim.x - pre.blocks)) * (kBoundsBlock / 64) + (int)(threadIdx.x >> 6);
+        ray_plan_body(plan, nodes, height_off[1] - height_off[0], blockIdx.y);
+        return;
+    }
+    if (kPose && pre.blocks > 0 && (int)blockIdx.x >= gx - pre.blocks) {
+        for (size_t g = ((size_t)blockIdx.y * gridDim.x + blockIdx.x) * kBoundsBlock + threadIdx.x; g < zeroed_n;
+             g += (size_t)gridDim.x * gridDim.y * kBoundsBlock)
+            zeroed[g] = make_uint4(0u, 0u, 0u, 0u);
+        const int qb = ((int)blockIdx.x - (gx - pre.blocks)) * (kBoundsBlock / 64) + (int)(threadIdx.x >> 6);
         if (qb < pre.qblocks)
             ray_block_prepass(verts + (size_t)blockIdx.y * V * 3, vidx[0], qperm, pre.vmask, V, qb, threadIdx.x & 63,
                               pre.qrec + (size_t)blockIdx.y * pre.qblocks * kRayQueries,
@@ -364,7 +434,7 @@
     return d;
 }
 
-template <bool kVerts, int kWaves>
+template <bool kVerts, int kWaves, bool kPlan = false>
 __global__ __launch_bounds__(64 * kWaves) void ray_near_kernel(
     const float* __restrict__ pts, const TreeNode* __restrict__ nodes, const float* __restrict__ bounds, int N,
     int num_leaves, const int32_t* __restrict__ qperm,
@@ -372,7 +442,9 @@
     int32_t* __restrict__ leaf_cnt,
     unsigned long long* __restrict__ stats,
     const int32_t* __restrict__ ring_off = nullptr, const int32_t* __restrict__ ring_vidx = nullptr,
-    float2* __restrict__ fans = nullptr)
+    float2* __restrict__ fans = nullptr,
+    const int2* __restrict__ bins = nullptr, int32_t* __restrict__ plan_state = nullptr, int32_t* __restrict__ pairs = nullptr,
+    int cap = 0)
 {
     if (kVerts && (int)blockIdx.x >= qblocks) {
         const int i = ((int)blockIdx.x - qblocks) * (64 * kWaves) + (int)threadIdx.x;
@@ -458,6 +530,34 @@
         return outside13(s0, s1, rx, rx, ry, ry, r4, r4, r5, r5, rz, r6, r7, r8, r9);
     };
     int nslots = 0;
+    const bool planned = kPlan && __builtin_amdgcn_readfirstlane(plan_state[(size_t)b * 4]) != 0;
+    int npend = 0, pend_leaf = 0;
+    uint32_t pend_lo = 0, pend_hi = 0;
+    auto place = [&]() {
+        if (npend == 0) return;
+        const bool have = lane < npend;
+        int dst = 0;
+        bool ok = false;
+        if (have) {
+            const int2 bin = bins[(size_t)b * num_leaves + pend_leaf];
+            const int n = __builtin_popcount(pend_lo) + __builtin_popcount(pend_hi);
+            const int old = atomicAdd(&leaf_cnt[(size_t)b * num_leaves + pend_leaf], n);
+            ok = old >= 0 && old <= bin.y - n;
+            dst = bin.x + old;
+        }
+        const unsigned long long okm = __builtin_amdgcn_ballot_w64(ok);
+        if (__builtin_amdgcn_ballot_w64(have && !ok) && lane == 0) plan_state[(size_t)b * 4 + 2] = 1;
+        int32_t* out = pairs + (size_t)b * cap;
+        for (int k = 0; k < npend; ++k) {
+            if (!((okm >> k) & 1ull)) continue;
+            const uint32_t lo = __builtin_amdgcn_readlane(pend_lo, k), hi = __builtin_amdgcn_readlane(pend_hi, k);
+            const int d = __builtin_amdgcn_readlane(dst, k);
+            const unsigned long long mask = ((unsigned long long)hi << 32) | lo;
+            if ((mask >> lane) & 1ull)
+                out[d + (int)__builtin_amdgcn_mbcnt_hi(hi, __builtin_amdgcn_mbcnt_lo(lo, 0))] = qb * kRayQueries + lane;
+        }
+        npend = 0;
+    };
     auto emit = [&](const uint4& s1, unsigned long long hit) {
         if (!hit) return;
         const int leaf = (int)(s1.z >> 16), nd = (int)s1.w;
@@ -465,7 +565,11 @@
         if (lane == 0) {
             const int slot = kWaves == 1 ? nslots - 1 : atomicAdd(&slots, 1);
             list[slot] = RayEntry{leaf, nd, (uint32_t)hit, (uint32_t)(hit >> 32)};
-            atomicAdd(&leaf_cnt[(size_t)b * num_leaves + leaf], __builtin_popcountll(hit));
+            if (!planned) atomicAdd(&leaf_cnt[(size_t)b * num_leaves + leaf], __builtin_popcountll(hit));
+        }
+        if (kPlan && planned) {
+            if (lane == npend) { pend_leaf = leaf; pend_lo = (uint32_t)hit; pend_hi = (uint32_t)(hit >> 32); }
+            if (++npend == 64) place();
         }
         if (stats) {
             const int len = nodes[nd].ex_len;
@@ -520,6 +624,7 @@
         }
         sync();
     }
+    if (kPlan) place();
     if (stats && lane == 0) { atomicAdd(stats + 1, useful); atomicAdd(stats + 2, listed); }
     if (threadIdx.x == 0) list_len[(size_t)b * qblocks + qb] = kWaves == 1 ? nslots : slots;
 }
@@ -605,7 +710,9 @@
     const int32_t* __restrict__ leaf_cnt, const TreeNode* __restrict__ nodes, const int32_t* __restrict__ leaf_nodes,
     int num_leaves, int cap, int max_tiles, int fallback_tiles, RayTile* __restrict__ tiles, RayBody* __restrict__ body,
     const RayEntry* __restrict__ lists, const int32_t* __restrict__ list_len, int qblocks, int32_t* __restrict__ leaf_fill,
-    int32_t* __restrict__ pairs, int list_stride)
+    int32_t* __restrict__ pairs, int list_stride,
+    const int32_t* __restrict__ plan_state = nullptr,
+    int32_t* __restrict__ hint = nullptr)
 {
     __builtin_amdgcn_s_setprio(3);
     extern __shared__ int32_t dyn[];
@@ -613,6 +720,20 @@
     int32_t* tile_s = dyn + num_leaves;
     int32_t* blk = dyn + 2 * num_leaves;
     const int b = blockIdx.x, lane = threadIdx.x;
+    if (plan_state) {
+        const bool walk = plan_state[(size_t)b * 4] != 0 && plan_state[(size_t)b * 4 + 2] == 0;
+        if (blockIdx.y == 0) {
+            for (int l = lane; l < num_leaves; l += kTilesFillBlock) hint[(size_t)b * num_leaves + l] = leaf_cnt[(size_t)b * num_leaves + l];
+            if (lane == 0) {
+                int32_t* rep = hint + (size_t)gridDim.x * num_leaves + (size_t)b * 4;
+                rep[0] = walk ? 1 : 0;
+                rep[1] += 1;
+                rep[2] += walk ? 0 : 1;
+                if (walk) body[b] = RayBody{plan_state[(size_t)b * 4 + 1], 0};
+            }
+        }
+        if (walk) return;
+    }
     const int per = (num_leaves + 63) / 64;
     const int l0 = min(lane * per, num_leaves), l1 = min(l0 + per, num_leaves);
     const int perq = (qblocks + 63) / 64;
@@ -683,7 +804,8 @@
     const int32_t* __restrict__ list_len, const TreeNode* __restrict__ nodes, int num_leaves,
     const int32_t* __restrict__ qperm, const int32_t* __restrict__ counts, int Q, int T, int qblocks, int num_bodies,
     int cap, int max_tiles, int32_t* __restrict__ count, unsigned long long* __restrict__ stats,
-    const int32_t* __restrict__ vmask, int32_t* __restrict__ seg_count)
+    const int32_t* __restrict__ vmask, int32_t* __restrict__ seg_count,
+    const int32_t* __restrict__ leaf_cnt)
 {
     const int lane = threadIdx.x;
     struct Work { int b, off, len, slot, qmask; bool active; float qx, qy, qz; };
@@ -698,17 +820,24 @@
             const int t = g - base;
             g += gridDim.y;
             const float* pb = pts + (size_t)b * Q * 3;
-            w.b = b;
             int i0;
             if (!__builtin_amdgcn_readfirstlane(body[b].overflow)) {
                 const RayTile tile = tiles[(size_t)b * max_tiles + t];
-                const int n = __builtin_amdgcn_readfirstlane(tile.n), first = __builtin_amdgcn_readfirstlane(tile.first);
+                int n = __builtin_amdgcn_readfirstlane(tile.n);
+                const int first = __builtin_amdgcn_readfirstlane(tile.first);
+                if (n < 0) {
+                    const int c = __builtin_amdgcn_readfirstlane(leaf_cnt[(size_t)b * num_leaves + (n & 0xffff)]);
+                    n = min(max(c - 64 * ((n >> 16) & 0x7fff), 0), 64);
+                    if (n == 0) continue;
+                }
                 w.active = lane < n;
                 w.slot = pairs[(size_t)b * cap + first + (w.active ? lane : 0)];
                 i0 = kVerts ? qperm[w.slot] : w.slot;
                 w.off = __builtin_amdgcn_readfirstlane(tile.ex_off);
                 w.len = __builtin_amdgcn_readfirstlane(tile.ex_len);
+                w.b = b;
             } else {
+                w.b = b;
                 const int nq = kVerts ? Q : (counts ? counts[b] : Q);
                 w.slot = (t / kFallbackChunks) * kRayQueries + lane;
                 w.active = w.slot < nq;
@@ -1307,7 +1436,7 @@
 
 struct RayLayout {
     size_t stream, bounds, lists, list_len, zeroed, zeroed_bytes, leaf_cnt, leaf_fill, count, leaf_off, tiles, body, pairs,
-        stats, fans, qrec, ranges, total;
+        stats, fans, qrec, ranges, bins, plan_state, total;
     int T, qblocks, cap, max_tiles, workers, columns;
     size_t seg_count;
 };
@@ -1606,6 +1735,8 @@
     l.fans = verts ? tuch_ws_take(o, (size_t)B * l.qblocks * kRayQueries * sizeof(float2)) : 0;
     l.qrec = verts ? tuch_ws_take(o, (size_t)B * l.qblocks * kRayQueries * sizeof(QRec)) : 0;
     l.ranges = verts ? tuch_ws_take(o, (size_t)B * l.qblocks * 4 * sizeof(float4)) : 0;
+    l.bins = verts ? tuch_ws_take(o, (size_t)B * L * sizeof(int2)) : 0;
+    l.plan_state = verts ? tuch_ws_take(o, (size_t)B * 4 * sizeof(int32_t)) : 0;
     l.total = o;
     return l;
 }
@@ -1633,7 +1764,7 @@
 }
 
 static void launch_ray_boxes(const tuch_contact_model* m, const RayLayout& l, const float* verts, int B, char* ws, hipStream_t s,
-                             bool one_launch, bool query_side = false)
+                             bool one_launch, bool query_side = false, const int32_t* plan_hint = nullptr)
 {
     RayElem* st = (RayElem*)(ws + l.stream);
     float* bounds = (float*)(ws + l.bounds);
@@ -1642,14 +1773,17 @@
     if (one_launch && m->tree_leaf_runs_tile) {
         const int leaf_blocks = ceil_div(m->tree_leaves, kBoundsBlock / 16);
         const bool fans = fans_in_bounds_launch(m);
-        hipLaunchKernelGGL(ray_leaf_bounds_kernel<true>, dim3(leaf_blocks + (fans ? ceil_div(m->V, kBoundsBlock) : 0) + pre.blocks, B),
+        const int slack = m->opt.ray_plan_slack < 1 ? 1 : (m->opt.ray_plan_slack > 64 ? 64 : m->opt.ray_plan_slack);
+        const RayPlanArgs plan{plan_hint, (int2*)(ws + l.bins), (int32_t*)(ws + l.plan_state), (RayTile*)(ws + l.tiles),
+                               (const int32_t*)m->tree_height_nodes, m->V, l.cap, l.max_tiles, slack};
+        hipLaunchKernelGGL(ray_leaf_bounds_kernel<true>, dim3(leaf_blocks + (fans ? ceil_div(m->V, kBoundsBlock) : 0) + pre.blocks + (plan_hint ? 1 : 0), B),
                            dim3(kBoundsBlock), 0,
                            s, (const RayElem*)st, l.T, (const TreeNode*)m->tree_node, m->tree_nodes,
                            (const int32_t*)m->tree_height_off, (const int32_t*)m->tree_height_nodes, bounds, verts,
                            (const int32_t*)m->tree_vidx, (const float*)m->tree_sign_word, m->V, m->tree_exact_len, st,
                            (uint4*)(ws + l.zeroed), l.zeroed_bytes / sizeof(uint4), fans ? leaf_blocks : 0,
                            (const int32_t*)m->tree_qperm, (const int32_t*)m->ring_off, (const int32_t*)m->ring_vidx,
-                           (float2*)(ws + l.fans), l.qblocks * kRayQueries, pre);
+                           (float2*)(ws + l.fans), l.qblocks * kRayQueries, pre, plan);
         return;
     }
     if (query_side)
@@ -1667,11 +1801,15 @@
 
 template <bool kVerts>
 static int launch_ray_counts(const tuch_contact_model* m, const RayLayout& l, const float* verts, const float* queries,
-                             const int32_t* counts, int B, int Q, char* ws, hipStream_t s, unsigned long long* stats)
+                             const int32_t* counts, int B, int Q, char* ws, hipStream_t s, unsigned long long* stats,
+                             int32_t* ray_hint = nullptr)
 {
     const bool one = kVerts && !stats && cross_in_one_launch(m);
-    launch_ray_boxes(m, l, verts, B, ws, s, kVerts, one);
     const int L = m->tree_leaves;
+    const size_t tf_lds = (2 * (size_t)L + l.qblocks + 1) * sizeof(int32_t);
+    const bool fill_in_one = l.qblocks <= kFillMaxBlocks && tf_lds <= 48u * 1024;
+    const bool plan = kVerts && ray_hint && m->opt.ray_plan != 0 && !stats && !one && m->tree_leaf_runs_tile && fill_in_one;
+    launch_ray_boxes(m, l, verts, B, ws, s, kVerts, one, plan ? ray_hint : nullptr);
     const TreeNode* nodes = (const TreeNode*)m->tree_node;
     if (one) {
         const int columns = B < 8 ? B : 8;
@@ -1700,7 +1838,25 @@
     int32_t* pairs = (int32_t*)(ws + l.pairs);
     const bool fans = kVerts && fans_in_near_launch(m);
     float2* fan_out = fans ? (float2*)(ws + l.fans) : nullptr;
-    if ((long)l.qblocks * B <= 2048)
+    bool near_done = false;
+    if constexpr (kVerts) {
+        if (plan) {
+            near_done = true;
+            const int2* bins = (const int2*)(ws + l.bins);
+            int32_t* state = (int32_t*)(ws + l.plan_state);
+            if ((long)l.qblocks * B <= 2048)
+                hipLaunchKernelGGL((ray_near_kernel<true, 4, true>), dim3(l.qblocks + (fans ? ceil_div(Q, 256) : 0), B), dim3(256), 0, s, queries,
+                                   nodes, (const float*)(ws + l.bounds), m->tree_nodes, L, qperm, counts, Q, l.qblocks, lists, list_len,
+                                   leaf_cnt, stats, (const int32_t*)m->ring_off, (const int32_t*)m->ring_vidx, fan_out, bins, state, pairs, l.cap);
+            else
+                hipLaunchKernelGGL((ray_near_kernel<true, 1, true>), dim3(l.qblocks + (fans ? ceil_div(Q, 64) : 0), B), dim3(64), 0, s, queries,
+                                   nodes, (const float*)(ws + l.bounds), m->tree_nodes, L, qperm, counts, Q, l.qblocks, lists, list_len,
+                                   leaf_cnt, stats, (const int32_t*)m->ring_off, (const int32_t*)m->ring_vidx, fan_out, bins, state, pairs, l.cap);
+        }
+    }
+    if (near_done)
+        ;
+    else if ((long)l.qblocks * B <= 2048)
         hipLaunchKernelGGL((ray_near_kernel<kVerts, 4>), dim3(l.qblocks + (fans ? ceil_div(Q, 256) : 0), B), dim3(256), 0, s, queries, nodes,
                            (const float*)(ws + l.bounds), m->tree_nodes, L, qperm, counts, Q, l.qblocks, lists, list_len,
                            leaf_cnt, stats, (const int32_t*)m->ring_off, (const int32_t*)m->ring_vidx, fan_out);
@@ -1708,11 +1864,11 @@
         hipLaunchKernelGGL((ray_near_kernel<kVerts, 1>), dim3(l.qblocks + (fans ? ceil_div(Q, 64) : 0), B), dim3(64), 0, s, queries, nodes,
                            (const float*)(ws + l.bounds), m->tree_nodes, L, qperm, counts, Q, l.qblocks, lists, list_len,
                            leaf_cnt, stats, (const int32_t*)m->ring_off, (const int32_t*)m->ring_vidx, fan_out);
-    const size_t tf_lds = (2 * (size_t)L + l.qblocks + 1) * sizeof(int32_t);
-    if (l.qblocks <= kFillMaxBlocks && tf_lds <= 48u * 1024)
+    if (fill_in_one)
         hipLaunchKernelGGL(ray_tiles_fill_kernel, dim3(B, std::min(256, std::max(kFillSplit, 2048 / B))), dim3(kTilesFillBlock), tf_lds, s, (const int32_t*)leaf_cnt,
                            nodes, leaf_nodes, L, l.cap, l.max_tiles, l.qblocks * kFallbackChunks, tiles, body,
-                           (const RayEntry*)lists, (const int32_t*)list_len, l.qblocks, (int32_t*)(ws + l.leaf_fill), pairs, L);
+                           (const RayEntry*)lists, (const int32_t*)list_len, l.qblocks, (int32_t*)(ws + l.leaf_fill), pairs, L,
+                           plan ? (const int32_t*)(ws + l.plan_state) : (const int32_t*)nullptr, plan ? ray_hint : (int32_t*)nullptr);
     else {
     hipLaunchKernelGGL(ray_tiles_kernel, dim3(B), dim3(kTilesBlock), 0, s, (const int32_t*)leaf_cnt, nodes, leaf_nodes, L, l.cap,
                        l.max_tiles, l.qblocks * kFallbackChunks, leaf_off, tiles, body);
@@ -1727,7 +1883,7 @@
     hipLaunchKernelGGL((ray_leaf_kernel<kVerts, COUNT, SEG>), grid, dim3(64), 0, s, queries, (const RayElem*)(ws + l.stream),  \
                        (const RayTile*)tiles, (const RayBody*)body, (const int32_t*)pairs, (const RayEntry*)lists,            \
                        (const int32_t*)list_len, nodes, L, qperm, counts, Q, l.T, l.qblocks, B, l.cap, l.max_tiles,           \
-                       (int32_t*)(ws + l.count), stats, vmask, seg_count)
+                       (int32_t*)(ws + l.count), stats, vmask, seg_count, (const int32_t*)leaf_cnt)
     if (stats) {
         if (seg) TUCH_LAUNCH_RAY_LEAF(true, kVerts); else TUCH_LAUNCH_RAY_LEAF(true, false);
     } else {
@@ -1738,13 +1894,14 @@
 }
 
 int tuch_ray_exterior_verts(const tuch_contact_model* m, const float* verts, int B, float thresh, uint8_t* exterior,
-                            float* w, void* workspace, hipStream_t s, unsigned long long* stats_host, uint8_t* exterior_copy)
+                            float* w, void* workspace, hipStream_t s, unsigned long long* stats_host, uint8_t* exterior_copy,
+                            int32_t* ray_hint)
 {
     const RayLayout l = full_layout(m, B, m->V, true);
     char* ws = (char*)workspace;
     unsigned long long* stats = stats_host ? (unsigned long long*)(ws + l.stats) : nullptr;
     if (stats && hipMemsetAsync(stats, 0, 4 * sizeof(unsigned long long), s) != hipSuccess) return TUCH_ERR_HIP;
-    const int rc = launch_ray_counts<true>(m, l, verts, verts, nullptr, B, m->V, ws, s, stats);
+    const int rc = launch_ray_counts<true>(m, l, verts, verts, nullptr, B, m->V, ws, s, stats, ray_hint);
     if (rc != TUCH_OK) return rc;
     if (w || exterior)
         hipLaunchKernelGGL(ray_finalize_verts_kernel, dim3(ceil_div(m->V, kBlock), B), dim3(kBlock), 0, s, verts,
@@ -1763,6 +1920,27 @@
         stats_host[3] = tiles * B / nb;
     }
     return tuch_check_launch("tuch_ray_exterior_verts");
+}
+
+extern "C" size_t tuch_ray_hint_bytes(const tuch_contact_model* m, int B)
+{
+    if (!tuch_ray_available(m) || B <= 0) return 0;
+    return ((size_t)B * m->tree_leaves + (size_t)B * 4) * sizeof(int32_t);
+}
+
+extern "C" int tuch_ray_plan_report(const tuch_contact_model* m, const int32_t* ray_hint, size_t ray_hint_bytes, int B,
+                                    int32_t* out_host, void* stream)
+{
+    TUCH_REQUIRE(m && ray_hint && out_host, "tuch_ray_plan_report: null pointer");
+    TUCH_REQUIRE(B > 0 && tuch_ray_hint_bytes(m, B) > 0 && ray_hint_bytes >= tuch_ray_hint_bytes(m, B),
+                 "tuch_ray_plan_report: hint of %zu bytes, batch %d", ray_hint_bytes, B);
+    hipStream_t s = (hipStream_t)stream;
+    if (hipMemcpyAsync(out_host, ray_hint + (size_t)B * m->tree_leaves, (size_t)B * 4 * sizeof(int32_t), hipMemcpyDeviceToHost, s) != hipSuccess ||
+        hipStreamSynchronize(s) != hipSuccess) {
+        tuch_set_error("tuch_ray_plan_report: copy back failed");
+        return TUCH_ERR_HIP;
+    }
+    return TUCH_OK;
 }
 
 const int32_t* tuch_ray_segment_counts(const tuch_contact_model* m, int B, const void* workspace)
diff --git a/tuch_amd/csrc/winding.hip b/tuch_amd/csrc/winding.hip
--- a/tuch_amd/csrc/winding.hip
+++ b/tuch_amd/csrc/winding.hip
@@ -851,10 +851,10 @@
     return exterior_layout(m, B).total;
 }
 
-extern "C" int tuch_exterior_flags(const tuch_contact_model* m, const float* verts, int B,
-                                   int apply_segments, float thresh, float* w, uint8_t* exterior,
-                                   float* seg_w, uint8_t* seg_exterior,
-                                   void* workspace, size_t workspace_bytes, void* stream)
+static int exterior_flags_impl(const tuch_contact_model* m, const float* verts, int B,
+                               int apply_segments, float thresh, float* w, uint8_t* exterior,
+                               float* seg_w, uint8_t* seg_exterior, int32_t* ray_hint,
+                               void* workspace, size_t workspace_bytes, void* stream)
 {
     TUCH_REQUIRE(m && verts && exterior, "tuch_exterior_flags: null pointer");
     TUCH_REQUIRE(B > 0 && B <= 65535, "tuch_exterior_flags: bad batch %d", B);
@@ -891,7 +891,7 @@
     }
     if (body_by_rays) {
         rc = tuch_ray_exterior_verts(m, verts, B, thresh, exterior, w, ws + l.ray, s, nullptr,
-                                     segments_fused ? (uint8_t*)(ws + l.body_flags) : (uint8_t*)nullptr);
+                                     segments_fused ? (uint8_t*)(ws + l.body_flags) : (uint8_t*)nullptr, ray_hint);
         if (rc != TUCH_OK) return rc;
     } else if (use_strips(m) && use_tree(m)) {
         launch_tree_walk(m, l, verts, B, ws, nullptr, s);
@@ -955,6 +955,28 @@
     return tuch_check_launch("tuch_exterior_flags");
 }
 
+extern "C" int tuch_exterior_flags(const tuch_contact_model* m, const float* verts, int B,
+                                   int apply_segments, float thresh, float* w, uint8_t* exterior,
+                                   float* seg_w, uint8_t* seg_exterior,
+                                   void* workspace, size_t workspace_bytes, void* stream)
+{
+    return exterior_flags_impl(m, verts, B, apply_segments, thresh, w, exterior, seg_w, seg_exterior, nullptr, workspace,
+                               workspace_bytes, stream);
+}
+
+extern "C" int tuch_exterior_flags_iterative(const tuch_contact_model* m, const float* verts, int B,
+                                             int apply_segments, float thresh, float* w, uint8_t* exterior,
+                                             float* seg_w, uint8_t* seg_exterior, int32_t* ray_hint, size_t ray_hint_bytes,
+                                             void* workspace, size_t workspace_bytes, void* stream)
+{
+    if (ray_hint) {
+        const size_t need = tuch_ray_hint_bytes(m, B);
+        TUCH_REQUIRE(need > 0 && ray_hint_bytes >= need, "tuch_exterior_flags_iterative: hint of %zu bytes, %zu needed", ray_hint_bytes, need);
+    }
+    return exterior_flags_impl(m, verts, B, apply_segments, thresh, w, exterior, seg_w, seg_exterior, ray_hint, workspace,
+                               workspace_bytes, stream);
+}
+
 extern "C" int tuch_winding_tree_work(const tuch_contact_model* m, const float* verts, int B,
                                       void* workspace, size_t workspace_bytes, unsigned long long* out_host, void* stream)
 {
diff --git a/tuch_amd/ops.py b/tuch_amd/ops.py
--- a/tuch_amd/ops.py
+++ b/tuch_amd/ops.py
@@ -705,6 +705,7 @@
         faces = np.asarray(faces.detach().cpu() if isinstance(faces, torch.Tensor) else faces)
         self.faces_np = faces.astype(np.int64)
         self._hints = {}
+        self._ray_hints = {}
         self._prev_flags = {}
         self.num_verts = int(faces.max()) + 1
         self.num_faces = int(faces.shape[0])
@@ -833,7 +834,7 @@
             cur, side = _current_stream(verts.device), _side_stream(verts.device)
             side.wait_stream(cur)
         first = not overlap or capped or self._py_options.get('inside_first', 0)
-        exterior = self.exterior_flags(verts, apply_segments=apply_segments) if first else None
+        exterior = self.exterior_flags(verts, apply_segments=apply_segments, iterative=iterative) if first else None
         with (torch.cuda.stream(side) if overlap else contextlib.nullcontext()):
             if overlap and zero is not None:
                 zero.record_stream(side)
@@ -843,7 +844,7 @@
                 self.v2v_fix(exterior, mn, partner, state[0])
             extra = call_also()
         if not first:
-            exterior = self.exterior_flags(verts, apply_segments=apply_segments)
+            exterior = self.exterior_flags(verts, apply_segments=apply_segments, iterative=iterative)
         if overlap:
             cur.wait_stream(side)
             for t in (mn, partner, *(st[0] for st in state), *(extra if isinstance(extra, (tuple, list)) else (extra,))):
@@ -877,7 +878,7 @@
                     lanes_inside_leaf_slabs=int(out[1]) / max(int(out[2]), 1))
 
     def exterior_flags(self, verts: torch.Tensor, apply_segments: bool = True, thresh: float = 0.99,
-                       return_details: bool = False):
+                       return_details: bool = False, iterative: bool = False):
         verts = _f32(verts)
         b = verts.shape[0]
         assert verts.shape[1] == self.num_verts
@@ -890,10 +891,35 @@
             seg_e = torch.empty(b, self.seg_q_total, dtype=torch.uint8, device=verts.device)
         nbytes = L.tuch_exterior_workspace_bytes(self._handle, b)
         ws = _workspace(nbytes, verts.device)
-        _C.check(L.tuch_exterior_flags(self._handle, _C.ptr(verts), b, int(apply_segments), float(thresh),
-                                       _C.ptr(w), _C.ptr(ext), _C.ptr(seg_w), _C.ptr(seg_e), _C.ptr(ws), nbytes,
-                                       _C.stream()))
+        hint = self._ray_hint(b) if iterative and verts.is_cuda else None
+        if hint is not None:
+            _C.check(L.tuch_exterior_flags_iterative(self._handle, _C.ptr(verts), b, int(apply_segments), float(thresh),
+                                                     _C.ptr(w), _C.ptr(ext), _C.ptr(seg_w), _C.ptr(seg_e), _C.ptr(hint),
+                                                     hint.numel() * hint.element_size(), _C.ptr(ws), nbytes, _C.stream()))
+        else:
+            _C.check(L.tuch_exterior_flags(self._handle, _C.ptr(verts), b, int(apply_segments), float(thresh),
+                                           _C.ptr(w), _C.ptr(ext), _C.ptr(seg_w), _C.ptr(seg_e), _C.ptr(ws), nbytes,
+                                           _C.stream()))
         return (ext, w, seg_w, seg_e) if return_details else ext
+
+    def _ray_hint(self, batch: int) -> Optional[torch.Tensor]:
+        buf = self._ray_hints.get(batch)
+        if buf is None:
+            n = _C.lib().tuch_ray_hint_bytes(self._handle, batch)
+            if n == 0:
+                return None
+            buf = self._ray_hints[batch] = torch.zeros(n // 4, dtype=torch.int32, device=self.device)
+        return buf
+
+    def ray_plan_report(self, batch: int) -> dict:
+        hint = self._ray_hint(batch)
+        if hint is None:
+            raise _C.TuchError('the model has no ray-crossing inside test')
+        out = (ctypes.c_int32 * (4 * batch))()
+        _C.check(_C.lib().tuch_ray_plan_report(self._handle, _C.ptr(hint), hint.numel() * hint.element_size(), batch, out,
+                                               _C.stream()))
+        rows = np.asarray(out, dtype=np.int32).reshape(batch, 4)
+        return dict(planned=rows[:, 0].astype(bool), calls=rows[:, 1].copy(), repaired=rows[:, 2].copy())
 
     def v2v_min(self, verts: torch.Tensor, leave_room: bool = False, zero: Optional[torch.Tensor] = None, iterative: bool = False,
                 cap: Optional[float] = None):
```

After: 149,700 body-fit iterations/s. -1.2%, worse.
